# ISLA-UH/quantum-inferno

Hardware: AMD Instinct MI355X
Metric: TFR Mpoints/sec (CWT+STX+entropy) (higher is better)
Workload: dtype f32; 1 GPU; BASELINE configs[1]: 1 channel(s) per GPU x 2^20 samples @ 1000 Hz, order N=3, CWT+STX+entropy, 48 bands; channels_per_gpu=1, n=1048576, bands=48, engine=auto, world_size=1, backend=none, gather_message_bytes_per_rank=0

## Files before the change

include/qi_tfr.h:

```cpp
#ifndef QI_TFR_H
#define QI_TFR_H

#include <stddef.h>
#include <stdint.h>

#ifdef __cplusplus
extern "C" {
#endif

#define QI_TFR_ABI_VERSION 1

typedef struct qi_plan qi_plan;
typedef void* qi_stream;

typedef enum { QI_F32 = 0, QI_F64 = 1 } qi_dtype;

typedef enum {
  QI_OK = 0,
  QI_ERR_ARG = -1,
  QI_ERR_STATE = -2,
  QI_ERR_HIP = -3,
  QI_ERR_FFT = -4,
  QI_ERR_NOMEM = -5,
  QI_ERR_UNSUPPORTED = -6
} qi_status;

typedef enum {
  QI_BANK_STYX = 0,
  QI_BANK_ATOMS = 1
} qi_bank;

typedef enum {
  QI_ENGINE_AUTO = 0,
  QI_ENGINE_HIPFFT = 1,
  QI_ENGINE_NATIVE = 2
} qi_engine;

typedef struct {
  int64_t n;
  int32_t dtype;
  int32_t device;
  int32_t engine;
  int32_t flags;
  int64_t workspace_bytes;
} qi_plan_desc;

typedef struct {
  void* coef;
  void* bits;
  void* power_band;
  void* power_time;
  void* stats;
  double power_scale;
  double eps;
} qi_tfr_out;

int qi_abi_version(void);
const char* qi_last_error(void);
int qi_device_info(int device, char* name, size_t name_len, int64_t* hbm_bytes, int32_t* compute_units);

int qi_plan_create(qi_plan** plan, const qi_plan_desc* desc);
int qi_plan_destroy(qi_plan* plan);

int qi_plan_set_gabor_bank(qi_plan* plan, int bank, int32_t n_bands, const double* p_re, const double* p_im,
                           const double* omega, const double* amp, qi_stream stream);

int qi_gabor_atoms(int device, int64_t n, int32_t n_bands, const double* p_re, const double* p_im,
                   const double* omega, const double* amp, void* out, qi_stream stream);

int qi_gabor_atoms_at(int device, int64_t n, int32_t n_bands, const double* p_re, const double* p_im,
                      const double* omega, const double* amp, const void* x, void* out, qi_stream stream);

int qi_plan_set_stx_bands(qi_plan* plan, int32_t n_bands, const int64_t* shift_index, const double* sigma);

int64_t qi_plan_bands(const qi_plan* plan, int which );
int64_t qi_plan_stage_bands(const qi_plan* plan, int which, int stage);

typedef struct {
  int32_t stage, cls, run_cls, flags;
} qi_band_route;
#define QI_ROUTE_ANALYTIC(f) ((f) & 3)
#define QI_ROUTE_NARROW(f) (((f) >> 2) & 3)
#define QI_ROUTE_NOWRAP 16
#define QI_ROUTE_SPLIT 32
#define QI_ROUTE_PASS2_KIND(f) (((f) >> 6) & 3)
#define QI_ROUTE_BEHIND 256
#define QI_ROUTE_F64_ZOOM 512
int qi_plan_band_route(const qi_plan* plan, int which, int32_t band, int64_t records, qi_band_route* route);

typedef enum {
  QI_STAGE_FORWARD = 0,
  QI_STAGE_MULTIPLY = 1,
  QI_STAGE_INVERSE = 2,
  QI_STAGE_EPILOGUE = 3,
  QI_STAGE_PASS1 = 4,
  QI_STAGE_PASS2 = 5,
  QI_STAGE_BLOCK = 6,
  QI_STAGE_ZOOM = 7,
  QI_STAGE_ZOOM_COARSE = 8,
  QI_STAGE_COUNT = 9
} qi_stage;
int qi_plan_profile(qi_plan* plan, int enable);
int qi_plan_profile_read(qi_plan* plan, double* stage_ms, int64_t* stage_launches, int32_t n_stages);

int qi_cwt(qi_plan* plan, int bank, const void* sig, int64_t n_channels, const qi_tfr_out* out, qi_stream stream);

int qi_stx(qi_plan* plan, const void* sig, int64_t n_channels, const qi_tfr_out* out, qi_stream stream);

int qi_cwt_stx(qi_plan* plan, int bank, const void* sig, int64_t n_channels, const qi_tfr_out* out_cwt,
               const qi_tfr_out* out_stx, qi_stream stream);

int64_t qi_stft_segments(int64_t n, int64_t seg, int64_t hop);
int64_t qi_stft_scratch_bytes(int dtype, int64_t n_channels, int64_t n, int64_t seg, int64_t hop, int64_t nfft);
int qi_stft(int dtype, int device, const void* sig, int64_t n_channels, int64_t n, const void* window, int64_t seg,
            int64_t hop, int64_t nfft, double scale, void* Z, void* bits, double eps, void* scratch,
            int64_t scratch_bytes, qi_stream stream);

int64_t qi_welch_scratch_bytes(int dtype, int64_t n_channels, int64_t n, int64_t seg, int64_t hop, int64_t nfft);
int qi_welch(int dtype, int device, const void* sig, int64_t n_channels, int64_t n, const void* window, int64_t seg,
             int64_t hop, int64_t nfft, double scale, void* pxx, void* scratch, int64_t scratch_bytes,
             qi_stream stream);

int qi_power_marginals(int dtype, int device, const void* power, int64_t n_channels, int64_t n_bands, int64_t n,
                       void* power_band, void* power_time, void* stats, void* scratch, int64_t scratch_bytes,
                       qi_stream stream);
int64_t qi_power_marginals_scratch_bytes(int64_t n_channels, int64_t n_bands, int64_t n);

int qi_log2_offset(int dtype, int device, const void* in, void* out, int64_t n_channels, int64_t count, double eps,
                   const void* ref, qi_stream stream);

int qi_widen(int device, const void* in, void* out, int64_t count, qi_stream stream);

int qi_log2_abs(int dtype, int device, const void* in, int is_complex, void* out, int64_t count, double eps,
                qi_stream stream);

int qi_shannon_panel(int dtype, int device, const void* power, const void* mult, int mode, int64_t n_channels,
                     int64_t n_bands, int64_t n, double deg_free, void* info, void* shannon_bits, void* isnr,
                     void* esnr, qi_stream stream);

int64_t qi_sliding_scratch_bytes(int dtype, int64_t n_channels, int64_t nfft, int64_t n_slices);
int qi_sliding_stft(int dtype, int device, const void* sig, int64_t n_channels, int64_t n, const void* window,
                    int64_t seg, int64_t hop, int64_t nfft, int64_t first, int64_t n_slices, int pad_mode, int detrend,
                    int64_t roll, void* Z, void* real_out, int real_kind, void* scratch, int64_t scratch_bytes,
                    qi_stream stream);
int qi_sliding_istft(int dtype, int device, const void* S, int64_t n_channels, const void* dual_window, int64_t seg,
                     int64_t hop, int64_t nfft, int64_t first, int64_t n_slices, int64_t roll, int64_t k0, int64_t k1,
                     void* out, void* scratch, int64_t scratch_bytes, qi_stream stream);

int qi_shannon_1d(int dtype, int device, const void* marginal, int64_t n_channels, int64_t n, void* info, void* entropy,
                  void* isnr, void* esnr, qi_stream stream);
int64_t qi_shannon_scratch_bytes(int dtype, int64_t n_channels, int64_t n);
int qi_shannon_tdr(int dtype, int device, const void* sig, int64_t n_channels, int64_t n, void* sig_norm, void* marginal,
                   void* scratch, int64_t scratch_bytes, qi_stream stream);
int qi_shannon_fft(int dtype, int device, const void* sig, int64_t n_channels, int64_t n, void* spectrum, void* angle,
                   void* marginal, void* scratch, int64_t scratch_bytes, qi_stream stream);

#ifdef __cplusplus
}
#endif
// ... 2 lines not shown
```

quantum_inferno_amd/_lib.py:

```python
import ctypes as C
import os

import torch

_HERE = os.path.dirname(os.path.abspath(__file__))
LIB_PATH = os.environ.get("QI_TFR_LIB") or os.path.join(_HERE, "libqi_tfr.so")

QI_F32, QI_F64 = 0, 1
QI_BANK_STYX, QI_BANK_ATOMS, QI_TABLE_STX = 0, 1, 2
QI_ENGINE_AUTO, QI_ENGINE_HIPFFT, QI_ENGINE_NATIVE = 0, 1, 2
STAGES = ("forward", "multiply", "inverse", "epilogue", "pass1", "pass2", "block", "zoom", "zoom_coarse")
ROUTE_NOWRAP, ROUTE_SPLIT, ROUTE_BEHIND, ROUTE_F64_ZOOM = 16, 32, 256, 512


def route_analytic(flags):
    return flags & 3


def route_narrow(flags):
    return (flags >> 2) & 3


def route_pass2_kind(flags):
    return (flags >> 6) & 3


class QiError(RuntimeError):
    pass


class PlanDesc(C.Structure):
    _fields_ = [
        ("n", C.c_int64),
        ("dtype", C.c_int32),
        ("device", C.c_int32),
        ("engine", C.c_int32),
        ("flags", C.c_int32),
        ("workspace_bytes", C.c_int64),
    ]


class BandRoute(C.Structure):
    _fields_ = [("stage", C.c_int32), ("cls", C.c_int32), ("run_cls", C.c_int32), ("flags", C.c_int32)]


class TfrOut(C.Structure):
    _fields_ = [
        ("coef", C.c_void_p),
        ("bits", C.c_void_p),
        ("power_band", C.c_void_p),
        ("power_time", C.c_void_p),
        ("stats", C.c_void_p),
        ("power_scale", C.c_double),
        ("eps", C.c_double),
    ]


_P = C.c_void_p
_D = C.POINTER(C.c_double)
_I64 = C.POINTER(C.c_int64)
_i64, _i32, _int, _dbl = C.c_int64, C.c_int32, C.c_int, C.c_double

PROTOTYPES = {
    "qi_abi_version": (_int, []),
    "qi_last_error": (C.c_char_p, []),
    "qi_device_info": (_int, [_int, C.c_char_p, C.c_size_t, _I64, C.POINTER(_i32)]),
    "qi_plan_create": (_int, [C.POINTER(_P), C.POINTER(PlanDesc)]),
    "qi_plan_destroy": (_int, [_P]),
    "qi_plan_set_gabor_bank": (_int, [_P, _int, _i32, _D, _D, _D, _D, _P]),
    "qi_gabor_atoms": (_int, [_int, _i64, _i32, _D, _D, _D, _D, _P, _P]),
    "qi_gabor_atoms_at": (_int, [_int, _i64, _i32, _D, _D, _D, _D, _P, _P, _P]),
    "qi_plan_set_stx_bands": (_int, [_P, _i32, _I64, _D]),
    "qi_plan_bands": (_i64, [_P, _int]),
    "qi_plan_stage_bands": (_i64, [_P, _int, _int]),
    "qi_plan_band_route": (_int, [_P, _int, _i32, _i64, C.POINTER(BandRoute)]),
    "qi_plan_profile": (_int, [_P, _int]),
    "qi_plan_profile_read": (_int, [_P, _D, _I64, _i32]),
    "qi_cwt": (_int, [_P, _int, _P, _i64, C.POINTER(TfrOut), _P]),
    "qi_stx": (_int, [_P, _P, _i64, C.POINTER(TfrOut), _P]),
    "qi_cwt_stx": (_int, [_P, _int, _P, _i64, C.POINTER(TfrOut), C.POINTER(TfrOut), _P]),
    "qi_stft_segments": (_i64, [_i64, _i64, _i64]),
    "qi_stft_scratch_bytes": (_i64, [_int, _i64, _i64, _i64, _i64, _i64]),
    "qi_stft": (_int, [_int, _int, _P, _i64, _i64, _P, _i64, _i64, _i64, _dbl, _P, _P, _dbl, _P, _i64, _P]),
    "qi_welch_scratch_bytes": (_i64, [_int, _i64, _i64, _i64, _i64, _i64]),
    "qi_welch": (_int, [_int, _int, _P, _i64, _i64, _P, _i64, _i64, _i64, _dbl, _P, _P, _i64, _P]),
    "qi_power_marginals": (_int, [_int, _int, _P, _i64, _i64, _i64, _P, _P, _P, _P, _i64, _P]),
    "qi_power_marginals_scratch_bytes": (_i64, [_i64, _i64, _i64]),
    "qi_log2_offset": (_int, [_int, _int, _P, _P, _i64, _i64, _dbl, _P, _P]),
    "qi_widen": (_int, [_int, _P, _P, _i64, _P]),
    "qi_log2_abs": (_int, [_int, _int, _P, _int, _P, _i64, _dbl, _P]),
    "qi_shannon_panel": (_int, [_int, _int, _P, _P, _int, _i64, _i64, _i64, _dbl, _P, _P, _P, _P, _P]),
    "qi_sliding_scratch_bytes": (_i64, [_int, _i64, _i64, _i64]),
    "qi_sliding_stft": (_int, [_int, _int, _P, _i64, _i64, _P, _i64, _i64, _i64, _i64, _i64, _int, _int, _i64, _P, _P, _int, _P, _i64, _P]),
    "qi_sliding_istft": (_int, [_int, _int, _P, _i64, _P, _i64, _i64, _i64, _i64, _i64, _i64, _i64, _i64, _P, _P, _i64, _P]),
    "qi_shannon_1d": (_int, [_int, _int, _P, _i64, _i64, _P, _P, _P, _P, _P]),
    "qi_shannon_scratch_bytes": (_i64, [_int, _i64, _i64]),
    "qi_shannon_tdr": (_int, [_int, _int, _P, _i64, _i64, _P, _P, _P, _i64, _P]),
    "qi_shannon_fft": (_int, [_int, _int, _P, _i64, _i64, _P, _P, _P, _P, _i64, _P]),
}

_lib = None


def _hip_runtimes_mapped():
    try:
        with open("/proc/self/maps") as fh:
            return sorted({ln.split()[-1] for ln in fh if "libamdhip64" in ln})
    except OSError:
        return []


def load():
    global _lib
    if _lib is not None:
        return _lib
    if not os.path.exists(LIB_PATH):
        raise QiError(
            f"{LIB_PATH} is missing: build it with `python -c 'import __graft_entry__ as g; g.build()'` "
            "(hipcc --offload-arch=gfx950).  There is no CPU fallback."
        )
    lib = C.CDLL(LIB_PATH)
    for name, (res, args) in PROTOTYPES.items():
        fn = getattr(lib, name)
        fn.restype = res
        fn.argtypes = args
    rts = _hip_runtimes_mapped()
    if len(rts) > 1:
        raise QiError(f"two HIP runtimes are mapped ({rts}); libqi_tfr.so must share torch's")
    _lib = lib
    return lib


def check(rc):
    if rc != 0:
        msg = load().qi_last_error()
        raise QiError(f"libqi_tfr error {rc}: {msg.decode() if msg else '?'}")


def require_gpu():
    if not torch.cuda.is_available():
        raise QiError("no HIP device visible: the TFR transforms run only on the GPU (no CPU fallback)")
    return load()


def darr(a):
    import numpy as np

    a = np.ascontiguousarray(a, dtype=np.float64)
    return a, a.ctypes.data_as(_D)


def iarr(a):
    import numpy as np

    a = np.ascontiguousarray(a, dtype=np.int64)
    return a, a.ctypes.data_as(_I64)

# ... 8 lines not shown
```

quantum_inferno_amd/csrc/qi_api.hip:

```cpp
#include "qi_host.hpp"

using namespace qi;
using namespace qi::host;

extern "C" {

int qi_abi_version(void) { return QI_TFR_ABI_VERSION; }
const char* qi_last_error(void) { return qi::last_error(); }

int qi_device_info(int device, char* name, size_t name_len, int64_t* hbm_bytes, int32_t* compute_units) {
  hipDeviceProp_t prop;
  QI_HIP(hipGetDeviceProperties(&prop, device));
  if (name && name_len) snprintf(name, name_len, "%s (%s)", prop.name, prop.gcnArchName);
  if (hbm_bytes) *hbm_bytes = (int64_t)prop.totalGlobalMem;
  if (compute_units) *compute_units = prop.multiProcessorCount;
  return QI_OK;
}

int qi_plan_create(qi_plan** plan, const qi_plan_desc* desc) {
  QI_REQUIRE(plan && desc, "null plan/desc");
  *plan = nullptr;
  QI_REQUIRE(desc->n >= 2 && desc->n <= (1ll << 28), "n = %lld out of range", (long long)desc->n);
  QI_REQUIRE(desc->dtype == QI_F32 || desc->dtype == QI_F64, "bad dtype %d", desc->dtype);
  QI_REQUIRE(desc->engine >= QI_ENGINE_AUTO && desc->engine <= QI_ENGINE_NATIVE, "bad engine %d", desc->engine);
  QI_REQUIRE(desc->flags == 0, "qi_plan_desc.flags = %d: the field is reserved and must be 0", desc->flags);
  if (desc->engine == QI_ENGINE_NATIVE && !(is_pow2(desc->n) && desc->n >= (1 << 18) &&
                                            (desc->dtype == QI_F32 || desc->n == (1 << 20)))) {
    set_error("native engine: float32 records of a power-of-two length >= 2^18, float64 records of 2^20 samples (got n = %lld, dtype %d)",
              (long long)desc->n, desc->dtype);
    return QI_ERR_UNSUPPORTED;
  }
  DeviceGuard g(desc->device);
  if (!g.ok) {
    set_error("hipSetDevice(%d) failed", desc->device);
    return QI_ERR_HIP;
  }
  qi_plan* p = new (std::nothrow) qi_plan();
  QI_REQUIRE(p, "out of host memory");
  p->d = *desc;
  p->n = desc->n;
  p->L = is_pow2(desc->n) ? 2 * desc->n : next_pow2(2 * desc->n - 1);
  if (p->native_kmax > (int64_t)native::kMaxPrunedTerms * native::kN2)
    p->native_kmax = (int64_t)native::kMaxPrunedTerms * native::kN2;
  if (const char* e = tune_env("QI_NATIVE_DEBUG")) p->native_debug = atoi(e);
  if (const char* e = tune_env("QI_NATIVE_FWD")) p->native_fwd = atoi(e);
#ifdef QI_NATIVE_STAMPS
  if (tune_env("QI_NATIVE_STAMPS")) {
    if (hipMalloc((void**)&p->stamps, 65536 * 8 * sizeof(unsigned long long)) != hipSuccess) p->stamps = nullptr;
    if (p->stamps) (void)hipMemset(p->stamps, 0, 65536 * 8 * sizeof(unsigned long long));
    if (hipMalloc((void**)&p->blk_stamps, 65536 * 8 * sizeof(unsigned long long)) != hipSuccess) p->blk_stamps = nullptr;
    if (p->blk_stamps) (void)hipMemset(p->blk_stamps, 0, 65536 * 8 * sizeof(unsigned long long));
  }
#endif
  if (const char* e = tune_env("QI_NATIVE_SHORT")) p->native_short = atoi(e);
  if (const char* e = tune_env("QI_NATIVE_BLOCK")) p->native_block = atoi(e);
  if (const char* e = tune_env("QI_NATIVE_ZOOM")) p->native_zoom = atoi(e);
  if (const char* e = tune_env("QI_NATIVE_ZOOM_LEVELS")) p->native_zoom_max_level = atoi(e);
  if (const char* e = tune_env("QI_NATIVE_SPLIT")) p->native_split = atoi(e);
  if (const char* e = tune_env("QI_NATIVE_FUSE")) p->native_fuse = atoi(e);
  if (const char* e = tune_env("QI_NATIVE_F64")) p->native_f64 = atoi(e);
  if (const char* e = tune_env("QI_NATIVE_Z64")) p->native_z64 = atoi(e);
  if (const char* e = tune_env("QI_NATIVE_Z64_FINE")) p->native_z64_fine = atoi(e);
  if (const char* e = tune_env("QI_NATIVE_Z64_COARSE")) p->native_z64_coarse = atoi(e);
  if (const char* e = tune_env("QI_NATIVE_Z64_BLOCK_FROM")) p->native_z64_block_from = atoi(e);
  if (const char* e = tune_env("QI_NATIVE_BLK64_WTAB")) p->native_blk64_wtab = atoi(e);
  if (const char* e = tune_env("QI_NATIVE_BLK64_NARROW")) p->native_blk64_narrow = atoi(e);
  if (const char* e = tune_env("QI_NATIVE_MIN_LOG2N")) p->native_min_log2n = atoi(e);
  if (desc->dtype == QI_F64) {
    if (!tune_env("QI_NATIVE_MIN_LOG2N")) p->native_min_log2n = 15;
    const int short64 = p->native_short && !(tune_env("QI_NATIVE_SHORT64") && atoi(tune_env("QI_NATIVE_SHORT64")) == 0);
    const int block64 = p->native_block && !(tune_env("QI_NATIVE_BLOCK64") && atoi(tune_env("QI_NATIVE_BLOCK64")) == 0);
    const int split64 = p->native_split && block64 && p->native_z64 &&
                        !(tune_env("QI_NATIVE_SPLIT64") && atoi(tune_env("QI_NATIVE_SPLIT64")) == 0);
    p->native_zoom = 0;
    p->native_split = split64;
    p->native_split_e = 2048;
    p->native_block = block64;
    p->native_short = short64;
    p->native_rows = 8;
    if (p->native_group <= 0) p->native_group = 8;
  }
  p->ws_bytes = desc->workspace_bytes > 0 ? (size_t)desc->workspace_bytes : ((size_t)2 << 30);
  if (hipMalloc((void**)&p->ws, p->ws_bytes) != hipSuccess) {
    set_error("hipMalloc of %zu workspace bytes failed", p->ws_bytes);
    delete p;
    return QI_ERR_HIP;
  }
  *plan = p;
  return QI_OK;
}

int qi_plan_destroy(qi_plan* p) {
  if (!p) return QI_OK;
  DeviceGuard g(p->d.device);
  (void)hipDeviceSynchronize();
  p->fft.clear();
  p->prof.clear();
#ifdef QI_NATIVE_STAMPS
  if (p->stamps) {
    std::vector<unsigned long long> h(65536 * 8);
    if (hipMemcpy(h.data(), p->stamps, h.size() * sizeof(unsigned long long), hipMemcpyDeviceToHost) == hipSuccess) {
      double sum[8] = {0};
      long cnt = 0;
      for (size_t w = 0; w < 65536; ++w) {
        unsigned long long tot = 0;
        for (int k = 0; k < 8; ++k) tot += h[w * 8 + k];
        if (!tot) continue;
        ++cnt;
        for (int k = 0; k < 8; ++k) sum[k] += (double)h[w * 8 + k];
      }
      fprintf(stderr, "[qi stamps] last pass-2 launch, %ld workgroups, mean cycles per workgroup: load %.0f | barrier %.0f | "
              "step1 %.0f | barrier %.0f | exchange %.0f | step2 %.0f | epilogue %.0f | loop head %.0f\n", cnt,
              sum[0] / cnt, sum[1] / cnt, sum[2] / cnt, sum[3] / cnt, sum[4] / cnt, sum[5] / cnt, sum[6] / cnt, sum[7] / cnt);
    }
    (void)hipFree(p->stamps);
  }
  if (p->blk_stamps) {
    std::vector<unsigned long long> h(65536 * 8);
    if (hipMemcpy(h.data(), p->blk_stamps, h.size() * sizeof(unsigned long long), hipMemcpyDeviceToHost) == hipSuccess) {
      if (const char* path = tune_env("QI_NATIVE_TIMELINE")) {
        if (FILE* f = fopen(path, "w")) {
          fprintf(f, "wg start_10ns end_10ns xcc cu bands wq\n");
          const unsigned long long m48 = 0xffffffffffffull;
          for (size_t w = 0; w < 65536; ++w)
            if (h[w * 8 + 7])
              fprintf(f, "%zu %llu %llu %llu %llu %llu %lld\n", w, h[w * 8 + 6] & m48, h[w * 8 + 7] & m48, h[w * 8 + 6] >> 56,
                      (h[w * 8 + 6] >> 48) & 0xff, (h[w * 8 + 7] >> 48) & 0xff, (long long)(signed char)(h[w * 8 + 7] >> 56));
          fclose(f);
// ... 94 lines not shown
  if (!use_native && p->d.engine == QI_ENGINE_NATIVE) {
    set_error("native engine does not support this bank at n = %lld", (long long)p->n);
    return QI_ERR_UNSUPPORTED;
  }
  drop_gabor_tables(p, bank);
  drop_band_slots(p, bank);
  const int rc = build_gabor_bank(p, bank, B, p_re, p_im, omega, amp, use_native, st);
  if (rc == QI_OK) {
    p->nb[bank] = B;
  } else {
    drop_gabor_tables(p, bank);
    free_device(p->bank[bank]);
  }
  return rc;
}

static int atoms_rows(int64_t n, int32_t B, const double* p_re, const double* p_im, const double* omega, const double* amp,
                      const double* x, void* out, hipStream_t st) {
  std::vector<double> host;
  DeviceTemp<double> d_par;
  QI_TRY(upload_atom_params(B, p_re, p_im, omega, amp, &host, &d_par));
  const double* q = d_par.ptr;
  QI_TRY(launch_bank_rows((double2*)out, n, n, 1, q, q + B, q + 2 * B, q + 3 * B, 0, B, st, 0.0, x));
  if (hipStreamSynchronize(st) != hipSuccess) {
    set_error("atom kernel failed: %s", hipGetErrorString(hipGetLastError()));
    return QI_ERR_HIP;
  }
  return QI_OK;
}

int qi_gabor_atoms(int device, int64_t n, int32_t B, const double* p_re, const double* p_im, const double* omega,
                   const double* amp, void* out, qi_stream stream) {
  QI_REQUIRE(p_re && p_im && omega && amp && out, "null argument");
  QI_REQUIRE(n >= 2 && B > 0 && B <= 65535, "bad atom bank shape");
  DeviceGuard g(device);
  return atoms_rows(n, B, p_re, p_im, omega, amp, nullptr, out, (hipStream_t)stream);
}

int qi_gabor_atoms_at(int device, int64_t n, int32_t B, const double* p_re, const double* p_im, const double* omega,
                      const double* amp, const void* x, void* out, qi_stream stream) {
  QI_REQUIRE(p_re && p_im && omega && amp && x && out, "null argument");
  QI_REQUIRE(n >= 1 && B > 0 && B <= 65535, "bad atom bank shape");
  DeviceGuard g(device);
  return atoms_rows(n, B, p_re, p_im, omega, amp, static_cast<const double*>(x), out, (hipStream_t)stream);
}

int qi_plan_set_stx_bands(qi_plan* p, int32_t B, const int64_t* shift_index, const double* sigma) {
  QI_REQUIRE(p && shift_index && sigma, "null argument");
  QI_REQUIRE(B > 0 && B <= 65535, "band count %d out of range", B);
  for (int32_t j = 0; j < B; ++j)
    QI_REQUIRE(shift_index[j] >= 0 && shift_index[j] < p->n, "shift_index[%d] = %lld outside [0, n)", j,
               (long long)shift_index[j]);
  for (int32_t j = 0; j < B; ++j)
    QI_REQUIRE(std::isfinite(sigma[j]) && sigma[j] > 0.0, "sigma[%d] = %g: must be positive and finite", j, sigma[j]);
  DeviceGuard g(p->d.device);
  p->table_gen++;
  if (p->d_stx_idx) {
    QI_HIP(hipDeviceSynchronize());
    QI_HIP(hipFree(p->d_stx_idx));
    QI_HIP(hipFree(p->d_stx_coef));
    p->d_stx_idx = nullptr;
    p->d_stx_coef = nullptr;
    p->nb_stx = 0;
  }
  std::vector<double> coef(B);
  const double k = 2.0 * M_PI / (double)p->n * std::sqrt(0.5 * M_LOG2E);
  for (int32_t j = 0; j < B; ++j) coef[j] = sigma[j] * k;
  QI_TRY(upload_table(&p->d_stx_idx, std::vector<int64_t>(shift_index, shift_index + B)));
  QI_TRY(upload_table(&p->d_stx_coef, coef));
  p->nb_stx = 0;
  drop_stx_tables(p);
  drop_band_slots(p, 2);
  QI_TRY(build_stx_tables(p, B, shift_index, sigma, coef));
  p->nb_stx = B;
  return QI_OK;
}

int64_t qi_plan_bands(const qi_plan* p, int which) {
  if (!p) return 0;
  if (which == QI_BANK_STYX || which == QI_BANK_ATOMS) return p->nb[which];
  return which == 2 ? p->nb_stx : 0;
}

int64_t qi_plan_stage_bands(const qi_plan* p, int which, int stage) {
  if (!p || which < 0 || which > 2) return 0;
  const int64_t total = qi_plan_bands(p, which);
  if (!p->nat[which].ready) return stage == QI_STAGE_INVERSE ? total : 0;
  int64_t blk = 0;
  if (which != 1 && p->blk[which].ready) blk = p->blk[which].rows;
  const int64_t zoom = p->nat[which].nzoom + p->nat[which].nz64;
  const int64_t left = which == 2 ? p->stx_left_n : 0;
  if (stage == QI_STAGE_BLOCK) return blk;
  if (stage == QI_STAGE_ZOOM) return zoom;
  if (stage == QI_STAGE_INVERSE) return left;
  return stage == QI_STAGE_PASS2 ? total - blk - zoom - left : 0;
}

int qi_plan_band_route(const qi_plan* p, int which, int32_t band, int64_t records, qi_band_route* route) {
  QI_REQUIRE(p && route, "null argument");
  QI_REQUIRE(which >= 0 && which <= 2, "bad table %d", which);
  QI_REQUIRE(band >= 0 && band < qi_plan_bands(p, which), "band %d outside the table's %lld rows", band,
             (long long)qi_plan_bands(p, which));
  QI_REQUIRE(records > 0, "records must be positive");
  *route = qi_band_route{QI_STAGE_INVERSE, 0, 0, 0};
  const auto& t = p->nat[which];
  if (!t.ready) return QI_OK;
  if (which == 2 && p->stx_left_n > 0 && band >= p->stx_left_lo && band < p->stx_left_lo + p->stx_left_n) {
    route->flags = QI_ROUTE_BEHIND;
    return QI_OK;
  }
  int found = 0;
  const bool split = which == 0 && std::find(p->h_split_bands.begin(), p->h_split_bands.end(), band) != p->h_split_bands.end();
  for (const auto& z : t.h_zoom)
    if (z.first == band) {
      const int run = records < p->native_zoom_short_from && z.second >= native::kZoomLevels ? 0 : z.second;
      *route = qi_band_route{QI_STAGE_ZOOM, z.second, run, split ? QI_ROUTE_SPLIT : 0};
      ++found;
    }
  for (size_t q = 0; q < t.h_z64.size(); ++q)
    if (t.h_z64[q] == band) {
      int level = -1, fine = -1;
      for (int g = 0; g < native::kZ64Levels; ++g)
        if ((int32_t)q >= t.z64_first[g] && (int32_t)q < t.z64_first[g] + t.z64_count[g]) level = g;
      for (int c = 0; c < native::kZ64FineClasses; ++c)
        if ((int32_t)q >= t.zf_first[c] && (int32_t)q < t.zf_first[c] + t.zf_count[c]) fine = c;
      *route = qi_band_route{QI_STAGE_ZOOM, level, fine, QI_ROUTE_F64_ZOOM | (split ? QI_ROUTE_SPLIT : 0)};
      ++found;
    }
  if (which != 1 && p->blk[which].ready) {
    const int cut = records >= batch_from(p) ? 1 : 0;
    for (const auto& b : p->blk[which].var[cut].h_route)
      if (b.out_band == band) {
        *route = qi_band_route{QI_STAGE_BLOCK, b.wq, b.wq, (b.analytic & 3) | ((b.narrow & 3) << 2) | (b.nowrap ? QI_ROUTE_NOWRAP : 0)};
        ++found;
      }
  }
  for (size_t q = 0; q < t.h_rows.size(); ++q)
    if (t.h_rows[q] == band) {
      *route = qi_band_route{QI_STAGE_PASS2, 0, 0, (t.h_row_mode[q] & 3) << 6};
      ++found;
    }
  if (which == 0 && p->nat[3].ready)
    for (int32_t r : p->nat[3].h_rows)
      if (r == band) {
        *route = qi_band_route{QI_STAGE_PASS2, 0, 0, 2 << 6};
        ++found;
      }
  if (found != 1) {
    set_error("band %d of table %d has %d producers", band, which, found);
    return QI_ERR_STATE;
  }
  return QI_OK;
}

int qi_plan_profile(qi_plan* p, int enable) {
  QI_REQUIRE(p, "null plan");
  DeviceGuard g(p->d.device);
  double ms[Profiler::kStages];
  int64_t c[Profiler::kStages];
  p->prof.read(ms, c);
  p->prof.on = enable != 0;
  p->prof.mask = (enable & 0xFFFF) == 1 ? ~0u : (uint32_t)(enable & 0xFFFF) >> 1;
  p->prof.period = (enable >> 16) > 0 ? (enable >> 16) : 1;
  p->prof.tick = 0;
  return QI_OK;
}
// ... 120 lines not shown
```

quantum_inferno_amd/csrc/qi_block.hip:

```cpp
#include "qi_common.hpp"
#include "qi_device.hpp"
#include "qi_native.hpp"
#include "qi_fft_reg.hpp"
#include "qi_zoom_gather.hpp"

namespace qi {
namespace native {

namespace {

constexpr int kBlkThreads = 256;
#ifndef QI_BLK_WAVES
#define QI_BLK_WAVES 3
#endif
#ifndef QI_BLK_LONG_WAVES
#define QI_BLK_LONG_WAVES 2
#endif
#ifdef QI_NATIVE_DEBUG
#define QI_BDBG(bit) (a.debug & (bit))
#else
#define QI_BDBG(bit) false
#endif
#ifdef QI_NATIVE_STAMPS
#define QI_BSTAMP(k)                                               \
// ... 1150 lines not shown
  __shared__ cplx<T> buf[kBlkBuf];
  __shared__ cplx<T> tw256[256];
  __shared__ double s_red[2][kBlkThreads / kWave];
  const int tid = threadIdx.x;
  {
    float s, c;
    sincospif((float)tid * (2.0f / 256.0f), &s, &c);
    tw256[tid] = mk<T>((T)c, (T)s);
  }
  cplx<T> w;
  {
    float s, c;
    const int lane = tid & (kWave - 1);
    const int col = (tid & ~(kWave - 1)) + (lane < 32 ? 2 * lane : 2 * (lane - 32) + 1);
    sincospif((float)col * (2.0f / 4096.0f), &s, &c);
    w = mk<T>((T)c, (T)s);
  }
  const DualItem it = load_uniform(items + blockIdx.x);
#ifdef QI_NATIVE_STAMPS
  const unsigned long long wall0 = __builtin_amdgcn_s_memrealtime();
#endif
  if (it.wq < 0) {
    const BlockItem e{it.wq, it.block, it.first0, it.count0, it.plane0, it.slot0};
    switch (-it.wq) {
      case 1: edge_item<T, 1, COEF, BITS>(a0, e, buf, tw256, w); break;
      case 2: edge_item<T, 2, COEF, BITS>(a0, e, buf, tw256, w); break;
      default: edge_item<T, 4, COEF, BITS>(a0, e, buf, tw256, w); break;
    }
  } else {
    switch (it.wq) {
      case 1: dual_item<T, 1, COEF, BITS>(a0, a2, it, buf, tw256, s_red, w); break;
      case 2: dual_item<T, 2, COEF, BITS>(a0, a2, it, buf, tw256, s_red, w); break;
      default: dual_item<T, 4, COEF, BITS>(a0, a2, it, buf, tw256, s_red, w); break;
    }
  }
#ifdef QI_NATIVE_STAMPS
  if (a0.stamps && tid == 0) {
    asm volatile("s_waitcnt vmcnt(0) lgkmcnt(0)" ::: "memory");
    unsigned long long* o = a0.stamps + ((int64_t)blockIdx.z * gridDim.x + blockIdx.x) * 8;
    unsigned hw;
    asm volatile("s_getreg_b32 %0, hwreg(HW_REG_HW_ID)" : "=s"(hw));
    unsigned xcc;
    asm volatile("s_getreg_b32 %0, hwreg(HW_REG_XCC_ID)" : "=s"(xcc));
    o[6] = (wall0 & 0xffffffffffffull) | ((unsigned long long)(xcc & 15) << 56) | ((unsigned long long)((hw >> 8) & 0xff) << 48);
    o[7] = (__builtin_amdgcn_s_memrealtime() & 0xffffffffffffull) | ((unsigned long long)(it.wq & 0xff) << 56) |
           ((unsigned long long)((it.count0 + it.count2) & 0xff) << 48);
  }
#endif
}

template <typename T>
__device__ __forceinline__ void zoom_coarse_plane(cplx<T>* __restrict__ plane0) {
  __shared__ cplx<T> buf[kBlkBuf];
  __shared__ cplx<T> tw256[256];
  const int tid = threadIdx.x, lane = tid & (kWave - 1);
  const int col = (tid & ~(kWave - 1)) + (lane < 32 ? 2 * lane : 2 * (lane - 32) + 1);
  cplx<T>* __restrict__ plane = plane0 + col;
  cplx<T> v[16];
#pragma unroll
  for (int b = 0; b < 16; ++b) v[b] = plane[256 * b];
  {
    float s, c;
    sincospif((float)tid * (2.0f / 256.0f), &s, &c);
    tw256[tid] = mk<T>((T)c, (T)s);
  }
  cplx<T> w;
  {
    float s, c;
    sincospif((float)col * (2.0f / 4096.0f), &s, &c);
    w = mk<T>((T)c, (T)s);
  }
  fft4096<T, 1>(v, buf, tw256, w, tid, col);
#pragma unroll
  for (int c = 0; c < 16; ++c) plane[256 * c] = v[brev(c, 4)];
}
template <typename T, bool STX, int NF>
__device__ __forceinline__ void zoom_coarse_plane_gather(const ZoomArgs<T>& a, const uint32_t plane_i,
                                                         cplx<T>* __restrict__ buf, cplx<T>* __restrict__ tw256) {
  const int tid = threadIdx.x, lane = tid & (kWave - 1);
  const int col = (tid & ~(kWave - 1)) + (lane < 32 ? 2 * lane : 2 * (lane - 32) + 1);
  const BandDesc bd = load_uniform(a.bands + *as_const(a.plane_band + plane_i));
  const uint32_t tau1 = plane_i - (uint32_t)bd.edge;
  const int64_t ch = blockIdx.z;
  const cplx<T>* __restrict__ X = a.X + ch * (a.Lf << a.x_shift);
  cplx<T> v[16];
#ifdef QI_NATIVE_DEBUG
  if (a.debug & 256) {
#pragma unroll
    for (int b = 0; b < 16; ++b) v[b] = mk<T>((T)(col + b), (T)tau1);
  } else
#endif
  zoom_gather16<T, STX, NF>(a, bd, tau1, col, X, v);
  {
    float s, c;
    sincospif((float)tid * (2.0f / 256.0f), &s, &c);
    tw256[tid] = mk<T>((T)c, (T)s);
  }
  cplx<T> w;
  {
    float s, c;
    sincospif((float)col * (2.0f / 4096.0f), &s, &c);
    w = mk<T>((T)c, (T)s);
  }
#ifdef QI_NATIVE_DEBUG
  if (!(a.debug & 512))
#endif
  fft4096<T, 1>(v, buf, tw256, w, tid, col);
  cplx<T>* __restrict__ plane = a.coarse + ((int64_t)ch * a.planes + plane_i) * kBlk + col;
#ifdef QI_NATIVE_DEBUG
  if ((a.debug & 1024) && v[3].x != (T)12345.678f) return;
#endif
#pragma unroll
  for (int c = 0; c < 16; ++c) plane[256 * c] = v[brev(c, 4)];
}
template <typename T, int NF>
__global__ void __launch_bounds__(kBlkThreads) k_zoom_coarse2g(ZoomArgs<T> a0, ZoomArgs<T> a2) {
  __shared__ cplx<T> buf[kBlkBuf];
  __shared__ cplx<T> tw256[256];
#ifdef QI_COARSE_PLAIN_ORDER
  const uint32_t pi = blockIdx.x;
#else
  const uint32_t q = blockIdx.x >> 3, pi = (q >> 3) * 64u + (blockIdx.x & 7u) * 8u + (q & 7u);
#endif
  if (pi >= (uint32_t)(a0.planes + a2.planes)) return;
  if (pi < (uint32_t)a0.planes) zoom_coarse_plane_gather<T, false, NF>(a0, pi, buf, tw256);
  else zoom_coarse_plane_gather<T, true, NF>(a2, pi - (uint32_t)a0.planes, buf, tw256);
}
template <typename T, bool STX>
__global__ void __launch_bounds__(kBlkThreads) k_zoom_coarse_g(ZoomArgs<T> a) {
  __shared__ cplx<T> buf[kBlkBuf];
  __shared__ cplx<T> tw256[256];
  zoom_coarse_plane_gather<T, STX, 8>(a, blockIdx.x, buf, tw256);
}

template <typename T>
__global__ void __launch_bounds__(kBlkThreads) k_zoom_coarse(ZoomArgs<T> a) {
  zoom_coarse_plane<T>(a.coarse + ((int64_t)blockIdx.z * a.planes + blockIdx.x) * kBlk);
}
template <typename T>
__global__ void __launch_bounds__(kBlkThreads) k_zoom_coarse2(ZoomArgs<T> a0, ZoomArgs<T> a2) {
  const bool first = blockIdx.x < (uint32_t)a0.planes;
  const ZoomArgs<T>& a = first ? a0 : a2;
  const int64_t plane = first ? blockIdx.x : blockIdx.x - (uint32_t)a0.planes;
  zoom_coarse_plane<T>(a.coarse + ((int64_t)blockIdx.z * a.planes + plane) * kBlk);
}

__global__ void k_block_taps_gabor(double2* __restrict__ g, int w, const double* __restrict__ par, int nb_total,
                                   const int32_t* __restrict__ ids) {
  const int j = ids[blockIdx.y];
  const double p_re = par[j], p_im = par[nb_total + j], omega = par[2 * nb_total + j], amp = par[3 * nb_total + j];
  double2* row = g + (int64_t)blockIdx.y * kBlk;
  for (int m = blockIdx.x * blockDim.x + threadIdx.x; m < kBlk; m += gridDim.x * blockDim.x) {
    int u;
    bool on = true;
    if (m <= w) u = -m;
    else if (m > kBlk - w) u = kBlk - m;
    else { u = 0; on = false; }
    double2 v = make_double2(0.0, 0.0);
    if (on) {
      const double x = (double)u + 0.5;
      const double env = amp * exp(-p_re * x * x);
      const double ph = omega * x - p_im * x * x;
      double s, c;
      sincos(ph, &s, &c);
      v = make_double2(env * c, -env * s);
    }
    row[m] = v;
// ... 357 lines not shown
```

quantum_inferno_amd/csrc/qi_host.hpp:

```cpp
#pragma once
#include <algorithm>
#include <cmath>
#include <cstring>
#include <map>
#include <mutex>
#include <new>
#include <tuple>
#include <vector>

#include <cstdlib>

#include "qi_common.hpp"
#include "qi_native.hpp"

namespace qi {

struct DeviceGuard {
  int prev = -1;
  bool ok = true;
  explicit DeviceGuard(int dev) {
    if (hipGetDevice(&prev) != hipSuccess) prev = -1;
    if (prev != dev) ok = hipSetDevice(dev) == hipSuccess;
  }
  ~DeviceGuard() {
// ... 141 lines not shown
    cur = last = -1;
  }
  void clear() {
    double ms[kStages];
    int64_t c[kStages];
    read(ms, c);
    for (auto e : pool) (void)hipEventDestroy(e);
    pool.clear();
  }
};

template <typename P>
inline void free_device(P*& ptr) {
  if (ptr) (void)hipFree(ptr);
  ptr = nullptr;
}
template <typename P, typename X>
inline int upload_table(P** dst, const std::vector<X>& v) {
  QI_HIP(hipMalloc((void**)dst, v.size() * sizeof(X)));
  QI_HIP(hipMemcpy(*dst, v.data(), v.size() * sizeof(X), hipMemcpyHostToDevice));
  return QI_OK;
}
template <typename X>
struct DeviceTemp {
  X* ptr = nullptr;
  DeviceTemp() = default;
  DeviceTemp(const DeviceTemp&) = delete;
  DeviceTemp& operator=(const DeviceTemp&) = delete;
  ~DeviceTemp() { free_device(ptr); }
};

extern std::mutex g_stft_mu;
extern std::map<int, FftCache> g_stft_fft;
const char* last_error();

}

using namespace qi;

struct FusedCarry {
  bool active = false;
  size_t ws_used = 0;
  native::BlockArgs<float> blk{};
  int demod = 0;
  int64_t ct = 0;
  native::TailCall<float> tail;
  bool has_zoom = false;
  native::ZoomArgs<float> zoom{};
};

struct qi_plan {
  qi_plan_desc d{};
  int64_t n = 0;
  int64_t L = 0;
  void* bank[2] = {nullptr, nullptr};
  int32_t nb[2] = {0, 0};
  int64_t* d_stx_idx = nullptr;
  double* d_stx_coef = nullptr;
  int32_t nb_stx = 0;
  char* ws = nullptr;
  size_t ws_bytes = 0;
  FftCache fft;
  Profiler prof;
  struct NativeGroup {
    int32_t first = 0, count = 0;
    int32_t gen_first = 0, ngen = 0;
  };
  struct NativeTable {
    bool ready = false;
    int64_t Lf = 0;
    int32_t nbands = 0, ngen = 0, imd_slots = 0;
    native::BandDesc* d_bands = nullptr;
    int32_t* d_gen_list = nullptr;
    std::vector<NativeGroup> groups;
    void* Hc = nullptr;
    void* Hfull = nullptr;
    native::BandDesc* d_zoom = nullptr;
    int32_t* d_zoom_plane_band = nullptr;
    std::vector<std::pair<int32_t, int32_t>> h_zoom;
    std::vector<int32_t> h_rows;
    std::vector<int32_t> h_row_mode;
    std::vector<int32_t> h_z64;
    int32_t nzoom = 0, zoom_count[native::kZoomClasses] = {0, 0, 0, 0, 0, 0, 0};
    int64_t zoom_planes = 0;
    int zoom_max_level = 0;
    native::BandDesc* d_z64 = nullptr;
    int32_t nz64 = 0, z64_first[native::kZ64Levels] = {}, z64_count[native::kZ64Levels] = {};
    int32_t zf_first[native::kZ64FineClasses] = {}, zf_count[native::kZ64FineClasses] = {};
    double2* d_z64_lane_ph = nullptr;
    double2* d_z64_wave_ph = nullptr;
    void release() {
      free_device(d_z64);
      free_device(d_z64_lane_ph);
      free_device(d_z64_wave_ph);
      free_device(d_zoom);
      free_device(d_zoom_plane_band);
      free_device(d_bands);
      free_device(d_gen_list);
      free_device(Hc);
      free_device(Hfull);
      *this = NativeTable();
    }
  } nat[4];
  struct BlockTable {
    bool ready = false;
    int demod = 0;
    void* bank = nullptr;
    int32_t rows = 0;
    struct ItemList {
      void* d_bands = nullptr;
      void* d_demod_pow = nullptr;
      void* d_gauss_w = nullptr;
      std::vector<std::pair<int32_t, int32_t>> h_bands;
      struct Route {
        int32_t out_band, wq, analytic, narrow, nowrap;
      };
      std::vector<Route> h_route;
      native::BlockItem* d_items = nullptr;
      int32_t nitems = 0, nplanes = 0;
      int32_t nlong = 0;
      int32_t nedge_items = 0;
      bool edge_merged = false;
      std::vector<native::BlockItem> h_items;
    } var[2];
    int64_t max_blocks = 0;
    void release() {
      free_device(bank);
      for (auto& v : var) {
        free_device(v.d_bands);
        free_device(v.d_demod_pow);
        free_device(v.d_gauss_w);
        free_device(v.d_items);
      }
      *this = BlockTable();
    }
  } blk[3];
  struct {
    int64_t C = -1, tile = 0;
    unsigned flags = 0;
    uint64_t gen = 0;
  } tile_cache;
  uint64_t table_gen = 1;
  int native_block = 1;
  const void* shared_sig = nullptr;
  int64_t shared_C = 0;
  bool shared_valid = false;
  int32_t* d_band_slots[3][2] = {};
  int native_zoom = 1;
  int native_zoom_short = 1;
  int native_zoom_short_from = 4;
  int native_zoom_max_level = 3;
  int native_zoom_waves = 2048;
  int native_zoom_wgs_joint = 768;
  int native_zoom_wgs = 0;
  float* d_zoom_w[native::kZoomClasses] = {};
  int native_z64 = 1;
  int native_z64_levels = native::kZ64Levels;
  double* d_z64_w[native::kZ64Levels] = {};
  double* d_z64f_w[native::kZ64FineClasses] = {};
  double2* d_demod_t1 = nullptr;
  double2* d_demod_t2 = nullptr;
  int native_z64_fine = 1;
  int32_t stx_left_lo = -1, stx_left_n = 0;
  int native_min_log2n = 14;
  int native_blk64_narrow = 1;
  int native_blk64_wtab = 1;
  int native_z64_block_from = 4;
  int native_z64_coarse = 3;
  int native_z64_rows = 0;
  int native_f64 = 1;
  int native_gather_fused = 1;
  hipStream_t side = nullptr;
  hipEvent_t ev_fork = nullptr, ev_join = nullptr;
  int native_split = 1;
  int64_t native_split_e = 1024;
  void* split_bank = nullptr;
  int32_t* d_split_bands = nullptr;
  std::vector<int32_t> h_split_bands;
  int32_t nsplit = 0;
  int native_blk_analytic = 1;
  FusedCarry carry;
  native::DualItem* d_dual[2] = {nullptr, nullptr};
  int32_t n_dual[2] = {0, 0};
  int32_t n_dual_long[2] = {0, 0};
  bool dual_valid[2] = {false, false};
  int native_fuse = 4;
  int native_blk_narrow = 1;
  int native_blk_fastw = 1;
  int native_edge_merge = 1;
  int native_blk_long = 1;
  int native_blk_half = 1;
  int native_tail = 1;
  int64_t native_tile = 0;
  int native_blk_maxwq = 4;
  int native_blk_bands = 6;
  int native_blk_bands_batch = 12;
  int native_blk_batch_from = 0;
  native::EdgeBand* d_edge = nullptr;
  int32_t nedge = 0;
  int64_t edge_wmax = 0;
  int native_short = 1;
  int64_t native_kmax = 12288;
  int native_debug = 0;
  int native_fwd = 1;
  int native_wgs = 256;
  unsigned long long* stamps = nullptr;
  unsigned long long* blk_stamps = nullptr;
  int native_group = 0;
  int native_rows = 16;
};

namespace qi {
namespace host {

inline size_t align_up(size_t v, size_t a = 256) { return (v + a - 1) / a * a; }
inline double power_scale_or_default(double power_scale) { return power_scale == 0.0 ? 1.0 : power_scale; }
inline double eps_or_default(double eps) { return eps == 0.0 ? 2.220446049250313e-16 : eps; }
enum class Kind { Linear, Circular, Stockwell };
#ifdef QI_HOST_SANITIZE
void layout_begin(const qi_plan* p, const char* run, bool keep_previous);
void layout_note(const qi_plan* p, const char* what, const void* ptr, size_t bytes, bool shared = false);
#define QI_LAYOUT_BEGIN(p, run, keep) ::qi::host::layout_begin(p, run, keep)
#define QI_LAYOUT_NOTE(p, what, ptr, bytes, ...) ::qi::host::layout_note(p, what, ptr, bytes, ##__VA_ARGS__)
#else
#define QI_LAYOUT_BEGIN(p, run, keep) ((void)0)
#define QI_LAYOUT_NOTE(p, what, ptr, bytes, ...) ((void)0)
#endif
constexpr int kZoomListOrder[native::kZoomClasses] = {6, 5, 0, 1, 2, 3, 4};

bool native_len_ok(int64_t Lf);
bool native_wanted(const qi_plan* p, int kind);
int batch_from(const qi_plan* p);
void release_styx_extras(qi_plan* p);
void drop_gabor_tables(qi_plan* p, int bank);
void drop_stx_tables(qi_plan* p);
void drop_band_slots(qi_plan* p, int kind);
int upload_atom_params(int32_t B, const double* p_re, const double* p_im, const double* omega, const double* amp,
                       std::vector<double>* host, DeviceTemp<double>* d_par);
template <typename T>
int build_native_bank(qi_plan* p, int bank, int32_t B, const double* d_par, const double* h_par, hipStream_t st);
template <typename T>
int build_bank(qi_plan* p, int bank, int32_t B, const double* d_par, hipStream_t st);
int build_stx_tables(qi_plan* p, int32_t B, const int64_t* shift_index, const double* sigma, const std::vector<double>& coef);

template <typename T>
int run_transform(qi_plan* p, Kind kind, const void* sig_v, int64_t C, const qi_tfr_out* out, hipStream_t st);
template <typename T>
int run_native(qi_plan* p, int kind, const void* sig_v, int64_t C, const qi_tfr_out* out, hipStream_t st,
               bool may_share = false, FusedCarry* defer = nullptr, FusedCarry* finish = nullptr, size_t* probe = nullptr);
template <typename T>
int run_stx_leftover(qi_plan* p, const void* sig, int64_t C, const qi_tfr_out* out, hipStream_t st);
int run_native64(qi_plan* p, int kind, const void* sig_v, int64_t C, const qi_tfr_out* out, hipStream_t st);
int flush_carry(qi_plan* p, FusedCarry* c, hipStream_t st);

}
}
```

quantum_inferno_amd/csrc/qi_host_util.hip:

```cpp
#include "qi_host.hpp"

namespace qi {

static thread_local char g_err[512] = "";

const char* tune_env(const char* name) {
  static const bool on = std::getenv("QI_TUNE") != nullptr;
  return on ? std::getenv(name) : nullptr;
}

void set_error(const char* fmt, ...) {
  va_list ap;
  va_start(ap, fmt);
  vsnprintf(g_err, sizeof(g_err), fmt, ap);
  va_end(ap);
}

const char* last_error() { return g_err; }

template <typename T>
int fft_c2c(FftCache& fc, cplx<T>* data, int64_t len, int64_t batch, int dir, hipStream_t st);
template <>
int fft_c2c<float>(FftCache& fc, float2* data, int64_t len, int64_t batch, int dir, hipStream_t st) {
  hipfftHandle h;
  QI_TRY(fc.get(HIPFFT_C2C, len, batch, &h));
  QI_FFT(hipfftSetStream(h, st));
  QI_FFT(hipfftExecC2C(h, (hipfftComplex*)data, (hipfftComplex*)data, dir));
  return QI_OK;
}
template <>
int fft_c2c<double>(FftCache& fc, double2* data, int64_t len, int64_t batch, int dir, hipStream_t st) {
  hipfftHandle h;
  QI_TRY(fc.get(HIPFFT_Z2Z, len, batch, &h));
  QI_FFT(hipfftSetStream(h, st));
  QI_FFT(hipfftExecZ2Z(h, (hipfftDoubleComplex*)data, (hipfftDoubleComplex*)data, dir));
  return QI_OK;
}
int fft_z2z_rows(FftCache& fc, double2* data, int64_t len, int64_t dist, int64_t batch, int dir, hipStream_t st) {
  hipfftHandle h;
  QI_TRY(fc.get(HIPFFT_Z2Z, len, batch, &h, dist));
  QI_FFT(hipfftSetStream(h, st));
  QI_FFT(hipfftExecZ2Z(h, (hipfftDoubleComplex*)data, (hipfftDoubleComplex*)data, dir));
  return QI_OK;
}
template <typename T>
int fft_r2c(FftCache& fc, T* in, cplx<T>* out, int64_t len, int64_t batch, hipStream_t st);
template <>
int fft_r2c<float>(FftCache& fc, float* in, float2* out, int64_t len, int64_t batch, hipStream_t st) {
  hipfftHandle h;
  QI_TRY(fc.get(HIPFFT_R2C, len, batch, &h));
  QI_FFT(hipfftSetStream(h, st));
  QI_FFT(hipfftExecR2C(h, in, (hipfftComplex*)out));
  return QI_OK;
}
template <>
int fft_r2c<double>(FftCache& fc, double* in, double2* out, int64_t len, int64_t batch, hipStream_t st) {
  hipfftHandle h;
  QI_TRY(fc.get(HIPFFT_D2Z, len, batch, &h));
  QI_FFT(hipfftSetStream(h, st));
  QI_FFT(hipfftExecD2Z(h, in, (hipfftDoubleComplex*)out));
  return QI_OK;
}

template <typename T>
int fft_c2r(FftCache& fc, cplx<T>* in, T* out, int64_t len, int64_t batch, hipStream_t st);
template <>
int fft_c2r<float>(FftCache& fc, float2* in, float* out, int64_t len, int64_t batch, hipStream_t st) {
  hipfftHandle h;
  QI_TRY(fc.get(HIPFFT_C2R, len, batch, &h));
  QI_FFT(hipfftSetStream(h, st));
  QI_FFT(hipfftExecC2R(h, (hipfftComplex*)in, out));
  return QI_OK;
}
template <>
int fft_c2r<double>(FftCache& fc, double2* in, double* out, int64_t len, int64_t batch, hipStream_t st) {
  hipfftHandle h;
  QI_TRY(fc.get(HIPFFT_Z2D, len, batch, &h));
  QI_FFT(hipfftSetStream(h, st));
  QI_FFT(hipfftExecZ2D(h, (hipfftDoubleComplex*)in, out));
  return QI_OK;
}

std::mutex g_stft_mu;
std::map<int, FftCache> g_stft_fft;

}

#ifdef QI_HOST_SANITIZE
namespace qi {
namespace host {
namespace {
struct LayoutRegion {
// ... 40 lines not shown
```

quantum_inferno_amd/csrc/qi_native.hip:

```cpp
#include <utility>

#include "qi_common.hpp"
#include "qi_device.hpp"
#include "qi_native.hpp"
#include "qi_fft_reg.hpp"
#include "qi_finalize.hpp"

namespace qi {
namespace native {

namespace {

template <typename T, int G_ = 16>
struct Cfg {
  static constexpr int NR = 1024, G = G_, TH = 64 * G_;
  static constexpr int SR = NR + 1;
  static constexpr int SA = 16 * G + 1;
  static constexpr int BUF = (G * SR > 64 * SA) ? G * SR : 64 * SA;
  static constexpr int TW1 = (kMaxPrunedTerms + 1) * G;
  static constexpr int TW2 = 64;
  static constexpr size_t LDS_BYTES = ((size_t)BUF + NR + TW2 + TW1) * sizeof(cplx<T>) + 256;
};

#ifdef QI_NATIVE_DEBUG
// ... 162 lines not shown
    }
  }
}

template <typename T, class C>
__device__ __forceinline__ void fill_step_twiddles(cplx<T>* tw) {
  for (int i = threadIdx.x; i < C::NR + C::TW2; i += C::TH) {
    T sf, cf;
    if (i < C::NR) {
      const int d = i / 64, aa = i % 64;
      sincospi_as<T>((double)(2 * (aa * d)) / (double)C::NR, &sf, &cf);
    } else {
      const int c2 = (i - C::NR) / 16, a1 = (i - C::NR) % 16;
      sincospi_as<T>((double)(2 * (a1 * c2)) / 64.0, &sf, &cf);
    }
    tw[i] = mk<T>(cf, sf);
  }
}

template <typename T, class C, class F, class F2>
__device__ __forceinline__ void rows_fft1024_regs(cplx<T> (&v)[16], cplx<T>* buf, const cplx<T>* tw, cplx<T> (&u)[16],
                                                  bool skip, F between, F2 before_step2
#ifdef QI_NATIVE_STAMPS
                                                  , unsigned long long (&st_acc)[8], unsigned long long& st_last
#endif
) {
  const int tid = threadIdx.x;
  const int g1 = tid / 64, a1 = tid % 64;
  const int d2 = tid / (4 * C::G), c2 = (tid % (4 * C::G)) / C::G, g2 = tid % C::G;
  if (!skip) {
    fft_reg<T, 16, 1>(v);
#pragma unroll
    for (int d = 1; d < 16; ++d) v[brev(d, 4)] = cmul(v[brev(d, 4)], tw[d * 64 + a1]);
  }
  __builtin_amdgcn_sched_barrier(0);
  QI_STAMP(2);
  __syncthreads();
  QI_STAMP(3);
  between();
#pragma unroll
  for (int d = 0; d < 16; ++d) buf[a1 * C::SA + d * C::G + g1] = v[brev(d, 4)];
  __builtin_amdgcn_sched_barrier(0);
  __syncthreads();
  const T sg = (c2 & 1) ? T(-1) : T(1), tau = (c2 & 2) ? T(-1) : T(1);
  const bool odd = c2 & 1;
  const cplx<T>* __restrict__ col = buf + d2 * C::G + g2;
#pragma unroll
  for (int a = 0; a < 16; ++a) {
    const cplx<T> t0 = col[a * C::SA], t1 = col[(a + 16) * C::SA], t2 = col[(a + 32) * C::SA], t3 = col[(a + 48) * C::SA];
    const cplx<T> u02 = mk<T>(t0.x + sg * t2.x, t0.y + sg * t2.y), u13 = mk<T>(t1.x + sg * t3.x, t1.y + sg * t3.y);
    const cplx<T> w13 = odd ? mk<T>(-u13.y, u13.x) : u13;
    u[a] = mk<T>(u02.x + tau * w13.x, u02.y + tau * w13.y);
  }
  __builtin_amdgcn_sched_barrier(0);
  __syncthreads();
  QI_STAMP(4);
  before_step2();
  if (!skip) {
#pragma unroll
    for (int a = 1; a < 16; ++a) u[a] = cmul(u[a], tw[C::NR + c2 * 16 + a]);
    fft_reg<T, 16, 1>(u);
  }
  __builtin_amdgcn_sched_barrier(0);
  QI_STAMP(5);
}

template <typename T, class C>
__device__ __forceinline__ void rows_fft1024(cplx<T>* buf, const cplx<T>* tw, cplx<T> (&u)[16], bool skip
#ifdef QI_NATIVE_STAMPS
                                             , unsigned long long (&st_acc)[8], unsigned long long& st_last
#endif
) {
  const int g1 = threadIdx.x / 64, a1 = threadIdx.x % 64;
  cplx<T> v[16];
#pragma unroll
  for (int b = 0; b < 16; ++b) v[b] = buf[g1 * C::SR + a1 + 64 * b];
#ifdef QI_NATIVE_STAMPS
  rows_fft1024_regs<T, C>(v, buf, tw, u, skip, [] {}, [] {}, st_acc, st_last);
#else
  rows_fft1024_regs<T, C>(v, buf, tw, u, skip, [] {}, [] {});
#endif
}

template <typename T, class C, int SRC, int NPH>
__global__ void __launch_bounds__(C::TH) k_pass1(RowArgs<T> a) {
  extern __shared__ __attribute__((aligned(16))) char smem[];
  cplx<T>* buf = reinterpret_cast<cplx<T>*>(smem);
  cplx<T>* tw = buf + C::BUF;
  const int tid = threadIdx.x;
  const int64_t ch = blockIdx.z;
  const int split = (NPH > 1 && a.phase_split) ? NPH : 1;
  uint32_t bx = blockIdx.x, by = blockIdx.y;
  if (SRC == 2 && gridDim.y == 1 && (gridDim.x & 7) == 0) {
    bx = (bx & 7u) * (gridDim.x >> 3) + (bx >> 3);
  } else if (SRC == 2 && NPH == 2 && split == 2 && gridDim.y == 2 && (gridDim.x & 7) == 0) {
    const uint32_t lin = bx + gridDim.x * by, per = gridDim.x >> 3;
    bx = (lin & 7u) * per + ((lin >> 3) >> 1);
    by = (lin >> 3) & 1u;
  }
  const uint32_t row0 = bx * C::G;
  const int d2 = tid / (4 * C::G), c2 = (tid % (4 * C::G)) / C::G, g2 = tid % C::G;
  fill_step_twiddles<T, C>(tw);
  const int ph_first = split > 1 ? (int)(by % NPH) : 0, ph_last = split > 1 ? ph_first + 1 : NPH;
  BandDesc bd{};
  if constexpr (SRC != 2) bd = a.bands[a.gen_list[by / split]];
  const cplx<T>* Xc = SRC == 2 ? nullptr : a.X + ch * a.Lf;
  const T* sigc = SRC == 2 ? a.sig + ch * a.n : nullptr;
  const uint32_t mask = (uint32_t)a.Lf - 1u;
  const uint32_t k2 = row0 + g2;
  cplx<T>* __restrict__ dst = a.imd + ((int64_t)ch * a.imd_slots + bd.gen_slot) * a.Lf + k2;
  const uint32_t roll = a.neg_last_row ? 1u : 0u, cmask = (uint32_t)a.N1 - 1u;
#ifdef QI_NATIVE_STAMPS
  unsigned long long st_acc[8] = {0, 0, 0, 0, 0, 0, 0, 0};
  unsigned long long st_last = __builtin_amdgcn_s_memtime();
#endif
#pragma unroll 1
  for (int ph = ph_first; ph < ph_last; ++ph) {
    if (!QI_DBG(2)) load_full<T, C, SRC, NPH>(buf, a, bd, Xc, sigc, row0, ph);
    __builtin_amdgcn_sched_barrier(0);
    __syncthreads();
    cplx<T> u[16];
#ifdef QI_NATIVE_STAMPS
    rows_fft1024<T, C>(buf, tw, u, QI_DBG(4), st_acc, st_last);
#else
    rows_fft1024<T, C>(buf, tw, u, QI_DBG(4));
#endif
    double wr, wi, sr, si;
    unit_root_t<T>((k2 * (uint32_t)(NPH * (d2 + 16 * c2) + ph)) & mask, a.two_over_len, &wr, &wi);
    unit_root_t<T>((k2 * (uint32_t)(64 * NPH)) & mask, a.two_over_len, &sr, &si);
#pragma unroll
    for (int c1 = 0; c1 < 16; ++c1) {
      const cplx<T> z = u[brev(c1, 4)];
      const uint32_t t1 = (uint32_t)(NPH * (d2 + 16 * c2 + 64 * c1)) + (uint32_t)ph;
      if (c1 == 15 && a.neg_last_row && t1 == cmask)
        unit_root_t<T>((0u - k2) & mask, a.two_over_len, &wr, &wi);
      const T cr = (T)wr, ci = (T)wi;
      if (!QI_DBG(1)) dst[(size_t)((t1 + roll) & cmask) * kN2] = mk<T>(z.x * cr - z.y * ci, z.x * ci + z.y * cr);
      const double nr = wr * sr - wi * si;
      wi = wr * si + wi * sr;
      wr = nr;
    }
  }
}

template <typename T, class C>
__global__ void __launch_bounds__(C::TH) k_fwd2(RowArgs<T> a, cplx<T>* __restrict__ Xout) {
  extern __shared__ __attribute__((aligned(16))) char smem[];
  cplx<T>* buf = reinterpret_cast<cplx<T>*>(smem);
  cplx<T>* tw = buf + C::BUF;
  const int tid = threadIdx.x;
  const int64_t ch = blockIdx.z;
  const uint32_t row0 = blockIdx.x * C::G;
  const int d2 = tid / (4 * C::G), c2 = (tid % (4 * C::G)) / C::G, g2 = tid % C::G;
  fill_step_twiddles<T, C>(tw);
  cplx<T> v[16], u[16];
  load_imd_direct<T>(v, a.imd + (int64_t)ch * a.imd_slots * a.Lf, row0 + tid / 64, tid % 64);
  __syncthreads();
#ifdef QI_NATIVE_STAMPS
  unsigned long long st_acc[8] = {0, 0, 0, 0, 0, 0, 0, 0};
  unsigned long long st_last = 0;
  rows_fft1024_regs<T, C>(v, buf, tw, u, false, [] {}, [] {}, st_acc, st_last);
#else
  rows_fft1024_regs<T, C>(v, buf, tw, u, false, [] {}, [] {});
#endif
  cplx<T>* __restrict__ dst = Xout + ch * a.Lf + row0 + g2 + (uint32_t)a.N1 * (d2 + 16 * c2);
  const uint32_t tstep = 64u * (uint32_t)a.N1;
#pragma unroll
  for (int c1 = 0; c1 < 16; ++c1) {
    const cplx<T> z = u[brev(c1, 4)];
    dst[(size_t)c1 * tstep] = mk<T>(z.x, -z.y);
  }
}

template <typename T, class C, int KIND, bool COEF, bool BITS>
__global__ void __launch_bounds__(C::TH) k_pass2(RowArgs<T> a) {
  constexpr bool STX = KIND == 2;
  constexpr int NOUT = KIND == 0 ? 8 : 16;
  extern __shared__ __attribute__((aligned(16))) char smem[];
  cplx<T>* buf = reinterpret_cast<cplx<T>*>(smem);
  cplx<T>* tw = buf + C::BUF;
  __shared__ double s_red[2][C::TH / kWave];
  __shared__ double s_fin[3][C::TH / kWave];
  __shared__ double ltab[sizeof(T) == 8 ? 128 : 1][2];
  const int tid = threadIdx.x, lane = tid & (kWave - 1), wv = tid / kWave;
  if (sizeof(T) == 8 && tid < 128) {
    ltab[tid][0] = kLog2Tab[tid][0];
    ltab[tid][1] = kLog2Tab[tid][1];
  }
  const int64_t grp = blockIdx.x, ch = blockIdx.z;
  const uint32_t row0 = (uint32_t)grp * C::G;
  const int d2 = tid / (4 * C::G), c2 = (tid % (4 * C::G)) / C::G, g2 = tid % C::G;
  fill_step_twiddles<T, C>(tw);
  __syncthreads();

  T col[NOUT];
#pragma unroll
  for (int c = 0; c < NOUT; ++c) col[c] = T(0);
  T mx = T(0);
  double plogp = 0.0;
  const uint32_t t1_first = row0 - (KIND == 0 ? 1u : 0u);
  const uint32_t tbase = row0 + g2 + (uint32_t)a.N1 * (d2 + 16 * c2);
  const uint32_t tstep = 64u * (uint32_t)a.N1;
  const cplx<T>* Xc = a.X + ch * a.Lf;
  int64_t pending = -1;
  int par = 0;

#ifdef QI_NATIVE_STAMPS
  unsigned long long st_acc[8] = {0, 0, 0, 0, 0, 0, 0, 0};
  unsigned long long st_last = __builtin_amdgcn_s_memtime();
#endif
  for (int64_t jj = blockIdx.y; jj < a.nbands; jj += gridDim.y) {
    const BandDesc bd = a.bands[jj];
    const int64_t j = bd.out_band;
    QI_STAMP(7);
    cplx<T> v[16], u[16];
    auto flush = [&] {
      if (pending >= 0 && tid == 0) {
        double s = 0.0;
        for (int w = 0; w < C::TH / kWave; ++w) s += s_red[par ^ 1][w];
        a.part_band[((int64_t)ch * a.panel_bands + pending) * a.nblk + grp] = s;
      }
    };
    if (bd.mode == 0) {
      if (!QI_DBG(2)) load_pruned<T, C, STX>(buf, tw + C::NR + C::TW2, a, bd, Xc, t1_first);
      __builtin_amdgcn_sched_barrier(0);
      QI_STAMP(0);
      __syncthreads();
      QI_STAMP(1);
#pragma unroll
      for (int b = 0; b < 16; ++b) v[b] = buf[(tid / 64) * C::SR + (tid % 64) + 64 * b];
    } else {
      if (!QI_DBG(2))
        load_imd_direct<T>(v, a.imd + ((int64_t)ch * a.imd_slots + bd.gen_slot) * a.Lf, row0 + tid / 64, tid % 64);
      QI_STAMP(0);
    }
#ifdef QI_NATIVE_STAMPS
    rows_fft1024_regs<T, C>(v, buf, tw, u, QI_DBG(4), flush, [] {}, st_acc, st_last);
#else
    rows_fft1024_regs<T, C>(v, buf, tw, u, QI_DBG(4), flush, [] {});
#endif

    const int64_t orow = ((int64_t)ch * a.panel_bands + j) * a.n;
    char* __restrict__ coef_row = reinterpret_cast<char*>(a.coef ? a.coef + orow : nullptr);
    char* __restrict__ bits_row = reinterpret_cast<char*>(a.bits ? a.bits + orow : nullptr);
    uint32_t tb = tbase;
    asm volatile("" : "+v"(tb));
    T rowacc = T(0), pl = T(0);
    if (KIND == 1 && !COEF && bd.edge > 0 && a.edge_z) {
      cplx<T>* ez = a.edge_z + ((int64_t)ch * a.nedge + bd.edge_slot) * 2 * a.edge_wmax;
      const uint32_t t_lo = tb, t_hi = (uint32_t)a.n - 1u - (tb + 15u * tstep);
      if (t_lo < (uint32_t)bd.edge) ez[t_lo] = u[brev(8, 4)];
      if (t_hi < (uint32_t)bd.edge) ez[a.edge_wmax + t_hi] = u[brev(7, 4)];
    }
#pragma unroll
// ... 285 lines not shown
    const double p = f[k].x * f[k].x + f[k].y * f[k].y;
    m = p > m ? p : m;
  }
  m = wave_max(m);
  if (lane == 0) s[wv] = m;
  __syncthreads();
  if (tid == 0) {
    double t = 0.0;
    for (int w = 0; w < 256 / kWave; ++w) t = s[w] > t ? s[w] : t;
    s_max = t;
  }
  __syncthreads();
  const double cut = s_max * thr2;
  double lo = (double)L, hi = -1.0, hi1 = -1.0, lo2 = (double)L;
  for (int64_t k = tid; k < L; k += 256) {
    const double p = f[k].x * f[k].x + f[k].y * f[k].y;
    if (p >= cut && p > 0.0) {
      lo = (double)k < lo ? (double)k : lo;
      hi = (double)k > hi ? (double)k : hi;
      if (k < L / 2) hi1 = (double)k > hi1 ? (double)k : hi1;
      else lo2 = (double)k < lo2 ? (double)k : lo2;
    }
  }
  lo = -wave_max(-lo);
  hi = wave_max(hi);
  hi1 = wave_max(hi1);
  lo2 = -wave_max(-lo2);
  __shared__ double s_lo[256 / kWave], s_hi[256 / kWave], s_hi1[256 / kWave], s_lo2[256 / kWave];
  if (lane == 0) {
    s_lo[wv] = lo;
    s_hi[wv] = hi;
    s_hi1[wv] = hi1;
    s_lo2[wv] = lo2;
  }
  __syncthreads();
  if (tid == 0) {
    for (int w = 0; w < 256 / kWave; ++w) {
      lo = s_lo[w] < lo ? s_lo[w] : lo;
      hi = s_hi[w] > hi ? s_hi[w] : hi;
      hi1 = s_hi1[w] > hi1 ? s_hi1[w] : hi1;
      lo2 = s_lo2[w] < lo2 ? s_lo2[w] : lo2;
    }
    if (hi1 >= 0.0 && lo2 < (double)L && (hi1 + 1.0) + ((double)L - lo2) < hi - lo + 1.0) {
      lo = lo2 - (double)L;
      hi = hi1;
    }
    out[blockIdx.x * 3 + 0] = s_max;
    out[blockIdx.x * 3 + 1] = lo;
    out[blockIdx.x * 3 + 2] = hi;
  }
}

template <typename T>
__global__ void k_copy_window(const double2* __restrict__ F, cplx<T>* __restrict__ dst, int64_t k_lo, int64_t count,
                              int conj, double scale, int64_t row_len, double ramp, int64_t ramp_center) {
  const int64_t i = (int64_t)blockIdx.x * blockDim.x + threadIdx.x;
  if (i >= count) return;
  int64_t k = k_lo + i;
  if (k < 0) k += row_len;
  if (k >= row_len) k -= row_len;
  const double2 v = F[k];
  double re = v.x * scale, im = (conj ? -v.y : v.y) * scale;
  if (ramp != 0.0) {
    double s, c;
    sincospi(2.0 * ramp * (double)(i - ramp_center), &s, &c);
    const double r2 = re * c - im * s;
    im = re * s + im * c;
    re = r2;
  }
  dst[i] = mk<T>((T)re, (T)im);
}

}


template <class Kern, typename T>
static int launch_lds(Kern kern, size_t lds, const RowArgs<T>& a, dim3 grid, int threads, hipStream_t st) {
  QI_TRY(allow_dynamic_lds(reinterpret_cast<const void*>(kern), lds));
  kern<<<grid, threads, lds, st>>>(a);
  QI_LAUNCH_CHECK();
  return QI_OK;
}

template <typename T, class C, int SRC, int NPH>
static int launch_p1(const RowArgs<T>& a, dim3 grid, hipStream_t st) {
  return launch_lds(k_pass1<T, C, SRC, NPH>, C::LDS_BYTES, a, grid, C::TH, st);
}
template <typename T, class C, int KIND, bool COEF, bool BITS>
static int launch_p2v(const RowArgs<T>& a, dim3 grid, hipStream_t st) {
  return launch_lds(k_pass2<T, C, KIND, COEF, BITS>, C::LDS_BYTES, a, grid, C::TH, st);
}
template <typename T, class C, int KIND>
static int launch_p2(const RowArgs<T>& a, dim3 grid, hipStream_t st) {
  if (a.coef) return a.bits ? launch_p2v<T, C, KIND, true, true>(a, grid, st) : launch_p2v<T, C, KIND, true, false>(a, grid, st);
  return a.bits ? launch_p2v<T, C, KIND, false, true>(a, grid, st) : launch_p2v<T, C, KIND, false, false>(a, grid, st);
}

template <typename T, class C>
static int launch_pass1_cfg(const RowArgs<T>& a0, int kind, int64_t n_channels, hipStream_t st) {
  RowArgs<T> a = a0;
  a.phase_split = a.N1 == 2048 && (a.N2 / C::G) * a.ngen_launch * n_channels < 256 ? 1 : 0;
  dim3 grid((unsigned)(a.N2 / C::G), (unsigned)(a.ngen_launch * (a.phase_split ? 2 : 1)), (unsigned)n_channels);
  const bool stx = kind == 2;
  if (a.N1 == 1024) return stx ? launch_p1<T, C, 1, 1>(a, grid, st) : launch_p1<T, C, 0, 1>(a, grid, st);
  if (a.N1 == 2048) return stx ? launch_p1<T, C, 1, 2>(a, grid, st) : launch_p1<T, C, 0, 2>(a, grid, st);
  set_error("native pass 1 supports N1 = 1024 or 2048, got %lld", (long long)a.N1);
  return QI_ERR_UNSUPPORTED;
}
template <>
int launch_pass1<float>(const RowArgs<float>& a, int kind, int64_t n_channels, hipStream_t st) {
  if (a.ngen_launch <= 0) return QI_OK;
  return launch_pass1_cfg<float, Cfg<float, 16>>(a, kind, n_channels, st);
}
template <>
int launch_pass1<double>(const RowArgs<double>& a, int kind, int64_t n_channels, hipStream_t st) {
  if (a.ngen_launch <= 0) return QI_OK;
  return launch_pass1_cfg<double, Cfg<double, 8>>(a, kind, n_channels, st);
}

template <typename T, class C1>
static int launch_forward_cfg(const RowArgs<T>& a0, cplx<T>* Xout, int64_t n_channels, hipStream_t st) {
  using C2 = C1;
  RowArgs<T> a = a0;
  a.phase_split = a.N1 == 2048 && (a.N2 / C1::G) * n_channels < 256 ? 1 : 0;
  dim3 g1((unsigned)(a.N2 / C1::G), a.phase_split ? 2u : 1u, (unsigned)n_channels);
  if (a.N1 == 1024)
    QI_TRY((launch_p1<T, C1, 2, 1>(a, g1, st)));
  else if (a.N1 == 2048)
    QI_TRY((launch_p1<T, C1, 2, 2>(a, g1, st)));
  else {
    set_error("native forward transform supports N1 = 1024 or 2048, got %lld", (long long)a.N1);
    return QI_ERR_UNSUPPORTED;
  }
  auto kern = k_fwd2<T, C2>;
  QI_TRY(allow_dynamic_lds(reinterpret_cast<const void*>(kern), C2::LDS_BYTES));
  dim3 g2((unsigned)(a.N1 / C2::G), 1, (unsigned)n_channels);
  kern<<<g2, C2::TH, C2::LDS_BYTES, st>>>(a, Xout);
  QI_LAUNCH_CHECK();
  return QI_OK;
}
template <>
int launch_forward<float>(const RowArgs<float>& a, float2* Xout, int64_t n_channels, hipStream_t st) {
  if (n_channels * (a.N2 / 16) < 256) return launch_forward_cfg<float, Cfg<float, 8>>(a, Xout, n_channels, st);
  return launch_forward_cfg<float, Cfg<float, 16>>(a, Xout, n_channels, st);
}
template <>
int launch_forward<double>(const RowArgs<double>& a, double2* Xout, int64_t n_channels, hipStream_t st) {
  return launch_forward_cfg<double, Cfg<double, 8>>(a, Xout, n_channels, st);
}

template <typename T, class C>
static int launch_pass2_cfg(const RowArgs<T>& a, int kind, int nchunk, int64_t n_channels, hipStream_t st) {
  dim3 grid((unsigned)(a.N1 / C::G), (unsigned)nchunk, (unsigned)n_channels);
  switch (kind) {
    case 0: return launch_p2<T, C, 0>(a, grid, st);
    case 1: return launch_p2<T, C, 1>(a, grid, st);
    default: return launch_p2<T, C, 2>(a, grid, st);
  }
}
template <>
int launch_pass2<double>(const RowArgs<double>& a, int kind, int rows_per_group, int nchunk, int64_t n_channels,
                         hipStream_t st) {
  if (rows_per_group != 8) {
    set_error("float64 pass 2 runs 8 rows per workgroup, got %d", rows_per_group);
    return QI_ERR_UNSUPPORTED;
  }
  return launch_pass2_cfg<double, Cfg<double, 8>>(a, kind, nchunk, n_channels, st);
}

template <>
int launch_pass2<float>(const RowArgs<float>& a, int kind, int rows_per_group, int nchunk, int64_t n_channels,
                        hipStream_t st) {
  if (rows_per_group == 16) return launch_pass2_cfg<float, Cfg<float, 16>>(a, kind, nchunk, n_channels, st);
  if (rows_per_group == 8) return launch_pass2_cfg<float, Cfg<float, 8>>(a, kind, nchunk, n_channels, st);
  set_error("pass 2 supports 8 or 16 rows per workgroup, got %d", rows_per_group);
  return QI_ERR_UNSUPPORTED;
}

template <typename T>
int launch_time_reduce(const T* part, T* out, int64_t C, int64_t n, int nchunk, const T* edge_time, int64_t wmax,
                       hipStream_t st) {
  const bool aligned = n % 4 == 0 && reinterpret_cast<uintptr_t>(out) % (4 * sizeof(T)) == 0 &&
                       reinterpret_cast<uintptr_t>(part) % (4 * sizeof(T)) == 0;
  if (aligned) {
    dim3 g((unsigned)(ceil_div(n, 1024) > 4096 ? 4096 : ceil_div(n, 1024)), (unsigned)C);
    k_time_reduce<T, 4><<<g, 256, 0, st>>>(part, out, n, nchunk, edge_time, wmax);
  } else {
    dim3 g((unsigned)(ceil_div(n, 256) > 4096 ? 4096 : ceil_div(n, 256)), (unsigned)C);
    k_time_reduce<T, 1><<<g, 256, 0, st>>>(part, out, n, nchunk, edge_time, wmax);
  }
  QI_LAUNCH_CHECK();
  return QI_OK;
}
template <typename T>
struct TailPack {
  const T* part;
  T* out;
  int64_t n;
  int nchunk, nfin;
  TailFin f;
};
template <typename T, int VEC>
__global__ void __launch_bounds__(256) k_tail2(TailPack<T> p0, TailPack<T> p1) {
  __shared__ double s[3][256 / kWave];
  const TailPack<T>& p = blockIdx.z == 0 ? p0 : p1;
  if ((int)blockIdx.x < p.nfin) {
    finalize_block(p.f.part_band, p.f.part_stat, p.f.power_band, p.f.stats, p.f.B, p.f.nblk, p.f.nstat, p.f.band_slots,
                   blockIdx.x, blockIdx.y, s);
    return;
  }
  time_reduce_block<T, VEC>(p.part, p.out, p.n, p.nchunk, nullptr, 0, (int64_t)blockIdx.x - p.nfin,
                            (int64_t)gridDim.x - p.nfin, blockIdx.y);
}

template <typename T>
int launch_tail(const TailCall<T>& t, hipStream_t st) {
  const bool aligned = t.n % 4 == 0 && reinterpret_cast<uintptr_t>(t.out_time) % (4 * sizeof(T)) == 0 &&
                       reinterpret_cast<uintptr_t>(t.time_part) % (4 * sizeof(T)) == 0;
  if (!aligned) {
    if (int rc = launch_time_reduce<T>(t.time_part, t.out_time, t.ct, t.n, t.chunk_total, t.edge_time, t.wmax, st)) return rc;
    return launch_finalize(t.part_band, t.part_stat, t.power_band, t.stats, t.ct, t.B, t.nbk, t.stat_slots, st, t.band_slots);
  }
  const TailFin f{t.part_band, t.part_stat, t.power_band, t.stats, t.B, t.nbk, t.stat_slots, t.band_slots};
  const int nfin = (int)t.B + 1;
  const int64_t gt = ceil_div(t.n, 1024) > 4096 ? 4096 : ceil_div(t.n, 1024);
  dim3 g((unsigned)(gt + nfin), (unsigned)t.ct);
  k_tail<T, 4><<<g, 256, 0, st>>>(t.time_part, t.out_time, t.n, t.chunk_total, t.edge_time, t.wmax, f, nfin);
  QI_LAUNCH_CHECK();
  return QI_OK;
}
// ... 77 lines not shown
```

quantum_inferno_amd/csrc/qi_native.hpp:

```cpp
#pragma once
#include "qi_common.hpp"

namespace qi {
namespace native {

constexpr int kN2 = 1024;
constexpr int kMaxPrunedTerms = 16;

struct BandDesc {
  int32_t mode;
  int32_t k_lo;
  int32_t k_len;
  int32_t gen_slot;
  int32_t out_band;
  int32_t bank_row;
  int32_t edge;
  int32_t edge_slot;
  int32_t add_row;
  int32_t pad_;
  int64_t src_off;
  int64_t shift;
  double coef;
};

template <typename T>
struct RowArgs {
  int64_t Lf, n, N1, N2;
  int32_t nbands;
  int32_t panel_bands;
  const BandDesc* bands;
  const int32_t* gen_list;
  int32_t ngen_launch, imd_slots;
  int32_t chunk_base, chunk_total;
  const T* sig;
  const cplx<T>* X;
  const cplx<T>* Hc;
  const cplx<T>* Hfull;
  cplx<T>* imd;
  T inv_len;
  float two_over_len;
  int32_t neg_last_row;
  int32_t phase_split;
  cplx<T>* coef;
  T* bits;
  cplx<T>* edge_z;
  int64_t edge_wmax;
  int32_t nedge;
  T* time_part;
  double* part_band;
  double* part_stat;
  int64_t nblk;
  int64_t stat_nblk;
  int64_t stat_stride;
  int32_t bands_per_chunk;
  T power_scale, eps;
  unsigned long long* stamps;
  int32_t debug;
};

template <typename T>
int launch_pass1(const RowArgs<T>& a, int kind, int64_t n_channels, hipStream_t st);
template <typename T>
int launch_forward(const RowArgs<T>& a, cplx<T>* Xout, int64_t n_channels, hipStream_t st);
template <typename T>
int launch_pass2(const RowArgs<T>& a, int kind, int rows_per_group, int nchunk, int64_t n_channels, hipStream_t st);
struct EdgeBand {
  int32_t out_band, w;
  double p_re, p_im, omega, amp;
};
template <typename T>
struct EdgeArgs {
  const EdgeBand* bands;
  int32_t nedge, panel_bands;
  int64_t n, wmax, stat_slots;
  const T* sig;
  cplx<T>* coef;
  cplx<T>* edge_z;
  T* bits;
  T* edge_p;
  T power_scale, eps;
};

constexpr int kBlk = 4096;
template <typename R>
struct BlockBandT {
  int32_t out_band;
  int32_t bank_row;
  int32_t shift;
  int32_t analytic;
  R rot[8];
  int32_t kappa_int;
  R kappa_frac, cw, amp;
  int32_t narrow, klo;
  R rot_a[2], rot_b[2];
  R rot8_a[2], rot8_b[2];
  R rot1[2];
  int32_t nowrap;
  R la;
};
using BlockBand = BlockBandT<float>;

constexpr int kBlkLongWq = 8;
constexpr int kBlkLong = 2 * kBlk;
constexpr int kBlkLongValid = kBlkLong - 2048;
struct BlockItem {
  int32_t wq;
  int32_t block;
  int32_t band_first, band_count;
  int32_t plane;
  int32_t stat_slot;
};
struct DualItem {
  int32_t wq, block;
  int32_t first0, count0, plane0, slot0;
  int32_t first2, count2, plane2, slot2;
};
template <typename T>
struct BlockArgs {
  int64_t n;
  int32_t nitems, panel_bands;
  int32_t nedge_items, nsplit;
  int32_t edge_merged;
  int32_t edge_wq;
  int32_t nlong;
  const int32_t* edge_band;
  const cplx<T>* edge_bank;
  const cplx<T>* edge_part;
  const BlockItem* items;
  const BlockBandT<T>* bands;
  const cplx<T>* bank;
  const T* gauss_w;
  const cplx<T>* demod_pow;
  const cplx<T>* demod_t1;
  const cplx<T>* demod_t2;
  const T* sig;
  cplx<T>* coef;
  T* bits;
  T* time_part;
  double* part_band;
  double* part_stat;
  int64_t nblk, stat_stride, stat_base;
  int32_t chunk_base, chunk_total;
  T power_scale, eps;
  float two_over_n;
  int32_t debug;
  unsigned long long* stamps;
};
int block_valid(int wq);
template <typename T>
int launch_block(const BlockArgs<T>& a, int demod, int64_t n_channels, hipStream_t st, hipStream_t side = nullptr,
                 hipEvent_t fork = nullptr, hipEvent_t join = nullptr);
template <typename T>
int launch_block_dual(const BlockArgs<T>& a0, const BlockArgs<T>& a2, const DualItem* items, int32_t nitems, int32_t nlong,
                      int32_t n_edge, int64_t n_channels, hipStream_t st);
int launch_block_taps_gabor(double2* g, int w, const double* d_par, int nb_total, const int32_t* d_ids, int count,
                            hipStream_t st);
int launch_block_taps_stx(double2* g, int w, const double2* om, int64_t n, int64_t idx, hipStream_t st);
int launch_stx_window_row(double2* row, int64_t n, double coef, hipStream_t st);
int launch_block_rotate_rows(double2* rows, int count, hipStream_t st);

int launch_block_taps_edge(double2* g, int w, int64_t n, double taper_e, const double* d_par, int nb_total,
                           const int32_t* d_ids, int count, hipStream_t st);

constexpr int kZoomD = 64;
constexpr int kZoomLevels = 5;
constexpr int kZoomClasses = 7;
constexpr int zoom_grid(int cls) { return cls < kZoomLevels ? cls : 0; }
constexpr int zoom_ntap(int cls) { return cls < kZoomLevels ? 10 : (cls == 5 ? 6 : 4); }
constexpr int zoom_design_oversampling(int cls) { return cls < kZoomLevels ? 4 : (cls == 5 ? 8 : 32); }
constexpr int zoom_span(int cls) { return 1 << zoom_grid(cls); }
constexpr int zoom_taps(int cls) { return zoom_ntap(cls) + zoom_span(cls) - 1; }
constexpr int zoom_steps(int cls) { return zoom_grid(cls) <= 2 ? 16 : (64 >> zoom_grid(cls)); }
constexpr int kZoomOversample = 4;
template <typename T>
struct ZoomArgs {
  int64_t n, Lf;
  int64_t planes;
  int32_t nbands, panel_bands;
  const BandDesc* bands;
  const int32_t* plane_band;
  int32_t lvl_first[kZoomClasses], lvl_count[kZoomClasses], lvl_chunk0[kZoomClasses], lvl_nchunk[kZoomClasses];
  int64_t lvl_stat_base[kZoomClasses];
  const float* lvl_weights[kZoomClasses];
  const cplx<T>* X;
  int32_t x_shift;
  const cplx<T>* Hc;
  cplx<T>* split_part;
  int32_t split_rows;
  int32_t debug;
  cplx<T>* coarse;
  int32_t stx;
  int32_t lane_off;
  int64_t tau_off;
  T inv_len;
  float two_over_len;
  cplx<T>* coef;
  T* bits;
  T* time_part;
  double* part_band;
  double* part_stat;
  int64_t nblk, stat_stride;
  int32_t chunk_base, chunk_total;
  T power_scale, eps;
};
int64_t zoom_groups(int64_t n, int level);
template <typename T>
int launch_zoom_gather(const ZoomArgs<T>& a, int max_level, int64_t n_channels, hipStream_t st);
template <typename T>
int launch_zoom_coarse(const ZoomArgs<T>& a, int max_level, int64_t n_channels, hipStream_t st);
template <typename T>
int launch_zoom(const ZoomArgs<T>& a, int64_t n_channels, hipStream_t st);
template <typename T>
int launch_zoom_gather2(const ZoomArgs<T>& a0, const ZoomArgs<T>& a2, int64_t n_channels, hipStream_t st);
template <typename T>
int launch_zoom2(const ZoomArgs<T>& a0, const ZoomArgs<T>& a2, int64_t n_channels, hipStream_t st);
template <typename T>
int launch_zoom_coarse2(const ZoomArgs<T>& a0, const ZoomArgs<T>& a2, int64_t n_channels, hipStream_t st);
template <typename T>
int launch_zoom_coarse_gather(const ZoomArgs<T>& a, int64_t n_channels, hipStream_t st);
template <typename T>
int launch_zoom_coarse_gather2(const ZoomArgs<T>& a0, const ZoomArgs<T>& a2, int64_t n_channels, hipStream_t st);
constexpr int kZ64Taps = 16;
#ifndef QI_Z64_TILE
#define QI_Z64_TILE 2048
#endif
constexpr int kZ64Tile = QI_Z64_TILE;
constexpr int kZ64Levels = 5;
constexpr int kZ64Pad = 16;
struct Z64Args {
  int64_t Lf, n, M;
  int32_t log2d, kind;
  int32_t nbands, panel_bands;
  const BandDesc* bands;
  const cplx<double>* X;
  const cplx<double>* Hc;
  cplx<double>* Z;
  const double* weights;
  double inv_len;
  float two_over_len;
  cplx<double>* coef;
  double* bits;
  cplx<double>* split_part;
  int32_t split_rows;
  double* time_part;
  double* part_band;
  double* part_stat;
  int64_t nblk, stat_stride;
  int64_t pb_stride, stat_nblk;
  int32_t chunk_base, chunk_total;
  double power_scale, eps;
};
int launch_z64_gather(const Z64Args& a, int64_t n_channels, hipStream_t st);
int launch_z64_interp(const Z64Args& a, int nchunk, int64_t n_channels, hipStream_t st);
int launch_z64_pad(cplx<double>* Z, int64_t M, int64_t rows, hipStream_t st);
int launch_z64_coarse(const Z64Args& a, int64_t n_channels, hipStream_t st);
void z64_weights(int log2d, double* w );

constexpr int kZ64FineLevels = 2;
constexpr int kZ64FineClasses = kZ64FineLevels + 4;
constexpr int z64f_level(int c) { return c < kZ64FineLevels ? c : 0; }
constexpr int z64f_ntap(int c) { return c < kZ64FineLevels ? 16 : 12 - 2 * (c - kZ64FineLevels); }
constexpr int z64f_oversampling(int c) { return c < kZ64FineLevels ? 4 : (8 << (c - kZ64FineLevels)); }
constexpr int z64f_span(int c) { return 1 << z64f_level(c); }
constexpr int z64f_win(int c) { return z64f_ntap(c) + z64f_span(c) - 1; }
constexpr int kZ64FineSteps = 16;
constexpr int kZ64FineWave = 64 * kZ64FineSteps;
struct Z64FineArgs {
  Z64Args z;
// ... 49 lines not shown
```

quantum_inferno_amd/csrc/qi_plan_build.hip:

```cpp
#include <algorithm>

#include "qi_host.hpp"

using namespace qi;

namespace qi {
namespace host {

bool native_len_ok(int64_t Lf) { return Lf == (1ll << 20) || Lf == (1ll << 21); }

bool native_wanted(const qi_plan* p, int kind) {
  if (p->d.engine == QI_ENGINE_HIPFFT) return false;
  const int64_t Lf = kind == 0 ? p->L : p->n;
  if (p->d.dtype == QI_F64 && !p->native_f64) return false;
  if (is_pow2(p->n) && native_len_ok(Lf)) return true;
  return kind != 1 && is_pow2(p->n) && p->n >= ((int64_t)1 << p->native_min_log2n) && Lf <= (1ll << 26);
}

bool z64_table(const qi_plan* p, int table) { return p->d.dtype == QI_F64 && p->native_z64 && table != 3; }
int64_t narrow_limit(const qi_plan* p, int table, int64_t Lf) {
  return z64_table(p, table) ? std::max<int64_t>(p->native_kmax, Lf >> (9 - p->native_z64_levels)) : p->native_kmax;
}

int batch_from(const qi_plan* p) {
  if (p->native_blk_batch_from > 0) return p->native_blk_batch_from;
  const int32_t rows = std::max(p->blk[0].ready ? p->blk[0].rows : 0, p->blk[2].ready ? p->blk[2].rows : 0);
  return rows <= 24 ? 8 : 4;
}

int64_t support_len(const double* sup) {
  const int64_t lo = (int64_t)sup[1], hi = (int64_t)sup[2];
  return hi >= lo ? hi - lo + 1 : 0;
}
double support_bits(const qi_plan* p) { return p->d.dtype == QI_F64 ? 50.0 : 30.0; }
double drop_bits(bool f64) { return f64 ? 52.0 : 30.0; }

int zoom_class(const qi_plan* p, int table, int64_t Lf, int64_t len) {
  if (!p->native_zoom || table == 3 || len <= 0 || Lf % native::kZoomD != 0) return -1;
  const int64_t M0 = Lf / native::kZoomD;
  if (!is_pow2(M0)) return -1;
  int g_min = 0;
  while ((M0 << g_min) < native::kBlk) ++g_min;
  for (int g = g_min; g < native::kZoomLevels; ++g) {
    if (p->n % ((int64_t)native::kZoomD * native::zoom_steps(g) * 4) != 0) return -1;
    if (native::kZoomOversample * len <= (M0 << g)) {
      if (g > p->native_zoom_max_level && native_len_ok(Lf)) return -1;
      if (g == 0 && p->native_zoom_short) {
        if ((int64_t)native::zoom_design_oversampling(6) * len <= M0) return 6;
        if ((int64_t)native::zoom_design_oversampling(5) * len <= M0) return 5;
      }
      return g;
    }
  }
  return -1;
}

int z64_level(const qi_plan* p, int table, int64_t Lf, int64_t len) {
  if (!z64_table(p, table) || len <= 0 || len > narrow_limit(p, table, Lf)) return -1;
  for (int g = 0; g < p->native_z64_levels; ++g)
    if (4 * len <= ((Lf / 64) << g)) return g;
  return -1;
}
bool z64_level_for_block(const qi_plan* p, int level) { return level >= p->native_z64_block_from; }

int band_mode(const qi_plan* p, int table, int64_t Lf, int64_t len) {
  const int zc = zoom_class(p, table, Lf, len);
  if (zc >= 0) return 2 + zc;
  return len > 0 && len <= narrow_limit(p, table, Lf) ? 0 : 1;
}

struct BlockPick {
  int32_t band;
  int wq;
  int64_t shift;
  int analytic = 0;
  double kappa = 0.0, cw = 0.0, amp = 0.0;
};
int block_group_of(double reach) { return reach <= 256.0 ? 1 : (reach <= 512.0 ? 2 : (reach <= 1024.0 ? 4 : 0)); }
void gabor_gaussian(BlockPick& pk, double p_re, double om, double am) {
  pk.kappa = om * (double)native::kBlk / (2.0 * M_PI);
  pk.cw = (2.0 * M_PI / (double)native::kBlk) * std::sqrt(M_LOG2E / (4.0 * p_re));
  pk.amp = am * std::sqrt(M_PI / p_re) / (double)native::kBlk;
}
void stx_gaussian(BlockPick& pk, int64_t n, double sigma) {
  pk.kappa = (double)pk.shift * (double)native::kBlk / (double)n;
  pk.cw = (2.0 * M_PI / (double)native::kBlk) * sigma * std::sqrt(M_LOG2E / 2.0);
  pk.amp = 1.0 / (double)native::kBlk;
}

double2 unit_root(int64_t m, int64_t N, bool negative) {
  const long double two_pi = 6.283185307179586476925286766559005768L;
  const long double ang = (negative ? -two_pi : two_pi) * (long double)(((m % N) + N) % N) / (long double)N;
  return make_double2((double)cosl(ang), (double)sinl(ang));
}

int upload_zoom_list(qi_plan* p, qi_plan::NativeTable& t, int64_t Lf, std::vector<native::BandDesc>& bands) {
  std::vector<native::BandDesc> rest;
  std::vector<std::vector<native::BandDesc>> by_level(native::kZoomClasses);
  for (const auto& d : bands) {
    if (d.mode >= 2) by_level[d.mode - 2].push_back(d);
    else rest.push_back(d);
  }
  auto join = [&](int from, int to) {
    by_level[to].insert(by_level[to].begin(), by_level[from].begin(), by_level[from].end());
    by_level[from].clear();
  };
  if (!by_level[6].empty() && by_level[6].size() < 6) join(6, 5);
  if (!by_level[5].empty() && by_level[5].size() < 6) join(5, 0);
  for (int g = 0; g + 1 < native::kZoomLevels; ++g) {
    if (by_level[g].empty() || by_level[g].size() >= 6) continue;
    for (int h = g + 1; h <= g + 2 && h < native::kZoomLevels; ++h)
      if (!by_level[h].empty()) {
        join(g, h);
        break;
      }
  }
  std::vector<native::BandDesc> zoom;
  t.h_zoom.clear();
  t.zoom_planes = 0;
  t.zoom_max_level = 0;
  for (int g = 0; g < native::kZoomClasses; ++g) t.zoom_count[g] = (int32_t)by_level[g].size();
  for (int gi = 0; gi < native::kZoomClasses; ++gi) {
    const int g = kZoomListOrder[gi];
    const int grid = native::zoom_grid(g);
    for (auto d : by_level[g]) {
      d.edge_slot = grid;
      d.edge = (int32_t)t.zoom_planes;
      t.zoom_planes += ((Lf / native::kZoomD) << grid) / native::kBlk;
      if (grid > t.zoom_max_level) t.zoom_max_level = grid;
      zoom.push_back(d);
      t.h_zoom.push_back({d.out_band, g});
    }
  }
  bands.swap(rest);
  if (zoom.empty()) return QI_OK;
  QI_TRY(upload_table(&t.d_zoom, zoom));
  t.nzoom = (int32_t)zoom.size();
  std::vector<int32_t> owner((size_t)t.zoom_planes);
  for (size_t j = 0; j < zoom.size(); ++j) {
    const int64_t planes = ((Lf / native::kZoomD) << zoom[j].edge_slot) / native::kBlk;
    for (int64_t q = 0; q < planes; ++q) owner[(size_t)(zoom[j].edge + q)] = (int32_t)j;
  }
  QI_TRY(upload_table(&t.d_zoom_plane_band, owner));
  for (int g = 0; g < native::kZoomClasses; ++g) {
    const bool needed = t.zoom_count[g] > 0 || (g == 0 && t.zoom_count[5] + t.zoom_count[6] > 0);
    if (p->d_zoom_w[g] || !needed) continue;
    std::vector<float> w((size_t)64 * native::zoom_taps(g));
    native::zoom_weights(g, 0, w.data());
    QI_TRY(upload_table(&p->d_zoom_w[g], w));
  }
  return QI_OK;
}

int order_z64_fine_classes(qi_plan* p, qi_plan::NativeTable& t, int64_t Lf, std::vector<std::vector<native::BandDesc>>& lvl) {
  const int64_t M0 = Lf / 64;
  std::vector<std::vector<native::BandDesc>> cls(native::kZ64FineClasses);
  for (const auto& d : lvl[0]) {
    int c = 0;
    for (int q = native::kZ64FineClasses - 1; q >= native::kZ64FineLevels && c == 0; --q)
      if ((int64_t)native::z64f_oversampling(q) * d.k_len <= M0) c = q;
    cls[c].push_back(d);
  }
  for (int q = native::kZ64FineClasses - 1; q >= native::kZ64FineLevels; --q) {
    if (cls[q].empty() || cls[q].size() >= 4) continue;
    const int to = q == native::kZ64FineLevels ? 0 : q - 1;
    cls[to].insert(cls[to].end(), cls[q].begin(), cls[q].end());
    cls[q].clear();
  }
  lvl[0].clear();
  int32_t pos = 0;
  std::vector<int> order0{0};
  for (int c = native::kZ64FineLevels; c < native::kZ64FineClasses; ++c) order0.push_back(c);
  for (int c : order0) {
    t.zf_first[c] = pos;
    t.zf_count[c] = (int32_t)cls[c].size();
    pos += t.zf_count[c];
    lvl[0].insert(lvl[0].end(), cls[c].begin(), cls[c].end());
  }
  for (int g = 1; g < native::kZ64FineLevels && g < native::kZ64Levels; ++g) {
    t.zf_first[g] = pos;
    t.zf_count[g] = (int32_t)lvl[g].size();
    pos += t.zf_count[g];
  }
  for (int c = 0; c < native::kZ64FineClasses; ++c) {
    if (t.zf_count[c] == 0 || p->d_z64f_w[c]) continue;
    std::vector<double> w((size_t)native::z64f_win(c) * 64);
    native::z64_fine_weights(c, w.data());
    QI_TRY(upload_table(&p->d_z64f_w[c], w));
  }
  return QI_OK;
}

int upload_z64_carriers(qi_plan::NativeTable& t, int kind, int64_t Lf, const std::vector<native::BandDesc>& z) {
  const int e = kind == 0 ? 1 : 0;
  std::vector<double2> lane(z.size() * 65);
  for (size_t j = 0; j < z.size(); ++j) {
    const int64_t kc = (int64_t)z[j].k_lo + z[j].k_len / 2;
    for (int l = 0; l < 64; ++l) lane[j * 65 + l] = unit_root(kc * (l - e), Lf, false);
    lane[j * 65 + 64] = unit_root(kc * 64, Lf, false);
  }
  const int64_t nw = Lf / native::kZ64FineWave;
  std::vector<double2> wave((size_t)nw);
  for (int64_t j = 0; j < nw; ++j) wave[(size_t)j] = unit_root(j * native::kZ64FineWave, Lf, false);
// ... 11 lines not shown
  }
  for (int c = 0; c < native::kZ64FineClasses; ++c) t.zf_first[c] = t.zf_count[c] = 0;
  if (p->native_z64_fine) QI_TRY(order_z64_fine_classes(p, t, Lf, lvl));
  std::vector<native::BandDesc> z;
  for (int g = 0; g < native::kZ64Levels; ++g) {
    t.z64_first[g] = (int32_t)z.size();
    t.z64_count[g] = (int32_t)lvl[g].size();
    z.insert(z.end(), lvl[g].begin(), lvl[g].end());
    if (!lvl[g].empty() && !p->d_z64_w[g]) {
      const int log2d = 6 - g;
      std::vector<double> w((size_t)(1 << log2d) * native::kZ64Taps);
      native::z64_weights(log2d, w.data());
      QI_TRY(upload_table(&p->d_z64_w[g], w));
    }
  }
  t.nz64 = (int32_t)z.size();
  t.h_z64.clear();
  for (const auto& d : z) t.h_z64.push_back(d.out_band);
  if (!z.empty()) QI_TRY(upload_table(&t.d_z64, z));
  if (!z.empty() && p->native_z64_fine && kind != 2) QI_TRY(upload_z64_carriers(t, kind, Lf, z));
  if (tune_env("QI_NATIVE_VERBOSE")) {
    fprintf(stderr, "[qi plan] table %d: float64 zoom bands per level %d %d %d %d %d, two-pass bands %zu; fine classes (taps: bands)", kind,
            t.z64_count[0], t.z64_count[1], t.z64_count[2], t.z64_count[3], t.z64_count[4], rest.size());
    for (int c = 0; c < native::kZ64FineClasses; ++c)
      fprintf(stderr, " %d@L%d: %d", native::z64f_ntap(c), native::z64f_level(c), t.zf_count[c]);
    fprintf(stderr, "\n");
  }
  bands.swap(rest);
  return QI_OK;
}

int upload_two_pass_groups(qi_plan* p, qi_plan::NativeTable& t, int64_t Lf, const std::vector<native::BandDesc>& bands) {
  t.h_rows.clear();
  t.h_row_mode.clear();
  for (const auto& d : bands) {
    t.h_rows.push_back(d.out_band);
    t.h_row_mode.push_back(d.mode == 1 ? 1 : 0);
  }
  t.Lf = Lf;
  if (bands.empty()) {
    t.ready = true;
    return QI_OK;
  }
  std::vector<int32_t> wide, narrow;
  for (size_t j = 0; j < bands.size(); ++j) (bands[j].mode == 1 ? wide : narrow).push_back((int32_t)j);
  const int32_t per = p->native_group > 0 ? p->native_group : (int32_t)wide.size();
  const int32_t ngroups = wide.empty() ? 1 : (int32_t)ceil_div((int64_t)wide.size(), per);
  std::vector<native::BandDesc> ordered;
  std::vector<int32_t> gen;
  t.groups.clear();
  size_t wi = 0, ni = 0;
  for (int32_t g = 0; g < ngroups; ++g) {
    qi_plan::NativeGroup grp;
    grp.first = (int32_t)ordered.size();
    grp.gen_first = (int32_t)gen.size();
    int32_t slot = 0;
    for (int32_t q = 0; q < per && wi < wide.size(); ++q, ++wi) {
      native::BandDesc d = bands[wide[wi]];
      d.gen_slot = slot++;
      gen.push_back((int32_t)ordered.size() - grp.first);
      ordered.push_back(d);
    }
    const size_t share = (narrow.size() * (size_t)(g + 1)) / (size_t)ngroups;
    for (; ni < share; ++ni) ordered.push_back(bands[narrow[ni]]);
    grp.count = (int32_t)ordered.size() - grp.first;
    grp.ngen = (int32_t)gen.size() - grp.gen_first;
    if (grp.count > 0) t.groups.push_back(grp);
  }
  QI_TRY(upload_table(&t.d_bands, ordered));
  if (!gen.empty()) QI_TRY(upload_table(&t.d_gen_list, gen));
  t.nbands = (int32_t)bands.size();
  t.ngen = (int32_t)wide.size();
  t.imd_slots = wide.empty() ? 0 : (per < (int32_t)wide.size() ? per : (int32_t)wide.size());
  t.ready = true;
  return QI_OK;
}

int upload_native_table(qi_plan* p, int kind, int64_t Lf, std::vector<native::BandDesc> bands) {
  auto& t = p->nat[kind];
  if (tune_env("QI_NATIVE_VERBOSE"))
    for (const auto& d : bands)
      fprintf(stderr, "[qi plan] table %d (Lf = %lld) band %d: %s, support [%d, +%d)\n", kind, (long long)Lf, d.out_band,
              d.mode == 0 ? "one-pass loader" : (d.mode == 1 ? "two-pass" : "zoom"), d.k_lo, d.k_len);
  QI_TRY(upload_zoom_list(p, t, Lf, bands));
  if (z64_table(p, kind)) QI_TRY(upload_z64_list(p, t, kind, Lf, bands));
  return upload_two_pass_groups(p, t, Lf, bands);
}

int analyse_support(qi_plan* p, int circular, int64_t L, int32_t B, int32_t j0, int32_t count, const double* d_par,
                    std::vector<double>* sup, hipStream_t st, double taper_e = 0.0) {
#ifdef QI_HOST_SANITIZE
  (void)st;
  (void)circular;
  const double bits = support_bits(p);
  sup->assign((size_t)count * 3, 0.0);
  for (int32_t q = 0; q < count; ++q) {
    const double p_re = d_par[j0 + q], om = d_par[2 * (int64_t)B + j0 + q];
    const double kc = om * (double)L / (2.0 * M_PI), hw = std::sqrt(4.0 * p_re * bits * M_LN2) * (double)L / (2.0 * M_PI);
    const bool cut = p_re * 0.25 * (double)p->n * (double)p->n <= bits * M_LN2;
    double lo = 0.0, hi = (double)(L - 1);
    if (!cut || taper_e > 0.0) {
      const double extra = cut ? (p->d.dtype == QI_F64 ? 13.2 : 6.6) * (double)L / taper_e : 0.0;
      lo = std::floor(kc - hw - extra);
      hi = std::ceil(kc + hw + extra);
      if (hi - lo + 1.0 >= (double)L) {
        lo = 0.0;
        hi = (double)(L - 1);
      }
    }
    (*sup)[3 * (size_t)q] = 1.0;
    (*sup)[3 * (size_t)q + 1] = lo;
    (*sup)[3 * (size_t)q + 2] = hi;
  }
  return QI_OK;
#endif
  const size_t row64 = (size_t)L * sizeof(double2);
  int64_t chunk = (int64_t)((p->ws_bytes - 4096) / row64);
  if (chunk < 1) {
    set_error("workspace too small to build one bank row (%zu bytes needed)", row64);
    return QI_ERR_NOMEM;
  }
  double2* rows = reinterpret_cast<double2*>(p->ws);
  DeviceTemp<double> d_sup;
  QI_HIP(hipMalloc((void**)&d_sup.ptr, (size_t)count * 3 * sizeof(double)));
  const double thr2 = std::ldexp(1.0, -2 * (int)support_bits(p));
  for (int32_t q = 0; q < count; q += (int32_t)chunk) {
    const int nbk = (count - q < chunk) ? count - q : (int)chunk;
    QI_TRY(launch_bank_rows(rows, p->n, L, circular, d_par, d_par + B, d_par + 2 * B, d_par + 3 * B, j0 + q, nbk, st, taper_e));
    QI_TRY(fft_c2c<double>(p->fft, rows, L, nbk, HIPFFT_FORWARD, st));
    QI_TRY(native::launch_band_support(rows, L, nbk, thr2, d_sup.ptr + (size_t)q * 3, st));
  }
  sup->assign((size_t)count * 3, 0.0);
  if (hipStreamSynchronize(st) != hipSuccess ||
      hipMemcpy(sup->data(), d_sup.ptr, sup->size() * sizeof(double), hipMemcpyDeviceToHost) != hipSuccess) {
    set_error("support analysis failed: %s", hipGetErrorString(hipGetLastError()));
    return QI_ERR_HIP;
  }
  return QI_OK;
}

template <typename T>
int fill_native_bank(qi_plan* p, int table, int circular, int64_t L, int32_t B, const std::vector<int32_t>& ids,
                     const std::vector<native::BandDesc>& bands, const double* d_par, hipStream_t st) {
  auto& t = p->nat[table];
  const size_t row64 = (size_t)L * sizeof(double2);
  int64_t chunk = (int64_t)((p->ws_bytes - 4096) / row64);
  double2* rows = reinterpret_cast<double2*>(p->ws);
  size_t q = 0;
  while (q < ids.size()) {
    size_t r = q + 1;
    const bool tapered = bands[q].add_row != 0;
    while (r < ids.size() && ids[r] == ids[r - 1] + 1 && (int64_t)(r - q) < chunk && (bands[r].add_row != 0) == tapered) ++r;
    const int nbk = (int)(r - q);
    QI_TRY(launch_bank_rows(rows, p->n, L, circular, d_par, d_par + B, d_par + 2 * B, d_par + 3 * B, ids[q], nbk, st,
                            tapered ? (double)p->native_split_e : 0.0));
    QI_TRY(fft_c2c<double>(p->fft, rows, L, nbk, HIPFFT_FORWARD, st));
    for (int jj = 0; jj < nbk; ++jj) {
      const native::BandDesc& d = bands[q + jj];
      if (d.mode != 1) {
        const bool zoomed = d.mode >= 2 || z64_level(p, table, L, d.k_len) >= 0;
        const double ramp = zoomed && !circular ? -1.0 / (double)L : 0.0;
        QI_TRY(native::launch_copy_window<T>(rows + (int64_t)jj * L, static_cast<cplx<T>*>(t.Hc) + d.src_off, d.k_lo,
                                              d.k_len, circular, 1.0 / (double)L, L, st, ramp, d.k_len / 2));
      }
      else
        QI_TRY(native::launch_copy_window<T>(rows + (int64_t)jj * L,
                                              static_cast<cplx<T>*>(t.Hfull) + (int64_t)d.bank_row * L, 0, L, circular,
// ... 615 lines not shown
```

quantum_inferno_amd/csrc/qi_run.hip:

```cpp
#include "qi_host.hpp"

using namespace qi;

namespace qi {
namespace host {



struct Tile {
  int64_t Ct, Bt, ntb, nblk;
  size_t off_x, off_y, off_pb, off_ps;
};

template <typename T>
int plan_tiles(const qi_plan* p, int64_t C, int64_t B, int64_t L, Tile* t) {
  const size_t row = (size_t)L * sizeof(cplx<T>);
  const int64_t nblk = ceil_div(p->n, kEpiSpan);
  const size_t part = align_up((size_t)B * nblk * 8) + align_up((size_t)B * nblk * 24);
  const size_t per_chan_full = row * (size_t)(B + 1) + part + 2048;
  int64_t Ct, Bt;
  if (per_chan_full <= p->ws_bytes) {
    Bt = B;
    Ct = (int64_t)(p->ws_bytes / per_chan_full);
    if (Ct > C) Ct = C;
// ... 335 lines not shown
  TwoPass tp;
  tp.subs.push_back({&p->nat[kind], kind, 0, 0, {}});
  tp.shorts = kind == 0 && p->nat[3].ready && p->nedge > 0;
  if (tp.shorts) tp.subs.push_back({&p->nat[3], 1, 0, 0, {}});
  for (auto& sb : tp.subs) {
    sb.N1 = sb.t->Lf / native::kN2;
    sb.nblk = sb.N1 / G;
    if (sb.nblk > tp.nblk_max) tp.nblk_max = sb.nblk;
    if ((int64_t)sb.t->imd_slots * sb.t->Lf > tp.imd_elems) tp.imd_elems = (int64_t)sb.t->imd_slots * sb.t->Lf;
    for (const auto& grp : sb.t->groups) {
      int nc = (int)ceil_div(p->native_wgs, sb.nblk * C);
      if (nc < 1) nc = 1;
      if (nc > grp.count) nc = grp.count;
      sb.nchunk.push_back(nc);
      tp.chunk_total += nc;
    }
  }
  return tp;
}

template <typename T>
struct Scratch {
  cplx<T>* X;
  cplx<T>* Xn;
  cplx<T>* imd;
  cplx<T>* zoom;
  cplx<T>* zadd;
  char* parts0;
  size_t parts_bytes;
  double* part_band;
  double* part_stat;
  T* time_part;
  T* edge_p;
  T* edge_time;
  cplx<T>* edge_z;
};
struct ScratchBytes {
  size_t x = 0, xn = 0, imd = 0, zoom = 0, add = 0, pb = 0, ps = 0, tp = 0, ep = 0, et = 0, ez = 0;
  size_t per_record() const { return x + xn + imd + zoom + add + pb + ps + tp + ep + et + ez; }
};
template <typename T>
ScratchBytes scratch_bytes(const qi_plan* p, int64_t n, int64_t B, int64_t nbk, int64_t stat_slots, int chunk_total, bool shorts,
                           bool time_via_part, bool panel, int32_t nsplit) {
  ScratchBytes e;
  e.xn = shorts ? (size_t)n * sizeof(cplx<T>) : 0;
  e.pb = (size_t)B * nbk * 8;
  e.ps = (size_t)stat_slots * 24;
  e.tp = time_via_part ? (size_t)chunk_total * n * sizeof(T) : 0;
  e.ep = shorts ? (size_t)p->nedge * 2 * p->edge_wmax * sizeof(T) : 0;
  e.et = shorts ? (size_t)2 * p->edge_wmax * sizeof(T) : 0;
  e.ez = shorts && !panel ? (size_t)p->nedge * 2 * p->edge_wmax * sizeof(cplx<T>) : 0;
  e.add = (size_t)nsplit * n * sizeof(cplx<T>);
  return e;
}

struct Arena {
  const qi_plan* p;
  char* w;
  int64_t Ct;
  const char* what;
  bool shared_first;
  template <typename U>
  U* carve(size_t bytes) {
    char* r = w;
    w += align_up(bytes * Ct);
    QI_LAYOUT_NOTE(p, what, r, bytes * Ct, shared_first);
    shared_first = false;
    return reinterpret_cast<U*>(r);
  }
  template <typename T>
  void carve_reductions(const ScratchBytes& e, Scratch<T>* s) {
    s->parts0 = w;
    s->part_band = carve<double>(e.pb);
    s->part_stat = carve<double>(e.ps);
    s->parts_bytes = (size_t)(w - s->parts0);
    s->time_part = carve<T>(e.tp);
    s->edge_p = carve<T>(e.ep);
    s->edge_time = carve<T>(e.et);
    s->edge_z = e.ez ? carve<cplx<T>>(e.ez) : nullptr;
  }
};

template <typename T>
int launch_spectra(qi_plan* p, const T* sig, int64_t n, int64_t Lf, bool shorts, bool have_spectra, const Scratch<T>& s,
                   int64_t ct, hipStream_t st) {
  p->prof.begin(st, QI_STAGE_FORWARD);
  if (have_spectra) {
  } else if (p->native_fwd && native_len_ok(Lf)) {
    native::RowArgs<T> f{};
    f.Lf = Lf;
    f.n = n;
    f.N1 = Lf / native::kN2;
    f.N2 = native::kN2;
    f.imd_slots = 1;
    f.imd = s.imd;
    f.sig = sig;
    f.two_over_len = (float)(2.0 / (double)Lf);
    f.debug = 0;
    QI_TRY(native::launch_forward<T>(f, s.X, ct, st));
  } else {
    QI_TRY(launch_pack_pad<T>(sig, s.X, ct, n, Lf, st));
    QI_TRY(fft_c2c<T>(p->fft, s.X, Lf, ct, HIPFFT_FORWARD, st));
  }
  if (shorts) QI_TRY(native::launch_even_bins<T>(s.X, s.Xn, ct, n, st));
  p->prof.end(QI_STAGE_FORWARD, st);
  return QI_OK;
}

template <typename T>
int launch_two_pass(qi_plan* p, const TwoPass& tp, const TileOut<T>& v, const Scratch<T>& s, int G, int64_t stat_nblk,
                    bool diag, int64_t ct, hipStream_t st) {
  int chunk_base = 0;
  for (size_t si = 0; si < tp.subs.size(); ++si) {
    const Sub& sb = tp.subs[si];
    const auto& t = *sb.t;
    native::RowArgs<T> a{};
    a.Lf = t.Lf;
    a.n = v.n;
    a.N1 = sb.N1;
    a.N2 = native::kN2;
    a.panel_bands = (int32_t)v.B;
    a.imd_slots = t.imd_slots;
    a.X = si == 0 ? s.X : s.Xn;
    a.Hc = static_cast<const cplx<T>*>(t.Hc);
    a.Hfull = static_cast<const cplx<T>*>(t.Hfull);
    a.imd = s.imd;
    a.inv_len = (T)(1.0 / (double)t.Lf);
    a.two_over_len = (float)(2.0 / (double)t.Lf);
    if (diag) {
      a.debug = p->native_debug;
      a.stamps = p->stamps;
    }
    a.neg_last_row = sb.kernel_kind == 0 ? 1 : 0;
    a.edge_z = s.edge_z;
    a.edge_wmax = p->edge_wmax;
    a.nedge = p->nedge;
    v.fill(a);
    a.stat_nblk = stat_nblk;
    for (size_t g = 0; g < t.groups.size(); ++g) {
      const auto& grp = t.groups[g];
      a.bands = t.d_bands + grp.first;
      a.nbands = grp.count;
      a.gen_list = t.d_gen_list ? t.d_gen_list + grp.gen_first : nullptr;
      a.ngen_launch = grp.ngen;
      a.chunk_base = chunk_base;
      if (grp.ngen > 0) {
        p->prof.begin(st, QI_STAGE_PASS1);
        QI_TRY(native::launch_pass1<T>(a, sb.kernel_kind, ct, st));
        p->prof.end(QI_STAGE_PASS1, st);
      }
      p->prof.begin(st, QI_STAGE_PASS2);
      QI_TRY(native::launch_pass2<T>(a, sb.kernel_kind, G, sb.nchunk[g], ct, st));
      p->prof.end(QI_STAGE_PASS2, st);
      chunk_base += sb.nchunk[g];
    }
  }
  return QI_OK;
}

template <typename T>
native::BlockArgs<T> block_args(const qi_plan* p, const qi_plan::BlockTable& bt, const qi_plan::BlockTable::ItemList& il,
                                const TileOut<T>& v, const T* sig, cplx<T>* zadd, int32_t nsplit, int64_t stat_base,
                                int chunk_base) {
  native::BlockArgs<T> b{};
  b.n = v.n;
  b.nitems = il.nitems;
  b.nedge_items = il.nedge_items;
  b.edge_merged = il.edge_merged ? 1 : 0;
  b.nsplit = nsplit;
  b.edge_band = p->d_split_bands;
  b.edge_bank = static_cast<const cplx<T>*>(p->split_bank);
  b.edge_part = zadd;
  b.panel_bands = (int32_t)v.B;
  b.items = il.d_items;
  b.bands = static_cast<const native::BlockBandT<T>*>(il.d_bands);
  b.bank = static_cast<const cplx<T>*>(bt.bank);
  b.sig = sig;
  v.fill(b);
  b.stat_base = stat_base;
  b.chunk_base = chunk_base;
  b.two_over_n = (float)(2.0 / (double)v.n);
  b.debug = p->native_debug;
// ... 64 lines not shown
  for (int g = 0; g < NL; ++g) r.count[g] = zt.zoom_count[g];
  if (C < p->native_zoom_short_from) {
    r.count[0] += r.count[5] + r.count[6];
    r.count[5] = r.count[6] = 0;
  }
  if (zt.nzoom <= 0) return r;
  const double level_cost[NL] = {1.0, 1.08, 1.25, 0.75, 1.0, 0.85, 0.75};
  int64_t wgs = 0;
  for (int g = 0; g < NL; ++g) {
    if (r.count[g] <= 0) continue;
    r.groups[g] = native::zoom_groups(n, g);
    r.nchunk[g] = 1;
    wgs += r.groups[g] * C;
  }
  const int64_t zoom_wgs = p->native_zoom_wgs > 0 ? p->native_zoom_wgs : (joint && p->native_fuse > 3 ? p->native_zoom_wgs_joint : 0);
  if (zoom_wgs > 0) {
    for (;;) {
      int best = -1;
      double best_load = 0.0;
      for (int g = 0; g < NL; ++g) {
        if (r.count[g] <= 0 || r.nchunk[g] >= r.count[g]) continue;
        const double load = level_cost[g] * (double)ceil_div(r.count[g], r.nchunk[g]);
        if (load > best_load) {
          best_load = load;
          best = g;
        }
      }
      if (best < 0 || wgs + r.groups[best] * C > zoom_wgs) break;
      bool is_max = true;
      for (int g = 0; g < NL; ++g)
        if (r.count[g] > 0 && level_cost[g] * (double)ceil_div(r.count[g], r.nchunk[g]) > best_load) is_max = false;
      if (!is_max) break;
      r.nchunk[best] += 1;
      wgs += r.groups[best] * C;
    }
  } else {
    for (int g = 0; g < NL; ++g) {
      if (r.count[g] <= 0) continue;
      int nc = (int)ceil_div(p->native_zoom_waves, 4 * r.groups[g] * C);
      if (nc < 1) nc = 1;
      if (nc > r.count[g]) nc = r.count[g];
      r.nchunk[g] = nc;
    }
  }
  for (int g = 0; g < NL; ++g) {
    if (r.count[g] <= 0) continue;
    r.planes += r.nchunk[g];
    r.stat_base[g] = r.stats;
    r.stats += (int64_t)r.nchunk[g] * r.groups[g];
    if (r.groups[g] > r.slots) r.slots = r.groups[g];
  }
  if (tune_env("QI_NATIVE_VERBOSE"))
    fprintf(stderr, "[qi run] zoom launch of table %d: bands per class %d %d %d %d %d | 6-tap %d 4-tap %d in rows %d %d %d %d %d | %d %d\n", kind,
            r.count[0], r.count[1], r.count[2], r.count[3], r.count[4], r.count[5],
            r.count[6], r.nchunk[0], r.nchunk[1], r.nchunk[2], r.nchunk[3], r.nchunk[4], r.nchunk[5], r.nchunk[6]);
  return r;
}

int upload_band_slots(qi_plan* p, int kind, int cut, int64_t nblk_max, bool blocks) {
  if (p->d_band_slots[kind][cut]) return QI_OK;
  std::vector<int32_t> slots((size_t)p->nat[kind].nbands, 0);
  for (int32_t r : p->nat[kind].h_rows) slots[r] = (int32_t)nblk_max;
  for (const auto& z : p->nat[kind].h_zoom) slots[z.first] = (int32_t)native::zoom_groups(p->n, z.second);
  if (blocks)
    for (const auto& b : p->blk[kind].var[cut].h_bands) slots[b.first] = b.second;
  return upload_table(&p->d_band_slots[kind][cut], slots);
}

native::ZoomArgs<float> zoom_args(const qi_plan* p, int kind, const ZoomRows& r, const TileOut<float>& v, const Scratch<float>& s,
                                  bool x_shift, int32_t nsplit, int64_t stat_base, int chunk_base) {
  using T = float;
  const auto& zt = p->nat[kind];
  const int64_t n = v.n;
  native::ZoomArgs<T> z{};
  z.n = n;
  z.Lf = zt.Lf;
  z.planes = zt.zoom_planes;
  z.nbands = zt.nzoom;
  z.panel_bands = (int32_t)v.B;
  z.bands = zt.d_zoom;
  z.plane_band = zt.d_zoom_plane_band;
  z.X = s.X;
  z.x_shift = x_shift ? 1 : 0;
  z.Hc = static_cast<const cplx<T>*>(zt.Hc);
  z.coarse = s.zoom;
  z.stx = kind == 2 ? 1 : 0;
  z.lane_off = kind == 0 ? 1 : 0;
  z.tau_off = kind == 2 ? 0 : n / 2 / native::kZoomD;
  z.inv_len = (T)(1.0 / (double)zt.Lf);
  z.two_over_len = (float)(2.0 / (double)zt.Lf);
  v.fill(z);
  z.chunk_base = chunk_base;
  z.split_part = s.zadd;
  z.split_rows = nsplit;
  z.debug = p->native_debug;
  int chunk0 = 0;
  for (int g = 0; g < native::kZoomClasses; ++g) {
    z.lvl_count[g] = r.count[g];
    z.lvl_chunk0[g] = chunk0;
    z.lvl_nchunk[g] = r.nchunk[g];
    z.lvl_stat_base[g] = stat_base + r.stat_base[g];
    z.lvl_weights[g] = p->d_zoom_w[g];
    chunk0 += r.nchunk[g];
  }
  int first = 0;
  for (int gi = 0; gi < native::kZoomClasses; ++gi) {
    const int g = kZoomListOrder[gi];
    z.lvl_first[g] = first;
    first += r.count[g];
    if (g == 0 && r.count[0] != zt.zoom_count[0]) z.lvl_first[0] = 0;
  }
  return z;
}

int launch_zoom_stage(qi_plan* p, const native::ZoomArgs<float>& z, int max_level, FusedCarry* defer, FusedCarry* finish,
                      int64_t ct, hipStream_t st) {
  using T = float;
  if (defer) {
    defer->zoom = z;
    defer->has_zoom = true;
    defer->ct = ct;
    return QI_OK;
  }
  const bool joint = finish && finish->has_zoom && finish->ct == ct;
  p->prof.begin(st, QI_STAGE_ZOOM_COARSE);
  const bool gfused = p->native_gather_fused > 0 && ct >= p->native_gather_fused;
  if (joint && gfused) {
    QI_TRY(native::launch_zoom_coarse_gather2<T>(finish->zoom, z, ct, st));
  } else if (joint) {
    QI_TRY(native::launch_zoom_gather2<T>(finish->zoom, z, ct, st));
    QI_TRY(native::launch_zoom_coarse2<T>(finish->zoom, z, ct, st));
  } else if (gfused) {
    QI_TRY(native::launch_zoom_coarse_gather<T>(z, ct, st));
  } else {
    QI_TRY(native::launch_zoom_gather<T>(z, max_level, ct, st));
    QI_TRY(native::launch_zoom_coarse<T>(z, max_level, ct, st));
  }
  p->prof.end(QI_STAGE_ZOOM_COARSE, st);
  p->prof.begin(st, QI_STAGE_ZOOM);
  const bool joint_fine = joint && p->native_fuse > 3 && (finish->zoom.coef != nullptr) == (z.coef != nullptr) &&
                          (finish->zoom.bits != nullptr) == (z.bits != nullptr);
  if (joint_fine) {
    QI_TRY(native::launch_zoom2<T>(finish->zoom, z, ct, st));
  } else {
    if (joint) QI_TRY(native::launch_zoom<T>(finish->zoom, ct, st));
    QI_TRY(native::launch_zoom<T>(z, ct, st));
  }
  if (joint) finish->has_zoom = false;
  p->prof.end(QI_STAGE_ZOOM, st);
  return QI_OK;
}

int launch_block_stage(qi_plan* p, const native::BlockArgs<float>& b, int demod, int cut, FusedCarry* defer, FusedCarry* finish,
                       int64_t ct, hipStream_t st) {
  using T = float;
  if (defer) {
    defer->blk = b;
    defer->demod = demod;
    defer->ct = ct;
    return QI_OK;
  }
  const bool joint = finish && p->native_fuse > 1 && finish->ct == ct && !finish->demod && demod &&
                     (finish->blk.coef != nullptr) == (b.coef != nullptr) && (finish->blk.bits != nullptr) == (b.bits != nullptr);
  p->prof.unchain_span();
  p->prof.begin(st, QI_STAGE_BLOCK);
  if (joint) {
    QI_TRY(build_dual_items(p, cut));
    QI_TRY(native::launch_block_dual<T>(finish->blk, b, p->d_dual[cut], p->n_dual[cut], p->n_dual_long[cut],
                                        p->blk[0].var[cut].nedge_items, ct, st));
  } else {
    if (finish) QI_TRY(native::launch_block<T>(finish->blk, finish->demod, finish->ct, st));
    QI_TRY(native::launch_block<T>(b, demod, ct, st));
  }
  p->prof.end(QI_STAGE_BLOCK, st);
  p->prof.unchain_span();
  return QI_OK;
}

int launch_tails(FusedCarry* finish, const native::TailCall<float>& tc, hipStream_t st) {
  finish->active = false;
  const native::TailCall<float>& t0 = finish->tail;
  if (t0.ct == tc.ct && t0.n == tc.n) return native::launch_tail2<float>(t0, tc, st);
  QI_TRY(native::launch_tail<float>(t0, st));
  return native::launch_tail<float>(tc, st);
}

template <typename T>
int run_native(qi_plan* p, int kind, const void* sig_v, int64_t C, const qi_tfr_out* out, hipStream_t st, bool may_share,
               FusedCarry* defer, FusedCarry* finish, size_t* probe) {
  static_assert(std::is_same<T, float>::value, "the native engine is float32");
  const int64_t n = p->n, B = p->nat[kind].nbands, Lf0 = p->nat[kind].Lf;
  const T* sig = static_cast<const T*>(sig_v);
  const int G = p->native_rows;
  const TwoPass tp = plan_two_pass(p, kind, C, G);
  const bool shorts = tp.shorts;
  const int chunk_p2 = tp.chunk_total;
  int chunk_total = chunk_p2;
  const auto& bt = p->blk[kind];
  const bool blocks = kind != 1 && bt.ready;
  const int cut = C >= batch_from(p) ? 1 : 0;
  const auto& il = bt.var[cut];
  int64_t blk_stats = 0, blk_slots = 0;
  if (blocks) {
    chunk_total += il.nplanes;
    blk_stats = il.nitems + il.nedge_items;
    blk_slots = bt.max_blocks;
  }
  const auto& zt = p->nat[kind];
  const bool zoom = zt.nzoom > 0;
  const ZoomRows zr = plan_zoom_rows(p, kind, C, defer || (finish && (finish->active || probe)));
  const int chunk_z0 = chunk_total;
  chunk_total += zr.planes;
  int64_t nbk = tp.nblk_max + (shorts ? 1 : 0);
  if (blk_slots > nbk) nbk = blk_slots;
  if (zr.slots > nbk) nbk = zr.slots;
  const int64_t p2_stats = (int64_t)chunk_p2 * tp.nblk_max;
  const int64_t stat_slots = p2_stats + blk_stats + zr.stats + (shorts ? p->nedge : 0);
  const bool sums = out->power_band || out->stats;
  const bool time_via_part = out->power_time && (chunk_total > 1 || shorts);
  if (!shorts) QI_TRY(upload_band_slots(p, kind, cut, tp.nblk_max, blocks));
  const int32_t* band_slots = shorts ? nullptr : p->d_band_slots[kind][cut];
  bool share = may_share && kind == 2 && (probe || (p->shared_valid && p->shared_sig == sig_v && p->shared_C == C)) &&
               p->nat[kind].h_rows.empty() && !shorts;
  const int32_t nsplit = kind == 0 ? p->nsplit : 0;
  ScratchBytes e = scratch_bytes<T>(p, n, B, nbk, stat_slots, chunk_total, shorts, time_via_part, out->coef != nullptr, nsplit);
  e.x = (size_t)(share ? 2 * Lf0 : Lf0) * sizeof(cplx<T>);
  e.imd = (size_t)(tp.imd_elems < Lf0 ? Lf0 : tp.imd_elems) * sizeof(cplx<T>);
  e.zoom = zoom ? (size_t)zt.zoom_planes * native::kBlk * sizeof(cplx<T>) : 0;
  const size_t per_chan = e.per_record();
  if (probe) {
    *probe = per_chan;
    return QI_OK;
  }
  if (p->ws_bytes < per_chan + 4096) {
    set_error("workspace of %zu bytes cannot hold one record's native scratch of %zu bytes", p->ws_bytes,
              per_chan + 4096);
    return QI_ERR_NOMEM;
  }
  int64_t Ct = (int64_t)((p->ws_bytes - 4096) / per_chan);
  if (Ct > C) Ct = C;
  if (share && Ct != C) {
    set_error("internal: shared spectra need all records in one tile");
    return QI_ERR_STATE;
  }
  const bool tail_one = time_via_part && sums && p->native_tail;
  const bool deferring = defer && kind == 0 && Ct == C && blocks && !shorts && tail_one;
  bool finishing = finish && finish->active && kind == 2 && share && blocks && tail_one;
  if (finishing) {
    const size_t need = align_up(e.x * (size_t)C) + align_up(finish->ws_used) + (per_chan - e.x) * (size_t)C + 64 * 256;
    if (need > p->ws_bytes) finishing = false;
  }
  if (finish && finish->active && !finishing) QI_TRY(flush_carry(p, finish, st));
  if (kind == 0) {
    p->shared_valid = Ct == C;
    p->shared_sig = sig_v;
    p->shared_C = C;
  } else if (!share) {
    p->shared_valid = false;
  }
  QI_LAYOUT_BEGIN(p, kind == 0 ? "run_native styx" : (kind == 1 ? "run_native atoms" : "run_native stx"), finishing);
  Arena ar{p, p->ws, Ct, "native scratch", share};
  Scratch<T> s{};
  s.X = ar.carve<cplx<T>>(e.x);
  if (finishing) ar.w = p->ws + align_up(finish->ws_used);
  s.Xn = ar.carve<cplx<T>>(e.xn);
  s.imd = ar.carve<cplx<T>>(e.imd);
  ar.carve_reductions(e, &s);
  s.zoom = e.zoom ? ar.carve<cplx<T>>(e.zoom) : nullptr;
  s.zadd = e.add ? ar.carve<cplx<T>>(e.add) : nullptr;
  for (int64_t c0 = 0; c0 < C; c0 += Ct) {
    const int64_t ct = (C - c0 < Ct) ? C - c0 : Ct;
    const T* sig_t = sig + c0 * n;
    const TileOut<T> v = tile_out<T>(out, c0, B, n, time_via_part ? s.time_part : nullptr, s.part_band, s.part_stat, nbk,
                                     stat_slots, chunk_total);
    if (shorts) QI_HIP(hipMemsetAsync(s.parts0, 0, s.parts_bytes, st));
    QI_TRY(launch_spectra<T>(p, sig_t, n, Lf0, shorts, share, s, ct, st));
    QI_TRY(launch_two_pass<T>(p, tp, v, s, G, tp.nblk_max, true, ct, st));
    if (zoom)
      QI_TRY(launch_zoom_stage(p, zoom_args(p, kind, zr, v, s, share, nsplit, p2_stats + blk_stats, chunk_z0), zt.zoom_max_level,
                               deferring && p->native_fuse > 2 ? defer : nullptr, finishing ? finish : nullptr, ct, st));
    if (finishing && finish->has_zoom) {
      QI_TRY(launch_zoom_all(p, finish->zoom, finish->ct, st));
      finish->has_zoom = false;
    }
    if (blocks) {
      native::BlockArgs<T> b = block_args<T>(p, bt, il, v, sig_t, s.zadd, nsplit, p2_stats, chunk_p2);
      b.nlong = il.nlong;
      QI_TRY(launch_block_stage(p, b, bt.demod, cut, deferring ? defer : nullptr, finishing ? finish : nullptr, ct, st));
    }
    p->prof.begin(st, QI_STAGE_EPILOGUE);
    if (shorts) QI_TRY(launch_edges<T>(p, v, s, sig_t, ct, st));
    native::TailCall<T> tc = tail_call<T>(v, ct, band_slots);
    if (deferring) {
      defer->tail = tc;
      defer->ws_used = (size_t)(ar.w - p->ws);
      defer->active = true;
    } else if (finishing) {
      QI_TRY(launch_tails(finish, tc, st));
    } else {
      tc.edge_time = shorts ? s.edge_time : nullptr;
      tc.wmax = p->edge_wmax;
      QI_TRY(launch_reductions<T>(tc, time_via_part, p->native_tail != 0, st));
    }
    p->prof.end(QI_STAGE_EPILOGUE, st);
  }
  return QI_OK;
}


struct Z64Rows {
  bool fine = false;
  int zchunk[native::kZ64Levels] = {};
  int frow[native::kZ64FineClasses] = {};
  size_t z_off[native::kZ64Levels] = {};
  size_t bytes = 0;
  int chunks = 0;
};

Z64Rows plan_z64_rows(const qi_plan* p, const qi_plan::NativeTable& t, int64_t C) {
  using T = double;
  const int64_t n = p->n, Lf = t.Lf;
  Z64Rows r;
  for (int c = 0; c < native::kZ64FineClasses; ++c) r.fine = r.fine || t.zf_count[c] > 0;
  const int64_t tiles_f = n / ((int64_t)native::kZ64FineWave * 4);
  for (int g = 0; g < native::kZ64Levels; ++g) {
    if (t.z64_count[g] == 0) continue;
    r.z_off[g] = r.bytes / sizeof(cplx<T>);
    r.bytes += (size_t)t.z64_count[g] * (size_t)(((Lf / 64) << g) + 2 * native::kZ64Pad) * sizeof(cplx<T>);
    if (r.fine && g < native::kZ64FineLevels) continue;
    int nc = (int)ceil_div(p->native_wgs, (n / native::kZ64Tile) * C);
    r.zchunk[g] = nc < 1 ? 1 : (nc > t.z64_count[g] ? t.z64_count[g] : nc);
    r.chunks += r.zchunk[g];
  }
  for (int c = 0; c < native::kZ64FineClasses; ++c) {
    if (t.zf_count[c] == 0) continue;
    double work = 0.0, mine = (double)t.zf_count[c] * (2.0 * native::z64f_win(c) + 40.0);
    for (int q = 0; q < native::kZ64FineClasses; ++q) work += (double)t.zf_count[q] * (2.0 * native::z64f_win(q) + 40.0);
    const double want_rows = std::max<double>((double)p->native_z64_rows, (double)p->native_wgs / (double)(tiles_f * C));
    int nr = (int)std::ceil(want_rows * (mine / work));
    r.frow[c] = nr < 1 ? 1 : (nr > t.zf_count[c] ? t.zf_count[c] : nr);
    r.chunks += r.frow[c];
  }
  return r;
}

int launch_z64_stage(qi_plan* p, int kind, const Z64Rows& r, const TileOut<double>& v, const Scratch<double>& s, int32_t nsplit,
                     int64_t stat_nblk, int chunk_base, int64_t ct, hipStream_t st) {
  using T = double;
  const auto& t = p->nat[kind];
  const int64_t n = v.n, Lf = t.Lf;
  native::Z64Args zl[native::kZ64Levels];
  for (int g = 0; g < native::kZ64Levels; ++g) {
    if (t.z64_count[g] == 0) continue;
    native::Z64Args& z = zl[g];
    z = native::Z64Args{};
    z.Lf = Lf;
    z.n = n;
    z.log2d = 6 - g;
    z.M = Lf >> z.log2d;
// ... 50 lines not shown
    zl[g].chunk_base = chunk_base;
    QI_TRY(native::launch_z64_interp(zl[g], r.zchunk[g], ct, st));
    chunk_base += r.zchunk[g];
  }
  p->prof.end(QI_STAGE_ZOOM, st);
  return QI_OK;
}

int launch_block64(qi_plan* p, native::BlockArgs<double> b, const qi_plan::BlockTable& bt,
                   const qi_plan::BlockTable::ItemList& il, int64_t ct, hipStream_t st) {
  using T = double;
  if (b.nsplit <= 0) b.nedge_items = 0;
  b.edge_wq = (int32_t)(p->native_split_e / 512);
  b.gauss_w = static_cast<const T*>(il.d_gauss_w);
  b.demod_pow = static_cast<const cplx<T>*>(il.d_demod_pow);
  b.demod_t1 = p->d_demod_t1;
  b.demod_t2 = p->d_demod_t2;
  p->prof.begin(st, QI_STAGE_BLOCK);
  if (b.nedge_items > 0 && !p->side) {
    QI_HIP(hipStreamCreateWithFlags(&p->side, hipStreamNonBlocking));
    QI_HIP(hipEventCreateWithFlags(&p->ev_fork, hipEventDisableTiming));
    QI_HIP(hipEventCreateWithFlags(&p->ev_join, hipEventDisableTiming));
  }
  QI_TRY(native::launch_block<T>(b, bt.demod, ct, st, p->side, p->ev_fork, p->ev_join));
  p->prof.end(QI_STAGE_BLOCK, st);
  return QI_OK;
}

int run_native64(qi_plan* p, int kind, const void* sig_v, int64_t C, const qi_tfr_out* out, hipStream_t st) {
  using T = double;
  const auto& t = p->nat[kind];
  const int64_t n = p->n, B = kind == 2 ? p->nb_stx : p->nb[kind], Lf = t.Lf;
  constexpr int G = 8;
  const T* sig = static_cast<const T*>(sig_v);
  const TwoPass tp = plan_two_pass(p, kind, C, G);
  const bool shorts = tp.shorts;
  const Z64Rows zr = plan_z64_rows(p, t, C);
  const int64_t nblk_z = zr.fine ? n / native::kZ64FineWave : n / native::kZ64Tile;
  int64_t nblk = tp.subs[0].nblk > nblk_z ? tp.subs[0].nblk : nblk_z;
  const auto& bt = p->blk[kind];
  const bool blocks = kind != 1 && bt.ready;
  if (blocks && bt.max_blocks > nblk) nblk = bt.max_blocks;
  const bool clear_parts = shorts || tp.subs[0].nblk != nblk || blocks;
  const auto& il = bt.var[C >= 4 ? 1 : 0];
  const int chunk_blk = tp.chunk_total + zr.chunks;
  const int chunk_total = chunk_blk + (blocks ? il.nplanes : 0);
  const int64_t blk_stats = blocks ? il.nitems + il.nedge_items : 0;
  const int32_t nsplit = kind == 0 && blocks ? p->nsplit : 0;
  const int64_t blk_stat_base = (int64_t)chunk_blk * nblk;
  const int64_t stat_slots = blk_stat_base + blk_stats + (shorts ? p->nedge : 0);
  if (chunk_total == 0) {
    set_error("float64 native table has no band");
    return QI_ERR_STATE;
  }
  const bool time_via_part = out->power_time && (chunk_total > 1 || shorts);
  const int64_t nbk = nblk + (shorts ? 1 : 0);
  ScratchBytes e = scratch_bytes<T>(p, n, B, nbk, stat_slots, chunk_total, shorts, time_via_part, out->coef != nullptr, nsplit);
  e.x = (size_t)Lf * sizeof(cplx<T>);
  e.imd = (size_t)(p->native_fwd && native_len_ok(Lf) && tp.imd_elems < Lf ? Lf : tp.imd_elems) * sizeof(cplx<T>);
  e.zoom = zr.bytes;
  const size_t per_chan = e.per_record();
  if (p->ws_bytes < per_chan + 16384) {
    set_error("workspace of %zu bytes cannot hold one record's float64 scratch of %zu bytes", p->ws_bytes, per_chan + 16384);
    return QI_ERR_NOMEM;
  }
  int64_t Ct = (int64_t)((p->ws_bytes - 16384) / per_chan);
  if (Ct > C) Ct = C;
  p->shared_valid = false;
  QI_LAYOUT_BEGIN(p, kind == 2 ? "run_native64 stx" : "run_native64 gabor", false);
  Arena ar{p, p->ws, Ct, "native64 scratch", false};
  Scratch<T> s{};
  s.X = ar.carve<cplx<T>>(e.x);
  s.Xn = ar.carve<cplx<T>>(e.xn);
  s.imd = ar.carve<cplx<T>>(e.imd);
  s.zoom = ar.carve<cplx<T>>(e.zoom);
  s.zadd = e.add ? ar.carve<cplx<T>>(e.add) : nullptr;
  ar.carve_reductions(e, &s);
  for (int64_t c0 = 0; c0 < C; c0 += Ct) {
    const int64_t ct = (C - c0 < Ct) ? C - c0 : Ct;
    const T* sig_t = sig + c0 * n;
    const TileOut<T> v = tile_out<T>(out, c0, B, n, time_via_part ? s.time_part : nullptr, s.part_band, s.part_stat, nbk,
                                     stat_slots, chunk_total);
    if (clear_parts) QI_HIP(hipMemsetAsync(s.parts0, 0, s.parts_bytes, st));
    QI_TRY(launch_spectra<T>(p, sig_t, n, Lf, shorts, false, s, ct, st));
    QI_TRY(launch_two_pass<T>(p, tp, v, s, G, nblk, false, ct, st));
    QI_TRY(launch_z64_stage(p, kind, zr, v, s, nsplit, nblk, tp.chunk_total, ct, st));
    if (blocks)
      QI_TRY(launch_block64(p, block_args<T>(p, bt, il, v, sig_t, s.zadd, nsplit, blk_stat_base, chunk_blk), bt, il, ct, st));
    p->prof.begin(st, QI_STAGE_EPILOGUE);
    if (shorts) QI_TRY(launch_edges<T>(p, v, s, sig_t, ct, st));
    native::TailCall<T> tc = tail_call<T>(v, ct, nullptr);
    tc.edge_time = shorts ? s.edge_time : nullptr;
    tc.wmax = p->edge_wmax;
    QI_TRY(launch_reductions<T>(tc, time_via_part, true, st));
    p->prof.end(QI_STAGE_EPILOGUE, st);
    p->prof.unchain();
  }
  return QI_OK;
}

template int run_transform<float>(qi_plan*, Kind, const void*, int64_t, const qi_tfr_out*, hipStream_t);
template int run_transform<double>(qi_plan*, Kind, const void*, int64_t, const qi_tfr_out*, hipStream_t);
template int run_native<float>(qi_plan*, int, const void*, int64_t, const qi_tfr_out*, hipStream_t, bool, FusedCarry*, FusedCarry*,
                               size_t*);

}
}
```

quantum_inferno_amd/csrc/qi_zoom.hip:

```cpp
#include "qi_common.hpp"
#include "qi_device.hpp"
#include "qi_native.hpp"
#include "qi_fft_reg.hpp"
#include "qi_zoom_gather.hpp"

namespace qi {
namespace native {

namespace {

constexpr int kZoomThreads = 256;

__device__ __forceinline__ float lane_value(float v, int lane) {
  return __uint_as_float(__builtin_amdgcn_readlane(__float_as_uint(v), lane));
}

template <typename T, bool STX>
__device__ __forceinline__ void zoom_gather_plane(const ZoomArgs<T>& a, const uint32_t plane) {
  const BandDesc bd = load_uniform(a.bands + *as_const(a.plane_band + plane));
  const int32_t kappa0 = (int32_t)(blockIdx.x * 256 + threadIdx.x);
  const uint32_t tau1 = plane - (uint32_t)bd.edge;
  const int64_t ch = blockIdx.z;
  const cplx<T>* __restrict__ X = a.X + ch * (a.Lf << a.x_shift);
  a.coarse[((int64_t)ch * a.planes + bd.edge) * kBlk + (int32_t)tau1 * kBlk + kappa0] =
      zoom_gather_value<T, STX>(a, bd, tau1, kappa0, X);
}
template <typename T, bool STX>
__global__ void __launch_bounds__(256) k_zoom_gather(ZoomArgs<T> a) {
  zoom_gather_plane<T, STX>(a, blockIdx.y);
}
template <typename T>
__global__ void __launch_bounds__(256) k_zoom_gather2(ZoomArgs<T> a0, ZoomArgs<T> a2) {
  if (blockIdx.y < (uint32_t)a0.planes) zoom_gather_plane<T, false>(a0, blockIdx.y);
  else zoom_gather_plane<T, true>(a2, blockIdx.y - (uint32_t)a0.planes);
}

template <typename T, int LEVEL, bool PHASOR, bool COEF, bool BITS, bool SDESC>
__device__ __forceinline__ void zoom_level(const ZoomArgs<T>& a, int chunk, int row, double (*s_red)[kZoomThreads / kWave],
                                           double (*s_fin)[kZoomThreads / kWave]) {
  constexpr int NW = kZoomThreads / kWave, S = zoom_span(LEVEL), TAPS = zoom_taps(LEVEL), STEPS = zoom_steps(LEVEL);
  if ((int64_t)blockIdx.x >= a.n / ((int64_t)kZoomD * STEPS * NW)) return;
  const int nchunk = a.lvl_nchunk[LEVEL];
  const float* __restrict__ weights = a.lvl_weights[LEVEL];
  constexpr int GRID = zoom_grid(LEVEL), HALF = zoom_ntap(LEVEL) / 2 - 1;
  constexpr int WIN = (STEPS - 1) * S + TAPS;
  static_assert(WIN <= 2 * kWave, "the window of one wave must fit two registers of its lanes");
  constexpr bool TWO = WIN > kWave;
  const int tid = threadIdx.x, lane = tid & (kWave - 1), wv = tid / kWave;
  const int64_t ch = blockIdx.z;
  const int64_t gw = (int64_t)blockIdx.x * NW + wv;
  const uint32_t step_a = (uint32_t)gw * STEPS;
  const uint32_t mmask = (uint32_t)((a.Lf / kZoomD) << GRID) - 1u, lmask = (uint32_t)a.Lf - 1u;
  const int plog2 = ilog2((int)(((a.Lf / kZoomD) << GRID) / kBlk));
  float wgt[TAPS];
#pragma unroll
  for (int j = 0; j < TAPS; ++j) wgt[j] = weights[j * kWave + lane];
  T colp[STEPS];
#pragma unroll
  for (int s = 0; s < STEPS; ++s) colp[s] = T(0);
  T mx = T(0);
  double plogp = 0.0;
  const uint32_t t_base = step_a * kZoomD + (uint32_t)lane;
  int par = 0;

  const uint32_t wtau = ((uint32_t)S * (step_a + (uint32_t)a.tau_off) - (uint32_t)HALF + (uint32_t)lane) & mmask;
  const uint32_t widx = (wtau & ((1u << plog2) - 1u)) * (uint32_t)kBlk + (wtau >> plog2);
  const uint32_t wtau2 = (wtau + (uint32_t)kWave) & mmask;
  const uint32_t widx2 = (wtau2 & ((1u << plog2) - 1u)) * (uint32_t)kBlk + (wtau2 >> plog2);
  const int jj0 = a.lvl_first[LEVEL] + chunk, jj_end = a.lvl_first[LEVEL] + a.lvl_count[LEVEL];
  cplx<T> smp_next = mk<T>(T(0), T(0)), smq_next = mk<T>(T(0), T(0));
  const BandDesc* first_bd = a.bands + (jj0 < jj_end ? jj0 : a.lvl_first[LEVEL]);
  BandDesc bd_next = SDESC ? load_uniform(first_bd) : *first_bd;
  if (jj0 < jj_end) {
    const cplx<T>* __restrict__ b = a.coarse + ((int64_t)ch * a.planes + bd_next.edge) * kBlk;
    smp_next = b[widx];
    if (TWO) smq_next = b[widx2];
  }
  for (int jj = jj0; jj < jj_end; jj += nchunk) {
    const BandDesc bd = bd_next;
    const cplx<T> smp = smp_next, smq = smq_next;
    if (jj + nchunk < jj_end) {
      bd_next = SDESC ? load_uniform(a.bands + jj + nchunk) : a.bands[jj + nchunk];
      const cplx<T>* __restrict__ b = a.coarse + ((int64_t)ch * a.planes + bd_next.edge) * kBlk;
      smp_next = b[widx];
      if (TWO) smq_next = b[widx2];
    }
    cplx<T> P = mk<T>(T(1), T(0)), Q = mk<T>(T(1), T(0));
    if (PHASOR) {
      const uint32_t kc = (uint32_t)(bd.k_lo + bd.k_len / 2);
      double c, s;
      unit_root((kc * (uint32_t)(lane - a.lane_off)) & lmask, a.two_over_len, &c, &s);
      P = mk<T>((T)c, (T)s);
      unit_root((kc * kZoomD * (step_a + (uint32_t)a.tau_off + (uint32_t)lane)) & lmask, a.two_over_len, &c, &s);
      Q = mk<T>((T)c, (T)s);
    }
    const int64_t orow = ((int64_t)ch * a.panel_bands + bd.out_band) * a.n;
    const bool part = bd.add_row != 0;
    char* __restrict__ coef_row = reinterpret_cast<char*>(
        part ? a.split_part + ((int64_t)ch * a.split_rows + (bd.add_row - 1)) * a.n : (a.coef ? a.coef + orow : nullptr));
    char* __restrict__ bits_row = reinterpret_cast<char*>(a.bits ? a.bits + orow : nullptr);
    const T pscale = part ? T(0) : a.power_scale;
    uint32_t tb = t_base;
    asm volatile("" : "+v"(tb));
    T rowacc = T(0), pl = T(0);
    T zr[STEPS], zi[STEPS];
    {
// ... 262 lines not shown
```

quantum_inferno_amd/csrc/qi_zoom_gather.hpp:

```cpp
#pragma once
#include "qi_common.hpp"
#include "qi_device.hpp"
#include "qi_native.hpp"

namespace qi {
namespace native {
namespace {

template <typename T, bool STX>
__device__ __forceinline__ cplx<T> zoom_gather_value(const ZoomArgs<T>& a, const BandDesc& bd, const uint32_t tau1,
                                                     const int32_t kappa0, const cplx<T>* __restrict__ X) {
  const int32_t M = (int32_t)((a.Lf / kZoomD) << bd.edge_slot), P = M / kBlk;
  const int32_t kc = STX ? 0 : bd.k_lo + bd.k_len / 2;
  const int32_t ks_lo = bd.k_lo - kc, ks_hi = ks_lo + bd.k_len;
  const uint32_t lmask = (uint32_t)a.Lf - 1u;
  cplx<T> acc = mk<T>(T(0), T(0));
  const int32_t ks0 = ks_lo + ((kappa0 - ks_lo) & (kBlk - 1));
  if (ks0 >= ks_hi) return acc;
  for (int32_t ks = ks0; ks < ks_hi; ks += kBlk) {
    const uint32_t r = ((uint32_t)ks & ((uint32_t)M - 1u)) / kBlk;
    const int32_t k = kc + ks;
    cplx<T> y;
    if (STX) {
      const cplx<T> x = X[((uint32_t)(k + (int32_t)bd.shift) & lmask) << a.x_shift];
      const T g0 = (T)bd.coef * (T)k;
      const T g = exp2_t(-g0 * g0) * a.inv_len;
      y = mk<T>(x.x * g, x.y * g);
    } else {
      y = cmul(X[((uint32_t)k & lmask) << a.x_shift], a.Hc[bd.src_off + (k - bd.k_lo)]);
    }
    float sr, cr;
    sincospif(2.0f * (float)((r * tau1) & (uint32_t)(P - 1)) / (float)P, &sr, &cr);
    const cplx<T> t = cmul(y, mk<T>((T)cr, (T)sr));
    acc.x += t.x;
    acc.y += t.y;
  }
  float s, c;
  sincospif(2.0f * (float)(((uint32_t)kappa0 * tau1) & ((uint32_t)M - 1u)) / (float)M, &s, &c);
  return cmul(acc, mk<T>((T)c, (T)s));
}

template <typename T, bool STX, int NF = 8>
__device__ __forceinline__ void zoom_gather16(const ZoomArgs<T>& a, const BandDesc& bd, const uint32_t tau1, const int col,
                                              const cplx<T>* __restrict__ X, cplx<T> (&v)[16]) {
  const int32_t M = (int32_t)((a.Lf / kZoomD) << bd.edge_slot), P = M / kBlk;
  const int32_t kc = STX ? 0 : bd.k_lo + bd.k_len / 2;
  const int32_t ks_lo = bd.k_lo - kc, ks_hi = ks_lo + bd.k_len;
  const uint32_t lmask = (uint32_t)a.Lf - 1u;
  const int nterm = (bd.k_len + kBlk - 1) / kBlk;
  int32_t ks0[16];
#pragma unroll
  for (int b = 0; b < 16; ++b) {
    v[b] = mk<T>(T(0), T(0));
    ks0[b] = ks_lo + (((col + 256 * b) - ks_lo) & (kBlk - 1));
  }
  const uint32_t r_a = ((uint32_t)ks_lo & ((uint32_t)M - 1u)) / kBlk;
  const uint32_t edge = (((uint32_t)ks_lo & ((uint32_t)M - 1u)) | (uint32_t)(kBlk - 1)) + 1u;
  float sf, cf;
  sincospif(2.0f * (float)((r_a * tau1) & (uint32_t)(P - 1)) / (float)P, &sf, &cf);
  cplx<T> w_a = mk<T>((T)cf, (T)sf);
  sincospif(2.0f * (float)(tau1 & (uint32_t)(P - 1)) / (float)P, &sf, &cf);
  const cplx<T> w_step = mk<T>((T)cf, (T)sf);
  cplx<T> w_b = cmul(w_a, w_step);
  const uint32_t base_mod = (uint32_t)ks_lo & ((uint32_t)M - 1u);
  for (int m = 0; m < nterm; ++m) {
#pragma unroll
    for (int hb = 0; hb < 16; hb += NF) {
      cplx<T> x[NF], h[NF];
      bool on[NF];
#pragma unroll
      for (int q = 0; q < NF; ++q) {
        const int b = hb + q;
        const int32_t ks = ks0[b] + kBlk * m;
        on[q] = ks < ks_hi;
        const int32_t k = kc + ks;
        x[q] = mk<T>(T(0), T(0));
        h[q] = mk<T>(T(0), T(0));
        if (on[q]) {
          if (STX) {
            x[q] = X[((uint32_t)(k + (int32_t)bd.shift) & lmask) << a.x_shift];
          } else {
            x[q] = X[((uint32_t)k & lmask) << a.x_shift];
            h[q] = a.Hc[bd.src_off + (k - bd.k_lo)];
          }
        }
      }
#pragma unroll
      for (int q = 0; q < NF; ++q) {
        const int b = hb + q;
        if (!on[q]) continue;
        cplx<T> y;
        if (STX) {
          const T g0 = (T)bd.coef * (T)(kc + ks0[b] + kBlk * m);
          const T g = exp2_t(-g0 * g0) * a.inv_len;
          y = mk<T>(x[q].x * g, x[q].y * g);
        } else {
          y = cmul(x[q], h[q]);
        }
        const bool second = base_mod + (uint32_t)(ks0[b] - ks_lo) >= edge;
        const cplx<T> t = cmul(y, second ? w_b : w_a);
        v[b].x += t.x;
        v[b].y += t.y;
      }
    }
    w_a = w_b;
    w_b = cmul(w_b, w_step);
  }
  sincospif(2.0f * (float)(((uint32_t)col * tau1) & ((uint32_t)M - 1u)) / (float)M, &sf, &cf);
  const cplx<T> e0 = mk<T>((T)cf, (T)sf);
  sincospif(2.0f * (float)((256u * tau1) & ((uint32_t)M - 1u)) / (float)M, &sf, &cf);
  const cplx<T> s1 = mk<T>((T)cf, (T)sf), s2 = cmul(s1, s1), s4 = cmul(s2, s2), s8 = cmul(s4, s4);
  cplx<T> pw[16];
  pw[0] = e0;
#pragma unroll
  for (int b = 1; b < 16; ++b) {
    const int low = b & -b;
    pw[b] = cmul(pw[b - low], low == 1 ? s1 : (low == 2 ? s2 : (low == 4 ? s4 : s8)));
  }
#pragma unroll
  for (int b = 0; b < 16; ++b) v[b] = cmul(v[b], pw[b]);
}

}
}
}
```

quantum_inferno_amd/engine.py:

```python
import collections
import ctypes as C
import os
import threading
from dataclasses import dataclass
from typing import Optional

import numpy as np
import torch

from . import _lib
from . import scales_dyadic as scales

_EPI_SPAN = 1024


def _real_dtype(dtype):
    if dtype in (torch.float32, np.float32, "float32", "f32"):
        return torch.float32
    if dtype in (torch.float64, np.float64, "float64", "f64", float):
        return torch.float64
    raise TypeError(f"unsupported dtype {dtype}: float32 or float64")


def _complex_of(rdtype):
# ... 90 lines not shown


class TfrPlan:

    def __init__(self, n, dtype=torch.float32, device=None, workspace_bytes=None, engine=_lib.QI_ENGINE_AUTO):
        self._lib = _lib.require_gpu()
        self.n = int(n)
        self.rdtype = _real_dtype(dtype)
        self.device = torch.device(device) if device is not None else default_device()
        if self.device.index is None:
            self.device = torch.device("cuda", torch.cuda.current_device())
        self.workspace_bytes = int(workspace_bytes) if workspace_bytes else 0
        self._handle = C.c_void_p()
        if os.environ.get("QI_FORCE_HIPFFT"):
            engine = _lib.QI_ENGINE_HIPFFT
        desc = _lib.PlanDesc(
            n=self.n,
            dtype=_lib.QI_F64 if self.rdtype == torch.float64 else _lib.QI_F32,
            device=self.device.index,
            engine=engine,
            flags=0,
            workspace_bytes=self.workspace_bytes,
        )
        _lib.check(self._lib.qi_plan_create(C.byref(self._handle), C.byref(desc)))
        self.freq = {}

    @staticmethod
    def workspace_for(n, n_bands, dtype, channels=1, cap_bytes=8 << 30):
        esz = 16 if _real_dtype(dtype) == torch.float64 else 8
        length = 2 * n if (n & (n - 1)) == 0 else 1 << (2 * n - 2).bit_length()
        nblk = -(-n // _EPI_SPAN)
        per_chan = (max(n_bands, 2) + 1) * length * esz + n_bands * nblk * 32 + 4096
        build = min(n_bands, 16) * length * 16
        need = max(per_chan * channels, build, 1 << 24)
        return int(min(max(need, per_chan), max(cap_bytes, per_chan)))

    def _stream(self):
        return _lib.stream_ptr(self.device)

    def set_gabor_bank(self, which, f_hz, p_re, p_im, omega, amp):
        keep = [_lib.darr(a) for a in (p_re, p_im, omega, amp)]
        with torch.cuda.device(self.device):
            _lib.check(
                self._lib.qi_plan_set_gabor_bank(
                    self._handle, which, len(keep[0][0]), keep[0][1], keep[1][1], keep[2][1], keep[3][1], self._stream()
                )
            )
        self.freq[which] = np.asarray(f_hz)

    def set_styx_bank(self, order, fs, dictionary_type="norm"):
        f_hz, p_re, p_im, omega, amp, _ = styx_bank_tables(order, self.n, fs, dictionary_type)
        self.set_gabor_bank(_lib.QI_BANK_STYX, f_hz, p_re, p_im, omega, amp)
        return f_hz

    def set_stx_bands(self, order, fs):
        f_hz = scales.log_frequency_hz_from_fft_points(fs, self.n, order)
        idx = scales.stx_shift_indices(f_hz, self.n, fs)
        sigma = scales.cycles_from_order(order) / (2 * np.pi * f_hz / fs)
        self.set_stx_table(f_hz, idx, sigma)
        return f_hz

    def set_stx_table(self, f_hz, shift_index, sigma):
        ia, ip = _lib.iarr(shift_index)
        sa, sp = _lib.darr(sigma)
        if len(ia) != len(sa):
            raise ValueError("shift_index and sigma must have one entry per band")
        _lib.check(self._lib.qi_plan_set_stx_bands(self._handle, len(ia), ip, sp))
        self.freq[_lib.QI_TABLE_STX] = np.asarray(f_hz)
        self.stx_index = ia

    def profile(self, enable=True, stages=None, period=1):
        code = 1 if enable else 0
        if enable and stages is not None:
            code = 0
            for name in stages:
                code |= 1 << (_lib.STAGES.index(name) + 1)
        if enable and period > 1:
            code |= int(period) << 16
        _lib.check(self._lib.qi_plan_profile(self._handle, code))

    def stage_bands(self, stage):
        k = _lib.STAGES.index(stage)
        return [int(self._lib.qi_plan_stage_bands(self._handle, which, k)) for which in (0, 1, 2)]

    def band_route(self, which, band, records=1):
        r = _lib.BandRoute()
        _lib.check(self._lib.qi_plan_band_route(self._handle, which, int(band), int(records), C.byref(r)))
        return _lib.STAGES[r.stage], r.cls, r.run_cls, r.flags

    def profile_read(self):
        ms = (C.c_double * len(_lib.STAGES))()
        cnt = (C.c_int64 * len(_lib.STAGES))()
        _lib.check(self._lib.qi_plan_profile_read(self._handle, ms, cnt, len(_lib.STAGES)))
        return {name: (ms[i], cnt[i]) for i, name in enumerate(_lib.STAGES)}

    def _signal(self, sig):
        if sig.dtype != self.rdtype or not sig.is_cuda or sig.device != self.device:
            sig = sig.to(device=self.device, dtype=self.rdtype)
        sig = sig.contiguous()
        if sig.dim() != 2 or sig.shape[1] != self.n:
            raise ValueError(f"signal must be [channels, {self.n}], got {tuple(sig.shape)}")
        return sig

    def _outputs(self, which, n_ch, coef, bits, reductions, power_scale, eps, out, reduced_out):
        f_hz = self.freq.get(which)
        if f_hz is None:
            raise _lib.QiError("band table not set on this plan")
        n_b = len(f_hz)
        dev = self.device
        if out is not None:
            res = out
            if (res.coef is not None and res.coef.shape[0] != n_ch) or (res.stats is not None and res.stats.shape[0] != n_ch):
                raise ValueError("out= buffers were made for another channel count")
            res.power_scale = power_scale
        else:
            res = TfrResult(frequency_hz=f_hz, power_scale=power_scale)
            if coef:
                res.coef = torch.empty((n_ch, n_b, self.n), dtype=_complex_of(self.rdtype), device=dev)
            if bits:
                res.bits = torch.empty((n_ch, n_b, self.n), dtype=self.rdtype, device=dev)
            if reductions:
                from .dist import reduced_slots

                slots = reduced_slots(n_ch, n_b, self.n, self.rdtype)
                if reductions == "band":
                    if reduced_out is not None:
                        raise ValueError('reductions="band" has no gather layout: reduced_out does not apply')
                    small = torch.empty(n_ch * (n_b + 4), dtype=torch.float64, device=dev)
                    res.power_band = small[: n_ch * n_b].view(n_ch, n_b)
                    res.stats = small[n_ch * n_b :].view(n_ch, 4)
                    slots = None
                elif reduced_out is not None:
                    if reduced_out.dtype != torch.float64 or reduced_out.numel() != slots or not reduced_out.is_contiguous():
                        raise ValueError(f"reduced_out must be a contiguous float64 tensor of {slots} elements")
                    res.reduced = reduced_out
                else:
                    res.reduced = torch.empty(slots, dtype=torch.float64, device=dev)
                if slots is not None:
                    o1 = res.reduced.numel() - n_ch * (n_b + 4)
                    o2 = o1 + n_ch * n_b
                    res.power_time = res.reduced[:o1].view(self.rdtype)[: n_ch * self.n].view(n_ch, self.n)
                    res.power_band = res.reduced[o1:o2].view(n_ch, n_b)
                    res.stats = res.reduced[o2:].view(n_ch, 4)
        desc = _lib.TfrOut(
            coef=_lib.ptr(res.coef),
            bits=_lib.ptr(res.bits),
            power_band=_lib.ptr(res.power_band),
            power_time=_lib.ptr(res.power_time),
            stats=_lib.ptr(res.stats),
            power_scale=float(power_scale),
            eps=float(eps),
        )
        return res, desc

    def _run(self, which, sig, coef, bits, reductions, power_scale, eps, out=None, reduced_out=None):
        sig = self._signal(sig)
        n_ch = sig.shape[0]
        res, desc = self._outputs(which, n_ch, coef, bits, reductions, power_scale, eps, out, reduced_out)
        with torch.cuda.device(self.device):
            if which == _lib.QI_TABLE_STX:
                rc = self._lib.qi_stx(self._handle, _lib.ptr(sig), n_ch, C.byref(desc), self._stream())
            else:
                rc = self._lib.qi_cwt(self._handle, which, _lib.ptr(sig), n_ch, C.byref(desc), self._stream())
        _lib.check(rc)
        return res

# ... 214 lines not shown
```

Measured before the change: 414,600 Mpoints/s.

## Compute only low-frequency forward FFT bins when zoom bands need them

Adds a pruned forward transform for f32 tables whose band supports all fall within a low-frequency window. The first pass writes only the rows needed for the low bins, and a new second-pass kernel produces just N2/2+1 rows into a compact wraparound buffer of 2*16*N1 bins. The zoom gather now indexes X through a mask sized to that buffer. This cuts forward-FFT work, intermediate memory traffic and scratch size. In exchange it adds eligibility logic and layout coupling between the forward and zoom stages, and it only applies when every table qualifies. tune_env also stops caching the QI_TUNE lookup.

```diff
diff --git a/include/qi_tfr.h b/include/qi_tfr.h
--- a/include/qi_tfr.h
+++ b/include/qi_tfr.h
@@ -75,6 +75,8 @@
 
 int64_t qi_plan_bands(const qi_plan* plan, int which );
 int64_t qi_plan_stage_bands(const qi_plan* plan, int which, int stage);
+
+int64_t qi_plan_forward_low(const qi_plan* plan, int which );
 
 typedef struct {
   int32_t stage, cls, run_cls, flags;
diff --git a/quantum_inferno_amd/_lib.py b/quantum_inferno_amd/_lib.py
--- a/quantum_inferno_amd/_lib.py
+++ b/quantum_inferno_amd/_lib.py
@@ -73,6 +73,7 @@
     "qi_plan_set_stx_bands": (_int, [_P, _i32, _I64, _D]),
     "qi_plan_bands": (_i64, [_P, _int]),
     "qi_plan_stage_bands": (_i64, [_P, _int, _int]),
+    "qi_plan_forward_low": (_i64, [_P, _int]),
     "qi_plan_band_route": (_int, [_P, _int, _i32, _i64, C.POINTER(BandRoute)]),
     "qi_plan_profile": (_int, [_P, _int]),
     "qi_plan_profile_read": (_int, [_P, _D, _I64, _i32]),
diff --git a/quantum_inferno_amd/csrc/qi_api.hip b/quantum_inferno_amd/csrc/qi_api.hip
--- a/quantum_inferno_amd/csrc/qi_api.hip
+++ b/quantum_inferno_amd/csrc/qi_api.hip
@@ -44,6 +44,7 @@
     p->native_kmax = (int64_t)native::kMaxPrunedTerms * native::kN2;
   if (const char* e = tune_env("QI_NATIVE_DEBUG")) p->native_debug = atoi(e);
   if (const char* e = tune_env("QI_NATIVE_FWD")) p->native_fwd = atoi(e);
+  if (const char* e = tune_env("QI_NATIVE_FWD_LOW")) p->native_fwd_low = atoi(e);
 #ifdef QI_NATIVE_STAMPS
   if (tune_env("QI_NATIVE_STAMPS")) {
     if (hipMalloc((void**)&p->stamps, 65536 * 8 * sizeof(unsigned long long)) != hipSuccess) p->stamps = nullptr;
@@ -304,6 +305,11 @@
   return which == 2 ? p->nb_stx : 0;
 }
 
+int64_t qi_plan_forward_low(const qi_plan* p, int which) {
+  if (!p || which < 0 || which > 2 || !forward_low(p)) return 0;
+  return table_low_bins(p, which);
+}
+
 int64_t qi_plan_stage_bands(const qi_plan* p, int which, int stage) {
   if (!p || which < 0 || which > 2) return 0;
   const int64_t total = qi_plan_bands(p, which);
diff --git a/quantum_inferno_amd/csrc/qi_block.hip b/quantum_inferno_amd/csrc/qi_block.hip
--- a/quantum_inferno_amd/csrc/qi_block.hip
+++ b/quantum_inferno_amd/csrc/qi_block.hip
@@ -1256,7 +1256,7 @@
   const BandDesc bd = load_uniform(a.bands + *as_const(a.plane_band + plane_i));
   const uint32_t tau1 = plane_i - (uint32_t)bd.edge;
   const int64_t ch = blockIdx.z;
-  const cplx<T>* __restrict__ X = a.X + ch * (a.Lf << a.x_shift);
+  const cplx<T>* __restrict__ X = a.X + ch * ((int64_t)a.x_mask + 1);
   cplx<T> v[16];
 #ifdef QI_NATIVE_DEBUG
   if (a.debug & 256) {
diff --git a/quantum_inferno_amd/csrc/qi_host.hpp b/quantum_inferno_amd/csrc/qi_host.hpp
--- a/quantum_inferno_amd/csrc/qi_host.hpp
+++ b/quantum_inferno_amd/csrc/qi_host.hpp
@@ -247,6 +247,7 @@
     std::vector<int32_t> h_row_mode;
     std::vector<int32_t> h_z64;
     int32_t nzoom = 0, zoom_count[native::kZoomClasses] = {0, 0, 0, 0, 0, 0, 0};
+    int64_t x_lo = 0, x_hi = -1;
     int64_t zoom_planes = 0;
     int zoom_max_level = 0;
     native::BandDesc* d_z64 = nullptr;
@@ -368,6 +369,7 @@
   int64_t native_kmax = 12288;
   int native_debug = 0;
   int native_fwd = 1;
+  int native_fwd_low = 1;
   int native_wgs = 256;
   unsigned long long* stamps = nullptr;
   unsigned long long* blk_stamps = nullptr;
@@ -395,6 +397,8 @@
 
 bool native_len_ok(int64_t Lf);
 bool native_wanted(const qi_plan* p, int kind);
+int64_t table_low_bins(const qi_plan* p, int kind);
+bool forward_low(const qi_plan* p);
 int batch_from(const qi_plan* p);
 void release_styx_extras(qi_plan* p);
 void drop_gabor_tables(qi_plan* p, int bank);
diff --git a/quantum_inferno_amd/csrc/qi_host_util.hip b/quantum_inferno_amd/csrc/qi_host_util.hip
--- a/quantum_inferno_amd/csrc/qi_host_util.hip
+++ b/quantum_inferno_amd/csrc/qi_host_util.hip
@@ -4,10 +4,7 @@
 
 static thread_local char g_err[512] = "";
 
-const char* tune_env(const char* name) {
-  static const bool on = std::getenv("QI_TUNE") != nullptr;
-  return on ? std::getenv(name) : nullptr;
-}
+const char* tune_env(const char* name) { return std::getenv("QI_TUNE") != nullptr ? std::getenv(name) : nullptr; }
 
 void set_error(const char* fmt, ...) {
   va_list ap;
diff --git a/quantum_inferno_amd/csrc/qi_native.hip b/quantum_inferno_amd/csrc/qi_native.hip
--- a/quantum_inferno_amd/csrc/qi_native.hip
+++ b/quantum_inferno_amd/csrc/qi_native.hip
@@ -268,8 +268,9 @@
 #endif
 }
 
-template <typename T, class C, int SRC, int NPH>
+template <typename T, class C, int SRC, int NPH, bool LOW = false>
 __global__ void __launch_bounds__(C::TH) k_pass1(RowArgs<T> a) {
+  static_assert(!LOW || SRC == 2, "the low-bins variant is the forward transform's");
   extern __shared__ __attribute__((aligned(16))) char smem[];
   cplx<T>* buf = reinterpret_cast<cplx<T>*>(smem);
   cplx<T>* tw = buf + C::BUF;
@@ -294,7 +295,8 @@
   const T* sigc = SRC == 2 ? a.sig + ch * a.n : nullptr;
   const uint32_t mask = (uint32_t)a.Lf - 1u;
   const uint32_t k2 = row0 + g2;
-  cplx<T>* __restrict__ dst = a.imd + ((int64_t)ch * a.imd_slots + bd.gen_slot) * a.Lf + k2;
+  cplx<T>* __restrict__ dst = LOW ? a.imd + (int64_t)ch * fwd_low_rows(a.N1) * kN2 + k2
+                                  : a.imd + ((int64_t)ch * a.imd_slots + bd.gen_slot) * a.Lf + k2;
   const uint32_t roll = a.neg_last_row ? 1u : 0u, cmask = (uint32_t)a.N1 - 1u;
 #ifdef QI_NATIVE_STAMPS
   unsigned long long st_acc[8] = {0, 0, 0, 0, 0, 0, 0, 0};
@@ -315,12 +317,13 @@
     unit_root_t<T>((k2 * (uint32_t)(NPH * (d2 + 16 * c2) + ph)) & mask, a.two_over_len, &wr, &wi);
     unit_root_t<T>((k2 * (uint32_t)(64 * NPH)) & mask, a.two_over_len, &sr, &si);
 #pragma unroll
-    for (int c1 = 0; c1 < 16; ++c1) {
+    for (int c1 = 0; c1 < (LOW ? 9 : 16); ++c1) {
       const cplx<T> z = u[brev(c1, 4)];
       const uint32_t t1 = (uint32_t)(NPH * (d2 + 16 * c2 + 64 * c1)) + (uint32_t)ph;
       if (c1 == 15 && a.neg_last_row && t1 == cmask)
         unit_root_t<T>((0u - k2) & mask, a.two_over_len, &wr, &wi);
       const T cr = (T)wr, ci = (T)wi;
+      if (LOW && c1 == 8 && t1 != (uint32_t)a.N1 / 2u) break;
       if (!QI_DBG(1)) dst[(size_t)((t1 + roll) & cmask) * kN2] = mk<T>(z.x * cr - z.y * ci, z.x * ci + z.y * cr);
       const double nr = wr * sr - wi * si;
       wi = wr * si + wi * sr;
@@ -356,6 +359,59 @@
     const cplx<T> z = u[brev(c1, 4)];
     dst[(size_t)c1 * tstep] = mk<T>(z.x, -z.y);
   }
+}
+
+template <typename T, class C>
+__global__ void __launch_bounds__(C::TH) k_fwd2_low(RowArgs<T> a, cplx<T>* __restrict__ Xlow) {
+  extern __shared__ __attribute__((aligned(16))) char smem[];
+  cplx<T>* buf = reinterpret_cast<cplx<T>*>(smem);
+  cplx<T>* tw = buf + C::BUF;
+  const int tid = threadIdx.x;
+  const int64_t ch = blockIdx.z;
+  const uint32_t row0 = blockIdx.x * C::G, half = (uint32_t)a.N1 / 2u;
+  const int g1 = tid / 64, a1 = tid % 64;
+  fill_step_twiddles<T, C>(tw);
+  cplx<T> v[16];
+  if (row0 + g1 <= half) {
+    load_imd_direct<T>(v, a.imd + ch * fwd_low_rows(a.N1) * kN2, row0 + g1, a1);
+  } else {
+#pragma unroll
+    for (int b = 0; b < 16; ++b) v[b] = mk<T>(T(0), T(0));
+  }
+  __syncthreads();
+  fft_reg<T, 16, 1>(v);
+#pragma unroll
+  for (int d = 1; d < 16; ++d) v[brev(d, 4)] = cmul(v[brev(d, 4)], tw[d * 64 + a1]);
+#pragma unroll
+  for (int d = 0; d < 16; ++d) buf[a1 * C::SA + d * C::G + g1] = v[brev(d, 4)];
+  __syncthreads();
+  if (tid >= C::TH / 2) return;
+  const int d2 = tid / (2 * C::G), sel = (tid / C::G) & 1, g2 = tid % C::G;
+  const uint32_t f1 = row0 + g2;
+  if (f1 > half) return;
+  const cplx<T>* __restrict__ col = buf + d2 * C::G + g2;
+  cplx<T> u[16];
+#pragma unroll
+  for (int q = 0; q < 16; ++q) {
+    const cplx<T> t0 = col[q * C::SA], t1 = col[(q + 16) * C::SA], t2 = col[(q + 32) * C::SA], t3 = col[(q + 48) * C::SA];
+    if (sel) {
+      const cplx<T> u02 = mk<T>(t0.x - t2.x, t0.y - t2.y), u13 = mk<T>(t1.x - t3.x, t1.y - t3.y);
+      const cplx<T> w = tw[C::NR + 16 + q];
+      u[q] = cmul(mk<T>(u02.x + u13.y, u02.y - u13.x), mk<T>(w.x, -w.y));
+    } else {
+      u[q] = mk<T>((t0.x + t2.x) + (t1.x + t3.x), (t0.y + t2.y) + (t1.y + t3.y));
+    }
+  }
+#pragma unroll
+  for (int s = 8; s >= 1; s >>= 1)
+#pragma unroll
+    for (int q = 0; q < s; ++q) u[q] = mk<T>(u[q].x + u[q + s].x, u[q].y + u[q + s].y);
+  const cplx<T> z = u[0];
+  const uint32_t lmask = (uint32_t)fwd_low_len(a.Lf) - 1u;
+  const int32_t j = (int32_t)f1 + (int32_t)a.N1 * (sel ? d2 - kFwdLowF2 : d2);
+  cplx<T>* __restrict__ dst = Xlow + ch * fwd_low_len(a.Lf);
+  dst[(uint32_t)j & lmask] = mk<T>(z.x, -z.y);
+  if (f1 != 0u && f1 != half) dst[(uint32_t)(-j) & lmask] = z;
 }
 
 template <typename T, class C, int KIND, bool COEF, bool BITS>
@@ -807,9 +863,9 @@
   return QI_OK;
 }
 
-template <typename T, class C, int SRC, int NPH>
+template <typename T, class C, int SRC, int NPH, bool LOW = false>
 static int launch_p1(const RowArgs<T>& a, dim3 grid, hipStream_t st) {
-  return launch_lds(k_pass1<T, C, SRC, NPH>, C::LDS_BYTES, a, grid, C::TH, st);
+  return launch_lds(k_pass1<T, C, SRC, NPH, LOW>, C::LDS_BYTES, a, grid, C::TH, st);
 }
 template <typename T, class C, int KIND, bool COEF, bool BITS>
 static int launch_p2v(const RowArgs<T>& a, dim3 grid, hipStream_t st) {
@@ -843,20 +899,20 @@
   return launch_pass1_cfg<double, Cfg<double, 8>>(a, kind, n_channels, st);
 }
 
-template <typename T, class C1>
-static int launch_forward_cfg(const RowArgs<T>& a0, cplx<T>* Xout, int64_t n_channels, hipStream_t st) {
-  using C2 = C1;
+template <typename T, class C1, bool LOW>
+static int launch_forward_p1(const RowArgs<T>& a0, int64_t n_channels, hipStream_t st) {
   RowArgs<T> a = a0;
   a.phase_split = a.N1 == 2048 && (a.N2 / C1::G) * n_channels < 256 ? 1 : 0;
   dim3 g1((unsigned)(a.N2 / C1::G), a.phase_split ? 2u : 1u, (unsigned)n_channels);
-  if (a.N1 == 1024)
-    QI_TRY((launch_p1<T, C1, 2, 1>(a, g1, st)));
-  else if (a.N1 == 2048)
-    QI_TRY((launch_p1<T, C1, 2, 2>(a, g1, st)));
-  else {
-    set_error("native forward transform supports N1 = 1024 or 2048, got %lld", (long long)a.N1);
-    return QI_ERR_UNSUPPORTED;
-  }
+  if (a.N1 == 1024) return launch_p1<T, C1, 2, 1, LOW>(a, g1, st);
+  if (a.N1 == 2048) return launch_p1<T, C1, 2, 2, LOW>(a, g1, st);
+  set_error("native forward transform supports N1 = 1024 or 2048, got %lld", (long long)a.N1);
+  return QI_ERR_UNSUPPORTED;
+}
+template <typename T, class C1>
+static int launch_forward_cfg(const RowArgs<T>& a, cplx<T>* Xout, int64_t n_channels, hipStream_t st) {
+  using C2 = C1;
+  QI_TRY((launch_forward_p1<T, C1, false>(a, n_channels, st)));
   auto kern = k_fwd2<T, C2>;
   QI_TRY(allow_dynamic_lds(reinterpret_cast<const void*>(kern), C2::LDS_BYTES));
   dim3 g2((unsigned)(a.N1 / C2::G), 1, (unsigned)n_channels);
@@ -864,13 +920,35 @@
   QI_LAUNCH_CHECK();
   return QI_OK;
 }
+template <typename T, class C2>
+static int launch_fwd2_low(const RowArgs<T>& a, cplx<T>* Xlow, int64_t n_channels, hipStream_t st) {
+  auto kern = k_fwd2_low<T, C2>;
+  QI_TRY(allow_dynamic_lds(reinterpret_cast<const void*>(kern), C2::LDS_BYTES));
+  dim3 g2((unsigned)ceil_div(fwd_low_rows(a.N1), C2::G), 1, (unsigned)n_channels);
+  kern<<<g2, C2::TH, C2::LDS_BYTES, st>>>(a, Xlow);
+  QI_LAUNCH_CHECK();
+  return QI_OK;
+}
 template <>
-int launch_forward<float>(const RowArgs<float>& a, float2* Xout, int64_t n_channels, hipStream_t st) {
-  if (n_channels * (a.N2 / 16) < 256) return launch_forward_cfg<float, Cfg<float, 8>>(a, Xout, n_channels, st);
-  return launch_forward_cfg<float, Cfg<float, 16>>(a, Xout, n_channels, st);
+int launch_forward<float>(const RowArgs<float>& a, float2* Xout, int64_t n_channels, hipStream_t st, bool low) {
+  const bool few = n_channels * (a.N2 / 16) < 256;
+  if (!low) {
+    if (few) return launch_forward_cfg<float, Cfg<float, 8>>(a, Xout, n_channels, st);
+    return launch_forward_cfg<float, Cfg<float, 16>>(a, Xout, n_channels, st);
+  }
+  if (few) QI_TRY((launch_forward_p1<float, Cfg<float, 8>, true>(a, n_channels, st)));
+  else QI_TRY((launch_forward_p1<float, Cfg<float, 16>, true>(a, n_channels, st)));
+  const int64_t rows = fwd_low_rows(a.N1) * n_channels;
+  if (rows >= 256 * 16) return launch_fwd2_low<float, Cfg<float, 16>>(a, Xout, n_channels, st);
+  if (rows >= 256 * 8) return launch_fwd2_low<float, Cfg<float, 8>>(a, Xout, n_channels, st);
+  return launch_fwd2_low<float, Cfg<float, 4>>(a, Xout, n_channels, st);
 }
 template <>
-int launch_forward<double>(const RowArgs<double>& a, double2* Xout, int64_t n_channels, hipStream_t st) {
+int launch_forward<double>(const RowArgs<double>& a, double2* Xout, int64_t n_channels, hipStream_t st, bool low) {
+  if (low) {
+    set_error("the low-bins forward transform is float32 only");
+    return QI_ERR_UNSUPPORTED;
+  }
   return launch_forward_cfg<double, Cfg<double, 8>>(a, Xout, n_channels, st);
 }
 
diff --git a/quantum_inferno_amd/csrc/qi_native.hpp b/quantum_inferno_amd/csrc/qi_native.hpp
--- a/quantum_inferno_amd/csrc/qi_native.hpp
+++ b/quantum_inferno_amd/csrc/qi_native.hpp
@@ -60,8 +60,12 @@
 
 template <typename T>
 int launch_pass1(const RowArgs<T>& a, int kind, int64_t n_channels, hipStream_t st);
-template <typename T>
-int launch_forward(const RowArgs<T>& a, cplx<T>* Xout, int64_t n_channels, hipStream_t st);
+constexpr int kFwdLowF2 = 16;
+constexpr int64_t fwd_low_bins(int64_t Lf) { return Lf / kN2 * kFwdLowF2; }
+constexpr int64_t fwd_low_len(int64_t Lf) { return 2 * fwd_low_bins(Lf); }
+constexpr int64_t fwd_low_rows(int64_t N1) { return N1 / 2 + 1; }
+template <typename T>
+int launch_forward(const RowArgs<T>& a, cplx<T>* Xout, int64_t n_channels, hipStream_t st, bool low = false);
 template <typename T>
 int launch_pass2(const RowArgs<T>& a, int kind, int rows_per_group, int nchunk, int64_t n_channels, hipStream_t st);
 struct EdgeBand {
@@ -184,6 +188,7 @@
   const float* lvl_weights[kZoomClasses];
   const cplx<T>* X;
   int32_t x_shift;
+  uint32_t x_mask;
   const cplx<T>* Hc;
   cplx<T>* split_part;
   int32_t split_rows;
diff --git a/quantum_inferno_amd/csrc/qi_plan_build.hip b/quantum_inferno_amd/csrc/qi_plan_build.hip
--- a/quantum_inferno_amd/csrc/qi_plan_build.hip
+++ b/quantum_inferno_amd/csrc/qi_plan_build.hip
@@ -8,6 +8,26 @@
 namespace host {
 
 bool native_len_ok(int64_t Lf) { return Lf == (1ll << 20) || Lf == (1ll << 21); }
+
+int64_t table_low_bins(const qi_plan* p, int kind) {
+  const auto& t = p->nat[kind];
+  if (!t.ready || p->d.dtype != QI_F32 || !p->native_fwd || !p->native_fwd_low || !native_len_ok(t.Lf)) return 0;
+  if (!t.h_rows.empty() || (kind == 0 && p->nat[3].ready && p->nedge > 0)) return 0;
+  const int64_t kmax = native::fwd_low_bins(t.Lf);
+  int64_t K = 1;
+  while (K <= kmax && !(t.x_lo > -K && t.x_hi < K)) K *= 2;
+  return K <= kmax ? K : 0;
+}
+bool forward_low(const qi_plan* p) {
+  if (p->d.dtype != QI_F32) return false;
+  bool any = false;
+  for (int kind = 0; kind < 3; ++kind) {
+    if (!p->nat[kind].ready) continue;
+    if (table_low_bins(p, kind) == 0) return false;
+    any = true;
+  }
+  return any;
+}
 
 bool native_wanted(const qi_plan* p, int kind) {
   if (p->d.engine == QI_ENGINE_HIPFFT) return false;
@@ -94,7 +114,7 @@
   return make_double2((double)cosl(ang), (double)sinl(ang));
 }
 
-int upload_zoom_list(qi_plan* p, qi_plan::NativeTable& t, int64_t Lf, std::vector<native::BandDesc>& bands) {
+int upload_zoom_list(qi_plan* p, qi_plan::NativeTable& t, int64_t Lf, std::vector<native::BandDesc>& bands, bool stx) {
   std::vector<native::BandDesc> rest;
   std::vector<std::vector<native::BandDesc>> by_level(native::kZoomClasses);
   for (const auto& d : bands) {
@@ -119,6 +139,18 @@
   t.h_zoom.clear();
   t.zoom_planes = 0;
   t.zoom_max_level = 0;
+  t.x_lo = 0;
+  t.x_hi = -1;
+  for (const auto& lvl : by_level)
+    for (const auto& d : lvl) {
+      const int64_t lo = d.k_lo + (stx ? d.shift : 0), hi = lo + d.k_len - 1;
+      if (t.x_lo > t.x_hi) {
+        t.x_lo = lo;
+        t.x_hi = hi;
+      }
+      t.x_lo = lo < t.x_lo ? lo : t.x_lo;
+      t.x_hi = hi > t.x_hi ? hi : t.x_hi;
+    }
   for (int g = 0; g < native::kZoomClasses; ++g) t.zoom_count[g] = (int32_t)by_level[g].size();
   for (int gi = 0; gi < native::kZoomClasses; ++gi) {
     const int g = kZoomListOrder[gi];
@@ -296,7 +328,7 @@
     for (const auto& d : bands)
       fprintf(stderr, "[qi plan] table %d (Lf = %lld) band %d: %s, support [%d, +%d)\n", kind, (long long)Lf, d.out_band,
               d.mode == 0 ? "one-pass loader" : (d.mode == 1 ? "two-pass" : "zoom"), d.k_lo, d.k_len);
-  QI_TRY(upload_zoom_list(p, t, Lf, bands));
+  QI_TRY(upload_zoom_list(p, t, Lf, bands, kind == 2));
   if (z64_table(p, kind)) QI_TRY(upload_z64_list(p, t, kind, Lf, bands));
   return upload_two_pass_groups(p, t, Lf, bands);
 }
diff --git a/quantum_inferno_amd/csrc/qi_run.hip b/quantum_inferno_amd/csrc/qi_run.hip
--- a/quantum_inferno_amd/csrc/qi_run.hip
+++ b/quantum_inferno_amd/csrc/qi_run.hip
@@ -441,8 +441,8 @@
 };
 
 template <typename T>
-int launch_spectra(qi_plan* p, const T* sig, int64_t n, int64_t Lf, bool shorts, bool have_spectra, const Scratch<T>& s,
-                   int64_t ct, hipStream_t st) {
+int launch_spectra(qi_plan* p, const T* sig, int64_t n, int64_t Lf, bool shorts, bool have_spectra, bool low,
+                   const Scratch<T>& s, int64_t ct, hipStream_t st) {
   p->prof.begin(st, QI_STAGE_FORWARD);
   if (have_spectra) {
   } else if (p->native_fwd && native_len_ok(Lf)) {
@@ -456,7 +456,7 @@
     f.sig = sig;
     f.two_over_len = (float)(2.0 / (double)Lf);
     f.debug = 0;
-    QI_TRY(native::launch_forward<T>(f, s.X, ct, st));
+    QI_TRY(native::launch_forward<T>(f, s.X, ct, st, low));
   } else {
     QI_TRY(launch_pack_pad<T>(sig, s.X, ct, n, Lf, st));
     QI_TRY(fft_c2c<T>(p->fft, s.X, Lf, ct, HIPFFT_FORWARD, st));
@@ -687,6 +687,7 @@
   z.plane_band = zt.d_zoom_plane_band;
   z.X = s.X;
   z.x_shift = x_shift ? 1 : 0;
+  z.x_mask = (uint32_t)((forward_low(p) ? native::fwd_low_len(zt.Lf) : zt.Lf) << z.x_shift) - 1u;
   z.Hc = static_cast<const cplx<T>*>(zt.Hc);
   z.coarse = s.zoom;
   z.stx = kind == 2 ? 1 : 0;
@@ -829,8 +830,14 @@
                p->nat[kind].h_rows.empty() && !shorts;
   const int32_t nsplit = kind == 0 ? p->nsplit : 0;
   ScratchBytes e = scratch_bytes<T>(p, n, B, nbk, stat_slots, chunk_total, shorts, time_via_part, out->coef != nullptr, nsplit);
-  e.x = (size_t)(share ? 2 * Lf0 : Lf0) * sizeof(cplx<T>);
-  e.imd = (size_t)(tp.imd_elems < Lf0 ? Lf0 : tp.imd_elems) * sizeof(cplx<T>);
+  const bool low = forward_low(p);
+  const int64_t x_len = low ? native::fwd_low_len(Lf0) : Lf0;
+  const int64_t fwd_imd = low ? native::fwd_low_rows(Lf0 / native::kN2) * native::kN2 : Lf0;
+  if (tune_env("QI_NATIVE_VERBOSE"))
+    fprintf(stderr, "[qi run] forward transform of table %d (Lf = %lld): %s, bins read (-%lld, %lld)\n", kind, (long long)Lf0,
+            low ? "low bins" : "every bin", (long long)table_low_bins(p, kind), (long long)table_low_bins(p, kind));
+  e.x = (size_t)(share ? 2 * x_len : x_len) * sizeof(cplx<T>);
+  e.imd = (size_t)(tp.imd_elems < fwd_imd ? fwd_imd : tp.imd_elems) * sizeof(cplx<T>);
   e.zoom = zoom ? (size_t)zt.zoom_planes * native::kBlk * sizeof(cplx<T>) : 0;
   const size_t per_chan = e.per_record();
   if (probe) {
@@ -879,7 +886,7 @@
     const TileOut<T> v = tile_out<T>(out, c0, B, n, time_via_part ? s.time_part : nullptr, s.part_band, s.part_stat, nbk,
                                      stat_slots, chunk_total);
     if (shorts) QI_HIP(hipMemsetAsync(s.parts0, 0, s.parts_bytes, st));
-    QI_TRY(launch_spectra<T>(p, sig_t, n, Lf0, shorts, share, s, ct, st));
+    QI_TRY(launch_spectra<T>(p, sig_t, n, Lf0, shorts, share, low, s, ct, st));
     QI_TRY(launch_two_pass<T>(p, tp, v, s, G, tp.nblk_max, true, ct, st));
     if (zoom)
       QI_TRY(launch_zoom_stage(p, zoom_args(p, kind, zr, v, s, share, nsplit, p2_stats + blk_stats, chunk_z0), zt.zoom_max_level,
@@ -1096,7 +1103,7 @@
     const TileOut<T> v = tile_out<T>(out, c0, B, n, time_via_part ? s.time_part : nullptr, s.part_band, s.part_stat, nbk,
                                      stat_slots, chunk_total);
     if (clear_parts) QI_HIP(hipMemsetAsync(s.parts0, 0, s.parts_bytes, st));
-    QI_TRY(launch_spectra<T>(p, sig_t, n, Lf, shorts, false, s, ct, st));
+    QI_TRY(launch_spectra<T>(p, sig_t, n, Lf, shorts, false, false, s, ct, st));
     QI_TRY(launch_two_pass<T>(p, tp, v, s, G, nblk, false, ct, st));
     QI_TRY(launch_z64_stage(p, kind, zr, v, s, nsplit, nblk, tp.chunk_total, ct, st));
     if (blocks)
diff --git a/quantum_inferno_amd/csrc/qi_zoom.hip b/quantum_inferno_amd/csrc/qi_zoom.hip
--- a/quantum_inferno_amd/csrc/qi_zoom.hip
+++ b/quantum_inferno_amd/csrc/qi_zoom.hip
@@ -21,7 +21,7 @@
   const int32_t kappa0 = (int32_t)(blockIdx.x * 256 + threadIdx.x);
   const uint32_t tau1 = plane - (uint32_t)bd.edge;
   const int64_t ch = blockIdx.z;
-  const cplx<T>* __restrict__ X = a.X + ch * (a.Lf << a.x_shift);
+  const cplx<T>* __restrict__ X = a.X + ch * ((int64_t)a.x_mask + 1);
   a.coarse[((int64_t)ch * a.planes + bd.edge) * kBlk + (int32_t)tau1 * kBlk + kappa0] =
       zoom_gather_value<T, STX>(a, bd, tau1, kappa0, X);
 }
diff --git a/quantum_inferno_amd/csrc/qi_zoom_gather.hpp b/quantum_inferno_amd/csrc/qi_zoom_gather.hpp
--- a/quantum_inferno_amd/csrc/qi_zoom_gather.hpp
+++ b/quantum_inferno_amd/csrc/qi_zoom_gather.hpp
@@ -13,7 +13,6 @@
   const int32_t M = (int32_t)((a.Lf / kZoomD) << bd.edge_slot), P = M / kBlk;
   const int32_t kc = STX ? 0 : bd.k_lo + bd.k_len / 2;
   const int32_t ks_lo = bd.k_lo - kc, ks_hi = ks_lo + bd.k_len;
-  const uint32_t lmask = (uint32_t)a.Lf - 1u;
   cplx<T> acc = mk<T>(T(0), T(0));
   const int32_t ks0 = ks_lo + ((kappa0 - ks_lo) & (kBlk - 1));
   if (ks0 >= ks_hi) return acc;
@@ -22,12 +21,12 @@
     const int32_t k = kc + ks;
     cplx<T> y;
     if (STX) {
-      const cplx<T> x = X[((uint32_t)(k + (int32_t)bd.shift) & lmask) << a.x_shift];
+      const cplx<T> x = X[((uint32_t)(k + (int32_t)bd.shift) << a.x_shift) & a.x_mask];
       const T g0 = (T)bd.coef * (T)k;
       const T g = exp2_t(-g0 * g0) * a.inv_len;
       y = mk<T>(x.x * g, x.y * g);
     } else {
-      y = cmul(X[((uint32_t)k & lmask) << a.x_shift], a.Hc[bd.src_off + (k - bd.k_lo)]);
+      y = cmul(X[((uint32_t)k << a.x_shift) & a.x_mask], a.Hc[bd.src_off + (k - bd.k_lo)]);
     }
     float sr, cr;
     sincospif(2.0f * (float)((r * tau1) & (uint32_t)(P - 1)) / (float)P, &sr, &cr);
@@ -46,7 +45,6 @@
   const int32_t M = (int32_t)((a.Lf / kZoomD) << bd.edge_slot), P = M / kBlk;
   const int32_t kc = STX ? 0 : bd.k_lo + bd.k_len / 2;
   const int32_t ks_lo = bd.k_lo - kc, ks_hi = ks_lo + bd.k_len;
-  const uint32_t lmask = (uint32_t)a.Lf - 1u;
   const int nterm = (bd.k_len + kBlk - 1) / kBlk;
   int32_t ks0[16];
 #pragma unroll
@@ -78,9 +76,9 @@
         h[q] = mk<T>(T(0), T(0));
         if (on[q]) {
           if (STX) {
-            x[q] = X[((uint32_t)(k + (int32_t)bd.shift) & lmask) << a.x_shift];
+            x[q] = X[((uint32_t)(k + (int32_t)bd.shift) << a.x_shift) & a.x_mask];
           } else {
-            x[q] = X[((uint32_t)k & lmask) << a.x_shift];
+            x[q] = X[((uint32_t)k << a.x_shift) & a.x_mask];
             h[q] = a.Hc[bd.src_off + (k - bd.k_lo)];
           }
         }
diff --git a/quantum_inferno_amd/engine.py b/quantum_inferno_amd/engine.py
--- a/quantum_inferno_amd/engine.py
+++ b/quantum_inferno_amd/engine.py
@@ -196,6 +196,9 @@
     def stage_bands(self, stage):
         k = _lib.STAGES.index(stage)
         return [int(self._lib.qi_plan_stage_bands(self._handle, which, k)) for which in (0, 1, 2)]
+
+    def forward_low(self, which):
+        return int(self._lib.qi_plan_forward_low(self._handle, which))
 
     def band_route(self, which, band, records=1):
         r = _lib.BandRoute()
```

New measurement: 423,600 Mpoints/s (median of 6 runs). 2.2% higher.
